# orjfickel/Small-Project-UV-Robot-Ray-Tracer

Hardware: AMD Instinct MI355X
Metric: Mray/s (extend+shade) on C046_1.glb 1920x1080x8-bounce (higher is better)
Workload: dtype f32; 1 GPU; testroomopt.glb (stand-in for the absent rooms/C046_1.glb), 2073600 photons/launch x 8 waves, lamp 0 of lange_route.xml, SEED_0=0; step = reset + generate + extend of all waves (batched), accumulate + shade replayed per wave + sync; triangles=44866, mode=batched, launch_pipelining=True, flavour=0, seed_mode=0, wide_bvh=False, parallelism=1 GPU, self_comm=False, high_priority_stream=False, full=False

## Files before the change

include/uvrt.h:

```cpp
#ifndef UVRT_H
#define UVRT_H

#include <stdint.h>

#ifdef __cplusplus
extern "C" {
#endif

typedef struct uvrt_ctx uvrt_ctx;

enum {
    UVRT_OK = 0,
    UVRT_ERR_INVALID = -1,
    UVRT_ERR_HIP = -2,
    UVRT_ERR_NO_DEVICE = -3,
    UVRT_ERR_BVH = -4,
    UVRT_ERR_STACK = -5
};

enum { UVRT_MAP_SUM = 0, UVRT_MAP_MAX = 1 };

const char* uvrt_last_error(void);
const char* uvrt_version(void);

// ... 32 lines not shown

int uvrt_get_seed(uvrt_ctx* ctx, uint32_t* seed);
int uvrt_set_seed(uvrt_ctx* ctx, uint32_t seed);
uint32_t uvrt_seed_next(const float light_pos[3], float light_length, uint32_t seed_prev);

int uvrt_advance_seed(uvrt_ctx* ctx, const float light_pos[3], float light_length);

int uvrt_set_seed_mode(uvrt_ctx* ctx, int32_t mode);
uint32_t uvrt_seed_next_mode(const float light_pos[3], float light_length, uint32_t seed_prev,
                             int32_t seed_mode);

int uvrt_generate_sweep(uvrt_ctx* ctx, const float from[3], const float to[3], float light_length,
                        int64_t first_gid, int64_t n);
uint32_t uvrt_seed_next_sweep(const float from[3], float light_length, uint32_t seed_prev);
int uvrt_write_free_rays(uvrt_ctx* ctx, const void* rays32, int64_t n);

int uvrt_occluded(uvrt_ctx* ctx, const void* rays32, int64_t n, uint8_t* out);
typedef struct {
    float from[3], to[3];
    float light_length;
    int32_t samples;
    uint32_t seed;
    int32_t photons_equiv;
    int32_t reserved[2];
} uvrt_gather_params;
enum { UVRT_GATHER_INDEPENDENT = 0, UVRT_GATHER_STRATIFIED = 1 };
int uvrt_set_gather_sampling(uvrt_ctx* ctx, int32_t mode);
int uvrt_get_gather_sampling(uvrt_ctx* ctx, int32_t* mode);
int uvrt_set_gather_variance(uvrt_ctx* ctx, int32_t on);
int uvrt_get_gather_variance(uvrt_ctx* ctx, int32_t* on);
int uvrt_read_variance(uvrt_ctx* ctx, double* out, int32_t first, int32_t count);
int uvrt_write_variance(uvrt_ctx* ctx, const double* in, int32_t first, int32_t count);
int uvrt_gather_direct(uvrt_ctx* ctx, const uvrt_gather_params* params, int32_t first_tri, int32_t tri_count);
int uvrt_accumulate_expected(uvrt_ctx* ctx, float time_step, int32_t tri_count);
int uvrt_read_expected(uvrt_ctx* ctx, double* out, int32_t first, int32_t count);
int uvrt_write_expected(uvrt_ctx* ctx, const double* in, int32_t first, int32_t count);

typedef struct {
    double  rel_error;
    double  min_expected;
    int32_t max_extra;
    uint32_t seed;
    int32_t reserved[2];
} uvrt_refine_params;
typedef struct { int64_t extra_rays; int32_t refined; int32_t reserved; } uvrt_refine_report;
int uvrt_gather_refine(uvrt_ctx* ctx, const uvrt_refine_params* params, int32_t first_tri, int32_t tri_count,
                       uvrt_refine_report* report );
int uvrt_read_gather_extra(uvrt_ctx* ctx, int32_t* out, int32_t first, int32_t count);
int uvrt_refine_counts(uvrt_ctx* ctx, int32_t samples0, const uvrt_refine_params* params, int32_t first_tri, int32_t tri_count,
                       int32_t* offsets_out );

enum { UVRT_GATHER_BATCH_MAX = 64 };
int uvrt_gather_direct_batch(uvrt_ctx* ctx, const uvrt_gather_params* launches, int32_t count,
                             int32_t first_tri, int32_t tri_count);
int uvrt_gather_batch_select(uvrt_ctx* ctx, int32_t k);
int uvrt_gather_batch_info(uvrt_ctx* ctx, int32_t out4[4]);
int uvrt_read_gather_batch(uvrt_ctx* ctx, int32_t k, int32_t which, double* out, int32_t first, int32_t count);

int uvrt_closest_hits(uvrt_ctx* ctx, const void* rays32, int64_t n, float* dist_out, int32_t* tri_out);

typedef struct {
    float    reflectance;
    int32_t  samples;
    uint32_t seed;
    int32_t  add;
    int32_t  reserved[2];
} uvrt_indirect_params;
int uvrt_indirect_source_from_expected(uvrt_ctx* ctx);
int uvrt_read_indirect_source(uvrt_ctx* ctx, double* out, int32_t first, int32_t count);
int uvrt_write_indirect_source(uvrt_ctx* ctx, const double* in, int32_t first, int32_t count);
int uvrt_gather_indirect(uvrt_ctx* ctx, const uvrt_indirect_params* params, int32_t first_tri, int32_t tri_count);
int uvrt_gather_indirect_rays(uvrt_ctx* ctx, const uvrt_indirect_params* params, int32_t first_tri, int32_t tri_count,
                              void* rays32_out);

typedef struct {
    int32_t  samples;
    uint32_t seed;
    int32_t  reserved[2];
} uvrt_links_params;
int uvrt_indirect_links_build(uvrt_ctx* ctx, const uvrt_links_params* params);
int uvrt_indirect_links_info(uvrt_ctx* ctx, int32_t out4[4]);
int uvrt_read_indirect_links(uvrt_ctx* ctx, int32_t* out, int32_t first_tri, int32_t tri_count);
typedef struct {
    float    reflectance;
    int32_t  bounces;
    int32_t  add;
    int32_t  reserved[3];
} uvrt_linked_params;
int uvrt_gather_indirect_linked(uvrt_ctx* ctx, const uvrt_linked_params* params, int32_t first_tri, int32_t tri_count);

int uvrt_set_gather_faces(uvrt_ctx* ctx, int32_t on);
int uvrt_get_gather_faces(uvrt_ctx* ctx, int32_t* on);
int uvrt_read_gather_faces(uvrt_ctx* ctx, int32_t face, double* out, int32_t first, int32_t count);
int uvrt_write_gather_faces(uvrt_ctx* ctx, int32_t face, const double* in, int32_t first, int32_t count);
int uvrt_indirect_links_build_sided(uvrt_ctx* ctx, const uvrt_links_params* params);
int uvrt_gather_indirect_linked_sided(uvrt_ctx* ctx, const uvrt_linked_params* params, int32_t first_tri, int32_t tri_count);

typedef struct {
    float duration;
    int32_t shade;
    int32_t which_map;
    int32_t photons_per_light;
    float scaled_power, min_value;
    int32_t threshold_view;
} uvrt_replay_op;

int uvrt_trace_batch(uvrt_ctx* ctx, const float* lamps, float light_length, int32_t count,
                     int64_t first_gid, int64_t n);
enum { UVRT_LAUNCH_STOP = 0, UVRT_LAUNCH_SWEEP = 1 };
typedef struct {
    float from[3];
    float to[3];
    int32_t kind;
    int32_t reserved;
} uvrt_launch;
int uvrt_trace_batch_launches(uvrt_ctx* ctx, const uvrt_launch* launches, float light_length,
                              int32_t count, int64_t first_gid, int64_t n);
int uvrt_replay_batch(uvrt_ctx* ctx, const uvrt_replay_op* ops, int32_t count, int32_t tri_count);
int uvrt_fold_batch(uvrt_ctx* ctx);
int uvrt_read_batch_counts(uvrt_ctx* ctx, int32_t launch, int32_t* out, int32_t first, int32_t count);

int uvrt_set_dedupe(uvrt_ctx* ctx, int32_t on);
int uvrt_set_dedupe_classes(uvrt_ctx* ctx, int32_t max_classes);
int uvrt_get_dedupe_classes(uvrt_ctx* ctx, int32_t* max_classes);
int32_t uvrt_dedupe_classes_default(void);
int uvrt_batch_deposits(uvrt_ctx* ctx, int64_t* out);
int uvrt_batch_residue(uvrt_ctx* ctx, int64_t* nonzero);
int uvrt_dedupe_classes(const float lamp[3], int32_t count, const uint32_t* seed_prev, const uint32_t* seed_next,
                        int32_t seed_mode, int64_t first_gid, int64_t n, int32_t max_classes, uint32_t* class_masks,
                        int32_t* class_count, int64_t* deposits);
int uvrt_set_helper_priority(uvrt_ctx* ctx, int32_t prio);
int uvrt_get_helper_priority(uvrt_ctx* ctx, int32_t* prio);
int uvrt_batch_traced_rays(uvrt_ctx* ctx, int64_t* out);
uint32_t uvrt_seed_input(int64_t gid, const float lamp[3], uint32_t seed_prev, uint32_t seed_next, int32_t seed_mode);
int uvrt_dedupe_plan(const float lamp[3], int32_t count, const uint32_t* seed_prev, const uint32_t* seed_next,
                     int32_t seed_mode, int64_t first_gid, int64_t n, uint32_t* masks);
int uvrt_dedupe_plan_tiled(const float lamp[3], int32_t count, const uint32_t* seed_prev, const uint32_t* seed_next,
                           int32_t seed_mode, int64_t first_gid, int64_t n, int32_t tile_keys, int64_t chunk_first,
                           int64_t chunk_n, uint32_t* masks);
int uvrt_dedupe_plan_strips(const float lamp[3], int32_t count, const uint32_t* seed_prev, const uint32_t* seed_next,
                            int32_t seed_mode, int64_t first_gid, int64_t n, int32_t tile_keys, int32_t strip_tiles,
                            int64_t chunk_first, int64_t chunk_n, uint32_t* masks);
int uvrt_dedupe_mark_device(uvrt_ctx* ctx, const float lamp[3], int32_t count, const uint32_t* seed_prev,
                            const uint32_t* seed_next, int32_t seed_mode, int64_t first_gid, int64_t n, int64_t chunk_first,
                            int64_t chunk_n, uint32_t* masks, uint32_t* block_owner_counts);
int uvrt_set_dedupe_periodic(uvrt_ctx* ctx, int32_t on);
int uvrt_get_dedupe_periodic(uvrt_ctx* ctx, int32_t* on);
int uvrt_dedupe_plan_periodic(const float lamp[3], int32_t count, const uint32_t* seed_prev, const uint32_t* seed_next,
                              int32_t seed_mode, int64_t first_gid, int64_t n, int64_t chunk_first, int64_t chunk_n,
                              uint32_t* masks, uint32_t* block_owner_counts, int64_t* from_table);
int uvrt_dedupe_generate_device(uvrt_ctx* ctx, const float lamp[3], float light_length, int32_t count, const uint32_t* seed_prev,
                                const uint32_t* seed_next, int32_t seed_mode, int64_t first_gid, int64_t n, int64_t chunk_first,
                                int64_t chunk_n, float* rays, uint32_t* words, uint32_t* total, uint32_t* deposits);

int uvrt_comm_available(void);
int uvrt_comm_unique_id(void* id128);
int uvrt_comm_init_rank(uvrt_ctx* ctx, const void* id128, int32_t rank, int32_t world);
int uvrt_comm_init_all(uvrt_ctx** ctxs, int32_t n);
int uvrt_comm_destroy(uvrt_ctx* ctx);
int uvrt_comm_info(uvrt_ctx* ctx, int32_t out4[4]);
int uvrt_reduce_batch(uvrt_ctx* ctx);
int uvrt_reduce_batch_group(uvrt_ctx** ctxs, int32_t n);

enum { UVRT_PLAN_CONVERGED = 0, UVRT_PLAN_ITERATION_CAP = 1 };
typedef struct {
    float min_dose;
    float scaled_power;
    int64_t photons_per_position;
    int32_t min_photons;
    int32_t max_iterations;
    double margin;
    double rel_gap;
    const uint8_t* mask;
    int32_t reserved[2];
} uvrt_plan_params;
typedef struct {
    int32_t status;
    int32_t iterations;
    int32_t positions;
    int32_t used_positions;
    int32_t required, unreachable, unresolved, masked_out;
    double area_required, area_unreachable, area_unresolved, area_masked_out;
    double total_duration;
    double lower_bound;
    double gap;
    double min_dose_ratio;
} uvrt_plan_report;
int uvrt_plan_begin(uvrt_ctx* ctx, int32_t positions);
int uvrt_plan_capture_batch(uvrt_ctx* ctx, const int32_t* position_of_launch, int32_t count);
int uvrt_plan_solve(uvrt_ctx* ctx, const uvrt_plan_params* params, float* durations_out, uvrt_plan_report* report);
int uvrt_plan_model_dose(uvrt_ctx* ctx, const float* durations, float* out, int32_t first, int32_t count);
int uvrt_plan_read_exposure(uvrt_ctx* ctx, int32_t position, uint32_t* out, int32_t first, int32_t count);
int uvrt_plan_read_required(uvrt_ctx* ctx, uint8_t* out, int32_t first, int32_t count);
int uvrt_plan_write_exposure(uvrt_ctx* ctx, int32_t position, const uint32_t* in, int32_t first, int32_t count);
int uvrt_plan_end(uvrt_ctx* ctx);
typedef struct {
    const float*   lower;
    const uint8_t* fixed;
    int32_t reserved[2];
} uvrt_plan_bounds;
typedef struct {
    int32_t fixed_columns, free_columns;
    int32_t met_by_lower;
    int32_t short_rows;
    double  area_met_by_lower, area_short;
    double  lower_total;
    int32_t reserved[2];
} uvrt_plan_bounds_report;
int uvrt_plan_solve_bounded(uvrt_ctx* ctx, const uvrt_plan_params* params, const uvrt_plan_bounds* bounds,
                            float* durations_out, uvrt_plan_report* report, uvrt_plan_bounds_report* bounds_report );
int uvrt_plan_read_classes(uvrt_ctx* ctx, uint8_t* out, int32_t first, int32_t count);
int uvrt_plan_begin_expected(uvrt_ctx* ctx, int32_t positions);
int uvrt_plan_capture_expected(uvrt_ctx* ctx, int32_t position);
int uvrt_plan_read_exposure_expected(uvrt_ctx* ctx, int32_t position, double* out, int32_t first, int32_t count);
int uvrt_plan_begin_expected_variance(uvrt_ctx* ctx, int32_t positions);
int uvrt_plan_read_exposure_variance(uvrt_ctx* ctx, int32_t position, double* out, int32_t first, int32_t count);
int uvrt_plan_lower_confidence(uvrt_ctx* ctx, double z);
float uvrt_plan_round_trip_up(float v);

int uvrt_set_sort_bits(uvrt_ctx* ctx, int32_t bits);
int uvrt_set_record_hits(uvrt_ctx* ctx, int32_t on);
int uvrt_set_flavour(uvrt_ctx* ctx, int32_t flavour);
int uvrt_set_wide_bvh(uvrt_ctx* ctx, int32_t on);
int uvrt_set_hot_records(uvrt_ctx* ctx, int32_t mode);
int uvrt_set_record_perm(uvrt_ctx* ctx, const uint32_t* perm, int32_t n);
int uvrt_read_record_perm(uvrt_ctx* ctx, uint32_t* out, int32_t n);

int uvrt_set_pipeline(uvrt_ctx* ctx, int32_t on);

int uvrt_set_variant(uvrt_ctx* ctx, int32_t variant);

int uvrt_read_rays(uvrt_ctx* ctx, void* rays32, int64_t first, int64_t count);
int uvrt_write_rays(uvrt_ctx* ctx, const void* rays32, int64_t n);
int uvrt_read_counts(uvrt_ctx* ctx, int32_t* out, int32_t first, int32_t count);
int uvrt_read_photon_map(uvrt_ctx* ctx, int32_t which_map, double* out, int32_t first,
                         int32_t count);
int uvrt_device_ptr(uvrt_ctx* ctx, int32_t which, void** ptr, int64_t* bytes);
int uvrt_copy_device(uvrt_ctx* ctx, int32_t which, void* ext_dev_ptr, int32_t to_ctx);
int uvrt_extend_time_ms(uvrt_ctx* ctx, double* ms, int64_t* launches);
int uvrt_set_timing(uvrt_ctx* ctx, int32_t on);
int uvrt_clock_probe_start(uvrt_ctx* ctx, int32_t microseconds);
int uvrt_clock_probe_read(uvrt_ctx* ctx, double* shader_mhz);
int uvrt_device_cus(uvrt_ctx* ctx);
int uvrt_device_count(void);

#ifdef __cplusplus
}
#endif
#endif
```

small-project-uv-robot-ray-tracer_amd/capi.py:

```python
from __future__ import annotations

import ctypes as C
import os

import numpy as np

_HERE = os.path.dirname(os.path.abspath(__file__))
LIB_PATH = os.path.join(_HERE, "libuvrt_hip.so")
LIB_DEV_PATH = os.path.join(_HERE, "libuvrt_hip_dev.so")

RAY_DT = np.dtype([("dirx", "<f4"), ("diry", "<f4"), ("dirz", "<f4"),
                   ("origx", "<f4"), ("origy", "<f4"), ("origz", "<f4"),
                   ("dist", "<f4"), ("triID", "<u4")])

MAP_SUM, MAP_MAX = 0, 1

_vp, _i32, _i64, _f32, _u32 = C.c_void_p, C.c_int32, C.c_int64, C.c_float, C.c_uint32
_fp = C.POINTER(C.c_float)
SYMBOLS = [
    ("uvrt_last_error", C.c_char_p, []),
    ("uvrt_version", C.c_char_p, []),
    ("uvrt_create", C.c_int, [C.c_int, C.POINTER(_vp)]),
    ("uvrt_destroy", None, [_vp]),
    ("uvrt_set_stream", C.c_int, [_vp, _vp]),
    ("uvrt_set_scene", C.c_int, [_vp, _vp, _i32, _vp, _i32, _vp]),
    ("uvrt_resize_rays", C.c_int, [_vp, _i64]),
    ("uvrt_reset", C.c_int, [_vp, _i32]),
    ("uvrt_generate", C.c_int, [_vp, _fp, _f32, _i64, _i64]),
    ("uvrt_extend", C.c_int, [_vp, _i64]),
    ("uvrt_accumulate", C.c_int, [_vp, _f32, _i32]),
    ("uvrt_compute_dosage", C.c_int, [_vp, _i32, _i32, _f32, _i32]),
    ("uvrt_dosage_to_color", C.c_int, [_vp, _f32, _i32, _i32]),
    ("uvrt_shade", C.c_int, [_vp, _i32, _i32, _f32, _f32, _i32, _i32]),
    ("uvrt_sync", C.c_int, [_vp]),
    ("uvrt_read_dosage", C.c_int, [_vp, _vp, _i32, _i32]),
    ("uvrt_read_color", C.c_int, [_vp, _vp, _i32, _i32]),
    ("uvrt_get_seed", C.c_int, [_vp, C.POINTER(_u32)]),
    ("uvrt_set_seed", C.c_int, [_vp, _u32]),
    ("uvrt_seed_next", _u32, [_fp, _f32, _u32]),
    ("uvrt_trace_batch", C.c_int, [_vp, _fp, _f32, _i32, _i64, _i64]),
    ("uvrt_trace_batch_launches", C.c_int, [_vp, _vp, _f32, _i32, _i64, _i64]),
    ("uvrt_replay_batch", C.c_int, [_vp, _vp, _i32, _i32]),
    ("uvrt_fold_batch", C.c_int, [_vp]),
    ("uvrt_read_batch_counts", C.c_int, [_vp, _i32, _vp, _i32, _i32]),
    ("uvrt_set_dedupe", C.c_int, [_vp, _i32]),
    ("uvrt_set_helper_priority", C.c_int, [_vp, _i32]),
    ("uvrt_get_helper_priority", C.c_int, [_vp, C.POINTER(_i32)]),
    ("uvrt_batch_traced_rays", C.c_int, [_vp, C.POINTER(_i64)]),
    ("uvrt_set_dedupe_classes", C.c_int, [_vp, _i32]),
    ("uvrt_get_dedupe_classes", C.c_int, [_vp, C.POINTER(_i32)]),
    ("uvrt_dedupe_classes_default", _i32, []),
    ("uvrt_batch_deposits", C.c_int, [_vp, C.POINTER(_i64)]),
    ("uvrt_batch_residue", C.c_int, [_vp, C.POINTER(_i64)]),
    ("uvrt_dedupe_classes", C.c_int, [_fp, _i32, _vp, _vp, _i32, _i64, _i64, _i32, _vp, C.POINTER(_i32), C.POINTER(_i64)]),
    ("uvrt_seed_input", _u32, [_i64, _fp, _u32, _u32, _i32]),
    ("uvrt_dedupe_plan", C.c_int, [_fp, _i32, _vp, _vp, _i32, _i64, _i64, _vp]),
    ("uvrt_dedupe_plan_tiled", C.c_int, [_fp, _i32, _vp, _vp, _i32, _i64, _i64, _i32, _i64, _i64, _vp]),
    ("uvrt_dedupe_plan_strips", C.c_int, [_fp, _i32, _vp, _vp, _i32, _i64, _i64, _i32, _i32, _i64, _i64, _vp]),
    ("uvrt_dedupe_mark_device", C.c_int, [_vp, _fp, _i32, _vp, _vp, _i32, _i64, _i64, _i64, _i64, _vp, _vp]),
    ("uvrt_set_dedupe_periodic", C.c_int, [_vp, _i32]),
    ("uvrt_get_dedupe_periodic", C.c_int, [_vp, C.POINTER(_i32)]),
    ("uvrt_dedupe_plan_periodic", C.c_int, [_fp, _i32, _vp, _vp, _i32, _i64, _i64, _i64, _i64, _vp, _vp, C.POINTER(_i64)]),
    ("uvrt_dedupe_generate_device", C.c_int, [_vp, _fp, C.c_float, _i32, _vp, _vp, _i32, _i64, _i64, _i64, _i64, _vp, _vp,
                                              C.POINTER(C.c_uint32), C.POINTER(C.c_uint32)]),
    ("uvrt_comm_available", C.c_int, []),
    ("uvrt_comm_info", C.c_int, [_vp, C.POINTER(_i32)]),
    ("uvrt_comm_unique_id", C.c_int, [_vp]),
    ("uvrt_comm_init_rank", C.c_int, [_vp, _vp, _i32, _i32]),
    ("uvrt_comm_init_all", C.c_int, [C.POINTER(_vp), _i32]),
    ("uvrt_comm_destroy", C.c_int, [_vp]),
    ("uvrt_reduce_batch", C.c_int, [_vp]),
    ("uvrt_reduce_batch_group", C.c_int, [C.POINTER(_vp), _i32]),
    ("uvrt_advance_seed", C.c_int, [_vp, _fp, _f32]),
    ("uvrt_set_seed_mode", C.c_int, [_vp, _i32]),
    ("uvrt_seed_next_mode", _u32, [_fp, _f32, _u32, _i32]),
    ("uvrt_set_sort_bits", C.c_int, [_vp, _i32]),
    ("uvrt_set_record_hits", C.c_int, [_vp, _i32]),
    ("uvrt_set_flavour", C.c_int, [_vp, _i32]),
    ("uvrt_set_variant", C.c_int, [_vp, _i32]),
    ("uvrt_set_pipeline", C.c_int, [_vp, _i32]),
    ("uvrt_set_record_perm", C.c_int, [_vp, _vp, _i32]),
    ("uvrt_read_record_perm", C.c_int, [_vp, _vp, _i32]),
    ("uvrt_set_hot_records", C.c_int, [_vp, _i32]),
    ("uvrt_set_wide_bvh", C.c_int, [_vp, _i32]),
    ("uvrt_read_rays", C.c_int, [_vp, _vp, _i64, _i64]),
    ("uvrt_write_rays", C.c_int, [_vp, _vp, _i64]),
    ("uvrt_write_free_rays", C.c_int, [_vp, _vp, _i64]),
    ("uvrt_generate_sweep", C.c_int, [_vp, _fp, _fp, _f32, _i64, _i64]),
    ("uvrt_seed_next_sweep", _u32, [_fp, _f32, _u32]),
    ("uvrt_occluded", C.c_int, [_vp, _vp, _i64, _vp]),
    ("uvrt_gather_direct", C.c_int, [_vp, _vp, _i32, _i32]),
    ("uvrt_set_gather_sampling", C.c_int, [_vp, _i32]),
    ("uvrt_get_gather_sampling", C.c_int, [_vp, C.POINTER(_i32)]),
    ("uvrt_accumulate_expected", C.c_int, [_vp, _f32, _i32]),
    ("uvrt_read_expected", C.c_int, [_vp, _vp, _i32, _i32]),
    ("uvrt_write_expected", C.c_int, [_vp, _vp, _i32, _i32]),
    ("uvrt_read_counts", C.c_int, [_vp, _vp, _i32, _i32]),
    ("uvrt_read_photon_map", C.c_int, [_vp, _i32, _vp, _i32, _i32]),
    ("uvrt_device_ptr", C.c_int, [_vp, _i32, C.POINTER(_vp), C.POINTER(_i64)]),
    ("uvrt_copy_device", C.c_int, [_vp, _i32, _vp, _i32]),
    ("uvrt_extend_time_ms", C.c_int, [_vp, C.POINTER(C.c_double), C.POINTER(_i64)]),
    ("uvrt_set_timing", C.c_int, [_vp, _i32]),
    ("uvrt_clock_probe_start", C.c_int, [_vp, _i32]),
    ("uvrt_clock_probe_read", C.c_int, [_vp, C.POINTER(C.c_double)]),
    ("uvrt_device_cus", C.c_int, [_vp]),
    ("uvrt_device_count", C.c_int, []),
    ("uvrt_plan_begin", C.c_int, [_vp, _i32]),
    ("uvrt_plan_capture_batch", C.c_int, [_vp, _vp, _i32]),
    ("uvrt_plan_solve", C.c_int, [_vp, _vp, _vp, _vp]),
    ("uvrt_plan_model_dose", C.c_int, [_vp, _vp, _vp, _i32, _i32]),
    ("uvrt_plan_read_exposure", C.c_int, [_vp, _i32, _vp, _i32, _i32]),
    ("uvrt_plan_read_required", C.c_int, [_vp, _vp, _i32, _i32]),
    ("uvrt_plan_end", C.c_int, [_vp]),
    ("uvrt_plan_solve_bounded", C.c_int, [_vp, _vp, _vp, _vp, _vp, _vp]),
    ("uvrt_plan_read_classes", C.c_int, [_vp, _vp, _i32, _i32]),
    ("uvrt_plan_round_trip_up", _f32, [_f32]),
    ("uvrt_plan_begin_expected", C.c_int, [_vp, _i32]),
    ("uvrt_plan_capture_expected", C.c_int, [_vp, _i32]),
    ("uvrt_plan_read_exposure_expected", C.c_int, [_vp, _i32, _vp, _i32, _i32]),
    ("uvrt_set_gather_variance", C.c_int, [_vp, _i32]),
    ("uvrt_get_gather_variance", C.c_int, [_vp, C.POINTER(_i32)]),
    ("uvrt_read_variance", C.c_int, [_vp, _vp, _i32, _i32]),
    ("uvrt_write_variance", C.c_int, [_vp, _vp, _i32, _i32]),
    ("uvrt_plan_begin_expected_variance", C.c_int, [_vp, _i32]),
    ("uvrt_plan_read_exposure_variance", C.c_int, [_vp, _i32, _vp, _i32, _i32]),
    ("uvrt_plan_lower_confidence", C.c_int, [_vp, C.c_double]),
    ("uvrt_plan_write_exposure", C.c_int, [_vp, _i32, _vp, _i32, _i32]),
    ("uvrt_gather_refine", C.c_int, [_vp, _vp, _i32, _i32, _vp]),
    ("uvrt_read_gather_extra", C.c_int, [_vp, _vp, _i32, _i32]),
    ("uvrt_refine_counts", C.c_int, [_vp, _i32, _vp, _i32, _i32, _vp]),
    ("uvrt_gather_direct_batch", C.c_int, [_vp, _vp, _i32, _i32, _i32]),
    ("uvrt_gather_batch_select", C.c_int, [_vp, _i32]),
    ("uvrt_gather_batch_info", C.c_int, [_vp, _vp]),
    ("uvrt_read_gather_batch", C.c_int, [_vp, _i32, _i32, _vp, _i32, _i32]),
    ("uvrt_closest_hits", C.c_int, [_vp, _vp, _i64, _vp, _vp]),
    ("uvrt_indirect_source_from_expected", C.c_int, [_vp]),
    ("uvrt_read_indirect_source", C.c_int, [_vp, _vp, _i32, _i32]),
    ("uvrt_write_indirect_source", C.c_int, [_vp, _vp, _i32, _i32]),
    ("uvrt_gather_indirect", C.c_int, [_vp, _vp, _i32, _i32]),
    ("uvrt_gather_indirect_rays", C.c_int, [_vp, _vp, _i32, _i32, _vp]),
    ("uvrt_indirect_links_build", C.c_int, [_vp, _vp]),
    ("uvrt_indirect_links_info", C.c_int, [_vp, _vp]),
    ("uvrt_read_indirect_links", C.c_int, [_vp, _vp, _i32, _i32]),
    ("uvrt_gather_indirect_linked", C.c_int, [_vp, _vp, _i32, _i32]),
    ("uvrt_set_gather_faces", C.c_int, [_vp, _i32]),
    ("uvrt_get_gather_faces", C.c_int, [_vp, C.POINTER(_i32)]),
    ("uvrt_read_gather_faces", C.c_int, [_vp, _i32, _vp, _i32, _i32]),
    ("uvrt_write_gather_faces", C.c_int, [_vp, _i32, _vp, _i32, _i32]),
    ("uvrt_indirect_links_build_sided", C.c_int, [_vp, _vp]),
    ("uvrt_gather_indirect_linked_sided", C.c_int, [_vp, _vp, _i32, _i32]),
]

PLAN_CONVERGED, PLAN_ITERATION_CAP = 0, 1


class GatherParams(C.Structure):
    _fields_ = [("from_", C.c_float * 3), ("to", C.c_float * 3), ("light_length", C.c_float), ("samples", C.c_int32),
                ("seed", C.c_uint32), ("photons_equiv", C.c_int32), ("reserved", C.c_int32 * 2)]


class RefineParams(C.Structure):
    _fields_ = [("rel_error", C.c_double), ("min_expected", C.c_double), ("max_extra", C.c_int32), ("seed", C.c_uint32),
                ("reserved", C.c_int32 * 2)]


class RefineReport(C.Structure):
    _fields_ = [("extra_rays", C.c_int64), ("refined", C.c_int32), ("reserved", C.c_int32)]


class IndirectParams(C.Structure):
    _fields_ = [("reflectance", C.c_float), ("samples", C.c_int32), ("seed", C.c_uint32), ("add", C.c_int32),
                ("reserved", C.c_int32 * 2)]


class LinksParams(C.Structure):
    _fields_ = [("samples", C.c_int32), ("seed", C.c_uint32), ("reserved", C.c_int32 * 2)]


class LinkedParams(C.Structure):
    _fields_ = [("reflectance", C.c_float), ("bounces", C.c_int32), ("add", C.c_int32), ("reserved", C.c_int32 * 3)]


class PlanParams(C.Structure):
    _fields_ = [("min_dose", C.c_float), ("scaled_power", C.c_float), ("photons_per_position", C.c_int64),
                ("min_photons", C.c_int32), ("max_iterations", C.c_int32), ("margin", C.c_double),
                ("rel_gap", C.c_double), ("mask", C.c_void_p), ("reserved", C.c_int32 * 2)]


class PlanReport(C.Structure):
    _fields_ = [("status", C.c_int32), ("iterations", C.c_int32), ("positions", C.c_int32), ("used_positions", C.c_int32),
                ("required", C.c_int32), ("unreachable", C.c_int32), ("unresolved", C.c_int32), ("masked_out", C.c_int32),
                ("area_required", C.c_double), ("area_unreachable", C.c_double), ("area_unresolved", C.c_double),
                ("area_masked_out", C.c_double), ("total_duration", C.c_double), ("lower_bound", C.c_double),
                ("gap", C.c_double), ("min_dose_ratio", C.c_double)]

    def as_dict(self):
        d = {name: getattr(self, name) for name, _ in self._fields_}
        d["converged"] = d["status"] == PLAN_CONVERGED
        return d


class PlanBounds(C.Structure):
    _fields_ = [("lower", C.c_void_p), ("fixed", C.c_void_p), ("reserved", C.c_int32 * 2)]


class PlanBoundsReport(C.Structure):
    _fields_ = [("fixed_columns", C.c_int32), ("free_columns", C.c_int32), ("met_by_lower", C.c_int32),
                ("short_rows", C.c_int32), ("area_met_by_lower", C.c_double), ("area_short", C.c_double),
                ("lower_total", C.c_double), ("reserved", C.c_int32 * 2)]

    def as_dict(self):
        return {name: getattr(self, name) for name, _ in self._fields_ if name != "reserved"}


PLAN_ACTIVE, PLAN_UNREACHABLE, PLAN_UNRESOLVED, PLAN_MASKED_OUT, PLAN_MET_BY_LOWER, PLAN_SHORT = range(6)


def round_trip_up(v):
    return np.float32(lib().uvrt_plan_round_trip_up(float(np.float32(v))))

REPLAY_OP_DT = np.dtype([("duration", "<f4"), ("shade", "<i4"), ("which_map", "<i4"), ("photons_per_light", "<i4"),
                         ("scaled_power", "<f4"), ("min_value", "<f4"), ("threshold_view", "<i4")])

LAUNCH_STOP, LAUNCH_SWEEP = 0, 1
LAUNCH_DT = np.dtype([("from", "<f4", (3,)), ("to", "<f4", (3,)), ("kind", "<i4"), ("reserved", "<i4")])


def stop(at):
    return (tuple(at), (0.0, 0.0, 0.0), LAUNCH_STOP, 0)


def sweep(frm, to):
    return (tuple(frm), tuple(to), LAUNCH_SWEEP, 0)


_LIB = {}


class UvrtError(RuntimeError):
    pass


def lib(dev=False):
    if dev not in _LIB:
        path = LIB_DEV_PATH if dev else LIB_PATH
        if not os.path.exists(path):
            raise UvrtError("HIP extension missing: %s (run `python -c 'import __graft_entry__ as g; "
                            "g.build()'` or `make -C small-project-uv-robot-ray-tracer_amd`). "
                            "There is no CPU fallback." % path)
        L = C.CDLL(path)
        for name, res, args in SYMBOLS:
            fn = getattr(L, name)
            fn.restype = res
            fn.argtypes = args
        _LIB[dev] = L
    return _LIB[dev]


def needs_dev(variant):
    return variant != 0 and variant % 10 != 1


def _f3(v):
    return (C.c_float * 3)(*[float(np.float32(x)) for x in v])


def _ptr(a):
    return a.ctypes.data_as(C.c_void_p)


def seed_next(light_pos, light_length, seed_prev, seed_mode=0):
    return int(lib().uvrt_seed_next_mode(_f3(light_pos), float(np.float32(light_length)), int(seed_prev),
                                         int(seed_mode)))


def seed_input(gid, lamp, seed_prev, seed_next_, seed_mode=0):
    return int(lib().uvrt_seed_input(int(gid), _f3(lamp), int(seed_prev), int(seed_next_), int(seed_mode)))


def dedupe_plan(lamp, seed_prev, seed_next_, seed_mode, first_gid, n):
    sp = np.ascontiguousarray(seed_prev, dtype=np.uint32)
    sn = np.ascontiguousarray(seed_next_, dtype=np.uint32)
    assert sp.size == sn.size
    out = np.empty((sp.size, int(n)), dtype=np.uint32)
    rc = lib().uvrt_dedupe_plan(_f3(lamp), int(sp.size), _ptr(sp), _ptr(sn), int(seed_mode), int(first_gid), int(n), _ptr(out))
    if rc != 0:
        raise UvrtError("uvrt error %d: %s" % (rc, lib().uvrt_last_error().decode()))
    return out


def dedupe_classes_default():
    return int(lib().uvrt_dedupe_classes_default())


def dedupe_classes(lamp, seed_prev, seed_next_, seed_mode, first_gid, n, max_classes=None):
    sp = np.ascontiguousarray(seed_prev, dtype=np.uint32)
    sn = np.ascontiguousarray(seed_next_, dtype=np.uint32)
    assert sp.size == sn.size
    max_classes = dedupe_classes_default() if max_classes is None else max_classes
    out = np.zeros(DEDUPE_CLASS_MAX, dtype=np.uint32)
    nc, dep = _i32(), _i64()
    rc = lib().uvrt_dedupe_classes(_f3(lamp), int(sp.size), _ptr(sp), _ptr(sn), int(seed_mode), int(first_gid), int(n),
                                   int(max_classes), _ptr(out), C.byref(nc), C.byref(dep))
    if rc != 0:
        raise UvrtError("uvrt error %d: %s" % (rc, lib().uvrt_last_error().decode()))
    return out[:int(nc.value)].copy(), int(dep.value)


DEDUPE_CLASS_MAX = 32
DEDUPE_CLASS_LAUNCHES = 30
DEDUPE_TILE_KEYS = 3840
DEDUPE_MARK_KEYS = 960
DEDUPE_STRIP_TILES = 4
DEDUPE_BLOCK_GIDS = 2048


def dedupe_plan_tiled(lamp, seed_prev, seed_next_, seed_mode, first_gid, n, tile_keys=DEDUPE_TILE_KEYS, chunk_first=None,
                      chunk_n=None, strip_tiles=None):
    sp = np.ascontiguousarray(seed_prev, dtype=np.uint32)
    sn = np.ascontiguousarray(seed_next_, dtype=np.uint32)
    assert sp.size == sn.size
    chunk_first = first_gid if chunk_first is None else chunk_first
    chunk_n = n if chunk_n is None else chunk_n
    out = np.empty((sp.size, int(chunk_n)), dtype=np.uint32)
    if strip_tiles is None:
        rc = lib().uvrt_dedupe_plan_tiled(_f3(lamp), int(sp.size), _ptr(sp), _ptr(sn), int(seed_mode), int(first_gid), int(n),
                                          int(tile_keys), int(chunk_first), int(chunk_n), _ptr(out))
    else:
        rc = lib().uvrt_dedupe_plan_strips(_f3(lamp), int(sp.size), _ptr(sp), _ptr(sn), int(seed_mode), int(first_gid), int(n),
                                           int(tile_keys), int(strip_tiles), int(chunk_first), int(chunk_n), _ptr(out))
    if rc != 0:
        raise UvrtError("uvrt error %d: %s" % (rc, lib().uvrt_last_error().decode()))
    return out


def dedupe_plan_periodic(lamp, seed_prev, seed_next_, seed_mode, first_gid, n, chunk_first=None, chunk_n=None):
    sp = np.ascontiguousarray(seed_prev, dtype=np.uint32)
    sn = np.ascontiguousarray(seed_next_, dtype=np.uint32)
    assert sp.size == sn.size
    chunk_first = first_gid if chunk_first is None else chunk_first
    chunk_n = n if chunk_n is None else chunk_n
    masks = np.empty((sp.size, int(chunk_n)), dtype=np.uint32)
    owners = np.empty((sp.size, (int(chunk_n) + DEDUPE_BLOCK_GIDS - 1) // DEDUPE_BLOCK_GIDS), dtype=np.uint32)
    from_table = _i64()
    rc = lib().uvrt_dedupe_plan_periodic(_f3(lamp), int(sp.size), _ptr(sp), _ptr(sn), int(seed_mode), int(first_gid), int(n),
                                         int(chunk_first), int(chunk_n), _ptr(masks), _ptr(owners), C.byref(from_table))
    if rc != 0:
        raise UvrtError("uvrt error %d: %s" % (rc, lib().uvrt_last_error().decode()))
    return masks, owners, int(from_table.value)


def seed_next_sweep(frm, light_length, seed_prev):
    return int(lib().uvrt_seed_next_sweep(_f3(frm), float(np.float32(light_length)), int(seed_prev)))


def comm_unique_id():
    buf = C.create_string_buffer(128)
    rc = lib().uvrt_comm_unique_id(buf)
    if rc != 0:
        raise UvrtError("uvrt error %d: %s" % (rc, lib().uvrt_last_error().decode()))
    return buf.raw


def comm_available():
    ok = bool(lib().uvrt_comm_available())
    return ok, ("" if ok else lib().uvrt_last_error().decode())


def _ctx_array(ctxs):
    return (C.c_void_p * len(ctxs))(*[c._h for c in ctxs])


def comm_init_all(ctxs):
    rc = lib().uvrt_comm_init_all(_ctx_array(ctxs), len(ctxs))
    if rc != 0:
        raise UvrtError("uvrt error %d: %s" % (rc, lib().uvrt_last_error().decode()))


def reduce_batch_group(ctxs):
    rc = lib().uvrt_reduce_batch_group(_ctx_array(ctxs), len(ctxs))
    if rc != 0:
        raise UvrtError("uvrt error %d: %s" % (rc, lib().uvrt_last_error().decode()))


class Ctx:

    def __init__(self, device=0, dev=False):
        self._L = lib(dev)
        h = C.c_void_p()
        self._h = None
        self._ck(self._L.uvrt_create(int(device), C.byref(h)))
        self._h = h
        self.T = 0

    def _ck(self, rc):
        if rc != 0:
            raise UvrtError("uvrt error %d: %s" % (rc, self._L.uvrt_last_error().decode()))

    def close(self):
        if self._h is not None:
            self._L.uvrt_destroy(self._h)
            self._h = None

    def __del__(self):
        try:
            self.close()
        except Exception:
            pass

    def set_stream(self, stream_ptr):
        self._ck(self._L.uvrt_set_stream(self._h, C.c_void_p(stream_ptr or 0)))

    def set_scene(self, tris, nodes, tri_idx):
        tris = np.ascontiguousarray(tris, dtype=np.float32).reshape(-1, 16)
        nodes = np.ascontiguousarray(nodes)
        tri_idx = np.ascontiguousarray(tri_idx, dtype=np.uint32)
        assert nodes.dtype.itemsize == 32
        self._ck(self._L.uvrt_set_scene(self._h, _ptr(tris), tris.shape[0], _ptr(nodes), nodes.shape[0],
                                        _ptr(tri_idx)))
        self.T = tris.shape[0]

    def resize_rays(self, n):
        self._ck(self._L.uvrt_resize_rays(self._h, int(n)))

    def reset(self, reset_color=True):
        self._ck(self._L.uvrt_reset(self._h, int(bool(reset_color))))

    def generate(self, light_pos, light_length, first_gid, n):
        self._ck(self._L.uvrt_generate(self._h, _f3(light_pos), float(np.float32(light_length)),
                                       int(first_gid), int(n)))

    def extend(self, n):
# ... 163 lines not shown

    def read_gather_batch(self, k, which=0, first=0, count=None):
        count = self.T - first if count is None else count
        out = np.empty(count, dtype=np.float64)
        self._ck(self._L.uvrt_read_gather_batch(self._h, int(k), int(which), _ptr(out), int(first), int(count)))
        return out

    def closest_hits(self, rays):
        rays = np.ascontiguousarray(rays, dtype=RAY_DT)
        dist = np.zeros(rays.size, dtype=np.float32)
        tri = np.zeros(rays.size, dtype=np.int32)
        self._ck(self._L.uvrt_closest_hits(self._h, _ptr(rays), rays.size, _ptr(dist), _ptr(tri)))
        return dist, tri

    def indirect_source_from_expected(self):
        self._ck(self._L.uvrt_indirect_source_from_expected(self._h))

    def read_indirect_source(self, first=0, count=None):
        count = self.T - first if count is None else count
        out = np.empty(count, dtype=np.float64)
        self._ck(self._L.uvrt_read_indirect_source(self._h, _ptr(out), int(first), int(count)))
        return out

    def write_indirect_source(self, values, first=0):
        v = np.ascontiguousarray(values, dtype=np.float64)
        self._ck(self._L.uvrt_write_indirect_source(self._h, _ptr(v), int(first), int(v.size)))

    @staticmethod
    def _indirect_params(reflectance, samples, seed, add):
        prm = IndirectParams()
        prm.reflectance = float(np.float32(reflectance))
        prm.samples = int(samples)
        prm.seed = int(seed) & 0xFFFFFFFF
        prm.add = int(add)
        return prm

    def gather_indirect(self, reflectance, samples, seed, add=0, first_tri=0, tri_count=None):
        prm = self._indirect_params(reflectance, samples, seed, add)
        self._ck(self._L.uvrt_gather_indirect(self._h, C.byref(prm), int(first_tri),
                                              self.T - int(first_tri) if tri_count is None else int(tri_count)))

    def gather_indirect_rays(self, reflectance, samples, seed, first_tri=0, tri_count=None):
        prm = self._indirect_params(reflectance, samples, seed, 0)
        tri_count = self.T - int(first_tri) if tri_count is None else int(tri_count)
        out = np.zeros(max(tri_count, 0) * max(int(samples), 0), dtype=RAY_DT)
        self._ck(self._L.uvrt_gather_indirect_rays(self._h, C.byref(prm), int(first_tri), tri_count, _ptr(out)))
        return out

    def indirect_links_build(self, samples, seed):
        prm = LinksParams()
        prm.samples = int(samples)
        prm.seed = int(seed) & 0xFFFFFFFF
        self._ck(self._L.uvrt_indirect_links_build(self._h, C.byref(prm)))

    def indirect_links_info(self):
        out = np.zeros(4, dtype=np.int32)
        self._ck(self._L.uvrt_indirect_links_info(self._h, _ptr(out)))
        return int(out[0]), int(out[1]) & 0xFFFFFFFF, int(out[2])

    def read_indirect_links(self, first_tri=0, tri_count=None):
        tri_count = self.T - int(first_tri) if tri_count is None else int(tri_count)
        s2 = self.indirect_links_info()[0]
        n = max(tri_count, 0) * s2
        out = np.zeros(max(n, 1), dtype=np.int32)
        self._ck(self._L.uvrt_read_indirect_links(self._h, _ptr(out), int(first_tri), tri_count))
        return out[:n].reshape(max(tri_count, 0), s2)

    def gather_indirect_linked(self, reflectance, bounces, add=0, first_tri=0, tri_count=None):
        prm = LinkedParams()
        prm.reflectance = float(np.float32(reflectance))
        prm.bounces = int(bounces)
        prm.add = int(add)
        self._ck(self._L.uvrt_gather_indirect_linked(self._h, C.byref(prm), int(first_tri),
                                                     self.T - int(first_tri) if tri_count is None else int(tri_count)))

    def indirect_links_build_sided(self, samples, seed):
        prm = LinksParams()
        prm.samples = int(samples)
        prm.seed = int(seed) & 0xFFFFFFFF
        self._ck(self._L.uvrt_indirect_links_build_sided(self._h, C.byref(prm)))

    def indirect_links_kind(self):
        out = np.zeros(4, dtype=np.int32)
        self._ck(self._L.uvrt_indirect_links_info(self._h, _ptr(out)))
        return int(out[3])

    def gather_indirect_linked_sided(self, reflectance, bounces, add=0, first_tri=0, tri_count=None):
        prm = LinkedParams()
        prm.reflectance = float(np.float32(reflectance))
        prm.bounces = int(bounces)
        prm.add = int(add)
        self._ck(self._L.uvrt_gather_indirect_linked_sided(self._h, C.byref(prm), int(first_tri),
                                                           self.T - int(first_tri) if tri_count is None else int(tri_count)))

    @property
    def seed(self):
        s = C.c_uint32()
        self._ck(self._L.uvrt_get_seed(self._h, C.byref(s)))
        return int(s.value)

    @seed.setter
    def seed(self, v):
        self._ck(self._L.uvrt_set_seed(self._h, int(v)))

    def trace_batch(self, lamps, light_length, first_gid, n):
        lamps = np.ascontiguousarray(lamps, dtype=np.float32).reshape(-1, 3)
        self._ck(self._L.uvrt_trace_batch(self._h, lamps.ctypes.data_as(_fp), float(np.float32(light_length)),
                                          lamps.shape[0], int(first_gid), int(n)))

    def trace_batch_launches(self, launches, light_length, first_gid, n):
        launches = np.ascontiguousarray(np.array(launches, dtype=LAUNCH_DT))
        self._ck(self._L.uvrt_trace_batch_launches(self._h, _ptr(launches), float(np.float32(light_length)),
                                                   launches.size, int(first_gid), int(n)))

    def replay_batch(self, ops, tri_count=None):
        ops = np.ascontiguousarray(np.array(ops, dtype=REPLAY_OP_DT))
        self._ck(self._L.uvrt_replay_batch(self._h, _ptr(ops), ops.size, self.T if tri_count is None else int(tri_count)))

    def fold_batch(self):
        self._ck(self._L.uvrt_fold_batch(self._h))

    def read_batch_counts(self, launch, first=0, count=None):
        count = self.T - first if count is None else count
        out = np.empty(count, dtype=np.int32)
        self._ck(self._L.uvrt_read_batch_counts(self._h, int(launch), _ptr(out), first, count))
        return out

    def set_dedupe(self, on):
        self._ck(self._L.uvrt_set_dedupe(self._h, 1 if on else 0))

    def set_helper_priority(self, prio):
        self._ck(self._L.uvrt_set_helper_priority(self._h, int(prio)))

    def get_helper_priority(self):
        m = _i32()
        self._ck(self._L.uvrt_get_helper_priority(self._h, C.byref(m)))
        return int(m.value)

    def set_dedupe_classes(self, max_classes):
        self._ck(self._L.uvrt_set_dedupe_classes(self._h, int(max_classes)))

    def get_dedupe_classes(self):
        m = _i32()
        self._ck(self._L.uvrt_get_dedupe_classes(self._h, C.byref(m)))
        return int(m.value)

    def set_dedupe_periodic(self, on):
        self._ck(self._L.uvrt_set_dedupe_periodic(self._h, 1 if on else 0))

    def get_dedupe_periodic(self):
        on = _i32()
        self._ck(self._L.uvrt_get_dedupe_periodic(self._h, C.byref(on)))
        return bool(on.value)

    def dedupe_generate_device(self, lamp, light_length, seed_prev, seed_next_, seed_mode, first_gid, n, chunk_first=None,
                               chunk_n=None):
        sp = np.ascontiguousarray(seed_prev, dtype=np.uint32)
        sn = np.ascontiguousarray(seed_next_, dtype=np.uint32)
        assert sp.size == sn.size
        chunk_first = first_gid if chunk_first is None else chunk_first
        chunk_n = n if chunk_n is None else chunk_n
        rays = np.zeros((sp.size * int(chunk_n), 4), dtype=np.float32)
        words = np.zeros(sp.size * int(chunk_n), dtype=np.uint32)
        total, deposits = C.c_uint32(), C.c_uint32()
        self._ck(self._L.uvrt_dedupe_generate_device(self._h, _f3(lamp), float(np.float32(light_length)), int(sp.size), _ptr(sp),
                                                     _ptr(sn), int(seed_mode), int(first_gid), int(n), int(chunk_first),
                                                     int(chunk_n), _ptr(rays), _ptr(words), C.byref(total), C.byref(deposits)))
        return rays[:total.value].copy(), words[:total.value].copy(), int(deposits.value)

    def batch_deposits(self):
        out = _i64()
        self._ck(self._L.uvrt_batch_deposits(self._h, C.byref(out)))
        return int(out.value)

    def batch_residue(self):
        out = _i64()
        self._ck(self._L.uvrt_batch_residue(self._h, C.byref(out)))
        return int(out.value)

    def batch_traced_rays(self):
        out = _i64()
        self._ck(self._L.uvrt_batch_traced_rays(self._h, C.byref(out)))
        return int(out.value)

    def dedupe_mark_device(self, lamp, seed_prev, seed_next_, seed_mode, first_gid, n, chunk_first=None, chunk_n=None):
        sp = np.ascontiguousarray(seed_prev, dtype=np.uint32)
        sn = np.ascontiguousarray(seed_next_, dtype=np.uint32)
        assert sp.size == sn.size
        chunk_first = first_gid if chunk_first is None else chunk_first
        chunk_n = n if chunk_n is None else chunk_n
        masks = np.empty((sp.size, int(chunk_n)), dtype=np.uint32)
        owners = np.empty((sp.size, (int(chunk_n) + DEDUPE_BLOCK_GIDS - 1) // DEDUPE_BLOCK_GIDS), dtype=np.uint32)
        self._ck(self._L.uvrt_dedupe_mark_device(self._h, _f3(lamp), int(sp.size), _ptr(sp), _ptr(sn), int(seed_mode),
                                                 int(first_gid), int(n), int(chunk_first), int(chunk_n), _ptr(masks),
                                                 _ptr(owners)))
        return masks, owners

    def comm_init_rank(self, id128, rank, world):
        assert len(id128) == 128
        self._ck(self._L.uvrt_comm_init_rank(self._h, C.c_char_p(id128), int(rank), int(world)))

    def comm_info(self):
        out = (C.c_int32 * 4)()
        self._ck(self._L.uvrt_comm_info(self._h, out))
        return {"world": int(out[0]), "rank": int(out[1]), "rccl_ranks": int(out[2]), "reserved_cus": int(out[3])}

    def comm_destroy(self):
        self._ck(self._L.uvrt_comm_destroy(self._h))

    def reduce_batch(self):
        self._ck(self._L.uvrt_reduce_batch(self._h))

    def advance_seed(self, light_pos, light_length):
        self._ck(self._L.uvrt_advance_seed(self._h, _f3(light_pos), float(np.float32(light_length))))

    def set_seed_mode(self, mode):
        self._ck(self._L.uvrt_set_seed_mode(self._h, int(mode)))

    def set_gather_sampling(self, mode):
        self._ck(self._L.uvrt_set_gather_sampling(self._h, int(mode)))

    def get_gather_sampling(self):
        m = _i32()
        self._ck(self._L.uvrt_get_gather_sampling(self._h, C.byref(m)))
        return int(m.value)

    def set_gather_variance(self, on):
        self._ck(self._L.uvrt_set_gather_variance(self._h, int(on)))

    def set_gather_faces(self, on):
        self._ck(self._L.uvrt_set_gather_faces(self._h, int(on)))

    def get_gather_faces(self):
        v = C.c_int32()
        self._ck(self._L.uvrt_get_gather_faces(self._h, C.byref(v)))
        return int(v.value)

    def get_gather_variance(self):
        v = _i32()
        self._ck(self._L.uvrt_get_gather_variance(self._h, C.byref(v)))
        return int(v.value)

    def set_sort_bits(self, bits):
        self._ck(self._L.uvrt_set_sort_bits(self._h, int(bits)))

    def set_record_hits(self, on):
        self._ck(self._L.uvrt_set_record_hits(self._h, int(bool(on))))

    def set_flavour(self, f):
        self._ck(self._L.uvrt_set_flavour(self._h, int(f)))

    def set_record_perm(self, perm):
        if perm is None:
            self._ck(self._L.uvrt_set_record_perm(self._h, None, 0))
            return
        perm = np.ascontiguousarray(perm, dtype=np.uint32)
        self._ck(self._L.uvrt_set_record_perm(self._h, perm.ctypes.data, int(perm.size)))

    def read_record_perm(self, npairs):
        out = np.empty(int(npairs), dtype=np.uint32)
        self._ck(self._L.uvrt_read_record_perm(self._h, _ptr(out), int(npairs)))
        return out

    def set_wide_bvh(self, on):
        self._ck(self._L.uvrt_set_wide_bvh(self._h, int(bool(on))))

    def set_hot_records(self, mode):
        self._ck(self._L.uvrt_set_hot_records(self._h, int(mode)))

    def set_pipeline(self, on):
        self._ck(self._L.uvrt_set_pipeline(self._h, int(bool(on))))

    def set_variant(self, v):
        self._ck(self._L.uvrt_set_variant(self._h, int(v)))

    def set_timing(self, on):
        self._ck(self._L.uvrt_set_timing(self._h, int(bool(on))))

    def extend_time_ms(self):
        ms, n = C.c_double(), C.c_int64()
        self._ck(self._L.uvrt_extend_time_ms(self._h, C.byref(ms), C.byref(n)))
        return float(ms.value), int(n.value)

    def copy_device(self, which, ext_ptr, to_ctx):
        self._ck(self._L.uvrt_copy_device(self._h, int(which), C.c_void_p(int(ext_ptr)), int(bool(to_ctx))))

    def clock_probe_start(self, microseconds):
        self._ck(self._L.uvrt_clock_probe_start(self._h, int(microseconds)))

    def clock_probe_read(self):
        mhz = C.c_double()
        self._ck(self._L.uvrt_clock_probe_read(self._h, C.byref(mhz)))
        return float(mhz.value)

    def device_cus(self):
        return int(self._L.uvrt_device_cus(self._h))

    def plan_begin(self, positions):
        self._ck(self._L.uvrt_plan_begin(self._h, int(positions)))
        self._plan_p = int(positions)

    def plan_begin_expected(self, positions):
        self._ck(self._L.uvrt_plan_begin_expected(self._h, int(positions)))
        self._plan_p = int(positions)

    def plan_capture_expected(self, position):
# ... 109 lines not shown
```

small-project-uv-robot-ray-tracer_amd/csrc/uvrt_capi.hip:

```cpp
#include "uvrt_ctx.h"
#include "uvrt_scene_layout.h"

#include <climits>
#include <cstddef>

using namespace uvrt;
using namespace uvrt_impl;

namespace uvrt_impl {

thread_local std::string g_err;

int fail(int code, const char* fmt, ...)
{
    char buf[512];
    va_list ap;
    va_start(ap, fmt);
    vsnprintf(buf, sizeof buf, fmt, ap);
    va_end(ap);
    g_err = buf;
    return code;
}

}

uvrt_ctx::~uvrt_ctx()
{
    plan_drop(this);
    (void)hot_reset(this, false);
    for (hipEvent_t e : {ev_fence, ev_mapfence}) if (e) (void)hipEventDestroy(e);
    for (hipEvent_t e : ev_pool) (void)hipEventDestroy(e);
    if (host_flag) (void)hipHostFree(host_flag);
    if (probe_stream) (void)hipStreamDestroy(probe_stream);
    if (own_stream) (void)hipStreamDestroy(own_stream);
}

namespace {

namespace sl = uvrt::scene_layout;
using sl::SceneLayout;

#define SAME_FIELD(A, B, f) (offsetof(A, f) == offsetof(B, f))
static_assert(sizeof(sl::F4) == sizeof(float4) && SAME_FIELD(sl::F4, float4, x) && SAME_FIELD(sl::F4, float4, y) &&
              SAME_FIELD(sl::F4, float4, z) && SAME_FIELD(sl::F4, float4, w), "F4 is float4's words");
static_assert(sizeof(sl::PairWords) == sizeof(PairRec) && SAME_FIELD(sl::PairWords, PairRec, c0min_ref0) &&
              SAME_FIELD(sl::PairWords, PairRec, c0max_ref1) && SAME_FIELD(sl::PairWords, PairRec, c1min) &&
              SAME_FIELD(sl::PairWords, PairRec, c1max), "PairWords is PairRec");
static_assert(sizeof(sl::QuadWords) == sizeof(QuadRec) && SAME_FIELD(sl::QuadWords, QuadRec, xz) && SAME_FIELD(sl::QuadWords, QuadRec, y01) &&
              SAME_FIELD(sl::QuadWords, QuadRec, y23) && SAME_FIELD(sl::QuadWords, QuadRec, ref) && SAME_FIELD(sl::QuadWords, QuadRec, pad),
              "QuadWords is QuadRec");
#undef SAME_FIELD
static_assert(sl::REF_LEAF_BIT == uvrt::REF_LEAF_BIT && sl::REF_DONE == uvrt::REF_DONE && sl::REF_COUNT_SHIFT == uvrt::REF_COUNT_SHIFT &&
              sl::MAX_TRIS == uvrt::MAX_TRIS && sl::TOP6_MAX == uvrt::TOP6_MAX, "uvrt_scene_layout.h restates uvrt_device.h's constants");

template <class I>
bool env_int(const char* name, long lo, long hi, I& field)
{
    const char* e = getenv(name);
    if (!e) return false;
    const long v = atol(e);
    if (v < lo || v > hi) return false;
    field = (I)v;
    return true;
}
void env_bool(const char* name, bool& field)
{
    if (const char* e = getenv(name)) field = atoi(e) != 0;
}

int provision_scene(uvrt_ctx* c, const SceneLayout& L, int32_t T)
{
    const bool resized = (T != c->T);
    int rc;
    if ((rc = c->pairs.ensure(std::max<size_t>(L.pairs.size(), 1) * sizeof(PairRec), false, c->stream))) return rc;
    for (int l = 0; l < c->nlanes; ++l)
        if ((rc = c->lanes[l].recs.ensure((L.pairs.size() + (size_t)T + 1) * 64, true, c->stream))) return rc;
    if ((rc = c->ltris.ensure((size_t)T * sizeof(LeafTri) + 16, true, c->stream))) return rc;
    if ((rc = c->leaf_count.ensure((size_t)T * 4, false, c->stream))) return rc;
    if ((rc = c->area.ensure((size_t)T * 4, false, c->stream))) return rc;
    if (resized || !c->photon_map.p) {
        for (DevBuf* b : {&c->photon_map, &c->max_map, &c->dosage}) b->release();
        for (Lane& La : c->lanes) La.counts.release();
        if ((rc = c->photon_map.ensure((size_t)T * 8, true, c->stream))) return rc;
        if ((rc = c->max_map.ensure((size_t)T * 8, true, c->stream))) return rc;
        int R = c->replicas_knob > 0 ? c->replicas_knob : 16;
        while (R > 1 && (size_t)R * (size_t)T * 4 > ((size_t)64 << 20)) R >>= 1;
        c->replicas = R;
        for (int l = 0; l < c->nlanes; ++l)
            if ((rc = c->lanes[l].counts.ensure((size_t)R * (size_t)T * 4, true, c->stream))) return rc;
        if ((rc = c->dosage.ensure((size_t)T * 4, true, c->stream))) return rc;
        if ((rc = c->color.ensure((size_t)T * 36, true, c->stream))) return rc;
    }
    return UVRT_OK;
}

int upload_scene(uvrt_ctx* c, const SceneLayout& L, const void* tris64, int32_t T, const uint32_t* tri_idx)
{
    int rc;
    if (!L.pairs.empty())
        HIP_TRY(hipMemcpyAsync(c->pairs.p, L.pairs.data(), L.pairs.size() * sizeof(PairRec), hipMemcpyHostToDevice, c->stream));
    if ((rc = c->quads.ensure(std::max<size_t>(L.quads.size(), 1) * sizeof(QuadRec), false, c->stream))) return rc;
    if (!L.quads.empty())
        HIP_TRY(hipMemcpyAsync(c->quads.p, L.quads.data(), L.quads.size() * sizeof(QuadRec), hipMemcpyHostToDevice, c->stream));
    HIP_TRY(hipMemcpyAsync(c->leaf_count.p, L.leaf_count.data(), (size_t)T * 4, hipMemcpyHostToDevice, c->stream));
    DevBuf d_tris, d_idx;
    if ((rc = d_tris.ensure((size_t)T * 64, false, c->stream))) return rc;
    if ((rc = d_idx.ensure((size_t)T * 4, false, c->stream))) return rc;
    HIP_TRY(hipMemcpyAsync(d_tris.p, tris64, (size_t)T * 64, hipMemcpyHostToDevice, c->stream));
    HIP_TRY(hipMemcpyAsync(d_idx.p, tri_idx, (size_t)T * 4, hipMemcpyHostToDevice, c->stream));
    launch_prepare_scene(d_tris.as<float4>(), d_idx.as<uint32_t>(), c->ltris.as<LeafTri>(),
                         c->area.as<float>(), T, c->stream);
    for (int l = 0; l < c->nlanes; ++l)
        launch_prepare_leaves6(c->ltris.as<LeafTri>(), c->lanes[l].recs.p, (int32_t)L.pairs.size(), T, c->stream);
    HIP_TRY(hipGetLastError());
    HIP_TRY(hipStreamSynchronize(c->stream));
    c->T = T;
    c->root_ref = L.root_ref;
    c->top_pairs = L.top_pairs;
    c->npairs = (int32_t)L.pairs.size();
    c->nquads = (int32_t)L.quads.size();
    c->top_quads = L.top_quads;
    c->scene_force_exact = L.force_exact;
    c->have_scene = true;
    return UVRT_OK;
}

int void_scene_state(uvrt_ctx* c)
{
    for (Lane& La : c->lanes) { La.recs_tag.valid = false; La.recs4_tag.valid = false; }
    for (Lane& La : c->lanes) La.recs4.release();
    c->have_perm = false;
    c->derived = {};
    if (int rc = hot_reset(c, true)) return rc;
    HIP_TRY(hipStreamSynchronize(c->stream));
    plan_drop(c);
    c->b_count = 0;
    c->b_is_folded = false;
    c->b_recs.clear();
    c->b_recs_key.clear();
    for (auto& bset : c->bs) for (DevBuf* b : {&bset.planes, &bset.folded}) b->release();
    return UVRT_OK;
}

}

extern "C" {

const char* uvrt_last_error(void) { return g_err.c_str(); }
const char* uvrt_version(void) { return "uvrt-mi355x 0.1 (gfx950)"; }
int uvrt_clock_probe_start(uvrt_ctx* c, int32_t microseconds)
{
    if (!c || microseconds < 1 || microseconds > 1000000) return fail(UVRT_ERR_INVALID, "uvrt_clock_probe_start: 1 .. 1 000 000 us");
    HIP_TRY(hipSetDevice(c->device));
    if (!c->probe_stream) {
        int lo = 0, hi = 0;
        HIP_TRY(hipDeviceGetStreamPriorityRange(&lo, &hi));
        HIP_TRY(hipStreamCreateWithPriority(&c->probe_stream, hipStreamNonBlocking, hi));
    }
    if (int rc = c->probe_out.ensure(16, true, c->probe_stream)) return rc;
    launch_clock_probe(c->probe_out.as<unsigned long long>(), (unsigned long long)microseconds * 100ull, c->probe_stream);
    HIP_TRY(hipGetLastError());
    return UVRT_OK;
}

int uvrt_clock_probe_read(uvrt_ctx* c, double* shader_mhz)
{
    if (!c || !shader_mhz || !c->probe_stream) return fail(UVRT_ERR_INVALID, "uvrt_clock_probe_read: no probe started");
    HIP_TRY(hipSetDevice(c->device));
    unsigned long long v[2] = {0, 0};
    HIP_TRY(hipMemcpyAsync(v, c->probe_out.p, 16, hipMemcpyDeviceToHost, c->probe_stream));
    HIP_TRY(hipStreamSynchronize(c->probe_stream));
    if (v[1] == 0) return fail(UVRT_ERR_HIP, "uvrt_clock_probe_read: the probe wrote nothing");
    *shader_mhz = (double)v[0] / (double)v[1] * 100.0;
    return UVRT_OK;
}

int uvrt_device_cus(uvrt_ctx* c) { return c ? c->num_cus : 0; }
int uvrt_device_count(void)
{
    int n = 0;
    return hipGetDeviceCount(&n) == hipSuccess ? n : 0;
}

int uvrt_create(int device_id, uvrt_ctx** out)
{
    if (!out) return fail(UVRT_ERR_INVALID, "uvrt_create: out is NULL");
    *out = nullptr;
    int ndev = 0;
    hipError_t e = hipGetDeviceCount(&ndev);
    if (e != hipSuccess || ndev <= 0)
        return fail(UVRT_ERR_NO_DEVICE, "uvrt_create: no HIP device (%s)", hipGetErrorString(e));
    if (device_id < 0 || device_id >= ndev)
        return fail(UVRT_ERR_INVALID, "uvrt_create: device %d out of range [0,%d)", device_id, ndev);
    hipDeviceProp_t prop;
    HIP_TRY(hipGetDeviceProperties(&prop, device_id));
    if (strncmp(prop.gcnArchName, "gfx950", 6) != 0)
        return fail(UVRT_ERR_NO_DEVICE, "uvrt_create: device %d is %s, this library is built for gfx950 only",
                    device_id, prop.gcnArchName);
    std::unique_ptr<uvrt_ctx> c(new uvrt_ctx());
    c->device = device_id;
    c->hot.reserve(uvrt_ctx::HOT_MAX);
    c->num_cus = prop.multiProcessorCount > 0 ? prop.multiProcessorCount : 256;
    if (c->num_cus > 256) c->num_cus = 256;
    env_int("UVRT_REPLICAS", 1, 64, c->replicas_knob);
    HIP_TRY(hipSetDevice(device_id));
    HIP_TRY(hipStreamCreateWithFlags(&c->own_stream, hipStreamNonBlocking));
    c->stream = c->own_stream;
    for (int l = 0; l < uvrt_ctx::MAXL; ++l) {
        if (l > 0) HIP_TRY(hipStreamCreateWithFlags(&c->lanes[l].side, hipStreamNonBlocking));
        HIP_TRY(hipEventCreateWithFlags(&c->lanes[l].ev_tail, hipEventDisableTiming));
    }
    HIP_TRY(hipEventCreateWithFlags(&c->ev_fence, hipEventDisableTiming));
    HIP_TRY(hipEventCreateWithFlags(&c->ev_mapfence, hipEventDisableTiming));
    env_int("UVRT_LANES", 1, uvrt_ctx::MAXL, c->nlanes);
    env_bool("UVRT_PIPELINE", c->pipeline);
    if (long mb = 0; env_int("UVRT_BATCH_CHUNK_MB", 1, LONG_MAX, mb)) c->batch_chunk_bytes = c->dedupe_chunk_bytes = (size_t)mb << 20;
#ifdef UVRT_DEV_VARIANTS
    env_int("UVRT_PROBE_SKIP_GENERATE", INT_MIN, INT_MAX, c->probe_skip_generate);
    env_bool("UVRT_NEARFAR_MINMAX", c->nearfar_minmax);
#endif
    env_bool("UVRT_DRAIN_MERGE", c->drain_merge);
    env_bool("UVRT_DEDUPE", c->dedupe);
    env_int("UVRT_DEDUPE_CLASSES", 0, DEDUPE_CLASS_MAX, c->dedupe_classes);
    env_bool("UVRT_DEDUPE_PERIODIC", c->dedupe_periodic);
    env_int("UVRT_DEDUPE_STRIP", 1, 1024, c->dedupe_strip);
    env_int("UVRT_DEDUPE_CLASS_REPLICAS", 1, 16, c->dedupe_class_replicas);
    if (long mb = 0; env_int("UVRT_DEDUPE_CLASS_MB", 1, 4096, mb)) c->dedupe_class_bytes = (size_t)mb << 20;
    env_int("UVRT_HELPER_PRIO", 0, 3, c->helper_prio);
    env_int("UVRT_BATCH_LANES", 1, uvrt_ctx::MAXL - 1, c->batch_lanes);
    if (int cus = 0; env_int("UVRT_COMM_RESERVE_CUS", 0, 64, cus) && cus % 8 == 0) c->comm_reserve_knob = cus;
    env_int("UVRT_HOT_SAMPLE", 256, 1 << 20, c->hot_sample);
    env_int("UVRT_HOT_DIRECT", 0, 8192, c->hot_direct);
    env_int("UVRT_HOT_TAIL", 0, 63, c->hot_tail);
    if (int rc = c->error_flag.ensure(256, true, c->stream)) return rc;
#ifndef UVRT_TRIP_STATS
    void* dp = nullptr;
    HIP_TRY(hipHostMalloc((void**)&c->host_flag, 64, hipHostMallocMapped | hipHostMallocCoherent));
    HIP_TRY(hipHostGetDevicePointer(&dp, c->host_flag, 0));
    memset(c->host_flag, 0, 64);
    c->host_flag_dev = (uint32_t*)dp;
#endif
    if (int rc = c->lanes[0].ovf.ensure((size_t)OVF_MAX_ENTRIES * sizeof(uint32_t), false, c->stream)) return rc;
    *out = c.release();
    return UVRT_OK;
}

void uvrt_destroy(uvrt_ctx* c)
{
    if (!c) return;
    (void)hipSetDevice(c->device);
    (void)hipStreamSynchronize(c->stream);
    for (Lane& L : c->lanes) if (L.side) (void)hipStreamSynchronize(L.side);
    if (c->probe_stream) (void)hipStreamSynchronize(c->probe_stream);
    if (c->comm) uvrt_comm_destroy(c);
    delete c;
}

int uvrt_set_stream(uvrt_ctx* c, void* hip_stream)
{
    if (!c) return fail(UVRT_ERR_INVALID, "null context");
    if (int rc = set_device(c)) return rc;
    if (int rc = join_all(c)) return rc;
    HIP_TRY(hipStreamSynchronize(c->stream));
    c->stream = hip_stream ? (hipStream_t)hip_stream : c->own_stream;
    c->lane = 0;
    return UVRT_OK;
}

int uvrt_set_scene(uvrt_ctx* c, const void* tris64, int32_t T, const void* nodes32,
                   int32_t node_count, const uint32_t* tri_idx)
{
    if (!c) return fail(UVRT_ERR_INVALID, "uvrt_set_scene: null argument");
    SceneLayout L;
    std::string why;
    if (int rc = sl::build_scene_layout(tris64, T, nodes32, node_count, tri_idx, L, why)) return fail(rc, "%s", why.c_str());
    if (int rc = set_device(c)) return rc;
    if (int rcj = join_all(c)) return rcj;
    HIP_TRY(hipStreamSynchronize(c->stream));
    c->lane = 0;
    if (int rc = provision_scene(c, L, T)) return rc;
    if (int rc = upload_scene(c, L, tris64, T, tri_idx)) return rc;
    return void_scene_state(c);
}

int uvrt_resize_rays(uvrt_ctx* c, int64_t photon_count)
{
    if (!c || photon_count < 0) return fail(UVRT_ERR_INVALID, "uvrt_resize_rays: bad argument");
    if (int rc = set_device(c)) return rc;
    if (photon_count == c->capacity && c->lanes[0].rays.p && (!c->record_hits || c->hits.p)) { c->last = {}; return UVRT_OK; }
    if (int rcj = join_all(c)) return rcj;
    HIP_TRY(hipStreamSynchronize(c->stream));
    c->lane = 0;
    int rc;
    const size_t n = (size_t)photon_count;
    for (int l = 0; l < c->nlanes; ++l)
        if ((rc = c->lanes[l].rays.ensure(n * 16, false, c->stream))) return rc;
    if ((rc = c->keyrank.ensure(n * 8, false, c->stream))) return rc;
    if ((rc = c->sorted.ensure(n * 16, false, c->stream))) return rc;
    if ((rc = c->order.ensure(n * 4, false, c->stream))) return rc;
    if (c->record_hits && (rc = c->hits.ensure(n * 8, false, c->stream))) return rc;
    for (Lane& L : c->lanes) L.oxz.release();
    c->capacity = photon_count;
    c->last = {};
    return UVRT_OK;
}

int uvrt_reset(uvrt_ctx* c, int32_t reset_color)
{
    if (!c || !c->have_scene) return fail(UVRT_ERR_INVALID, "uvrt_reset: no scene");
    if (int rc = set_device(c)) return rc;
    if (int rc = join_all(c)) return rc;
    launch_reset(c->photon_map.as<double>(), c->max_map.as<double>(), c->lanes[0].counts.as<int32_t>(),
                 c->replicas, c->T, c->color.as<float>(), reset_color, c->T, c->helper_prio, c->stream);
    HIP_TRY(hipGetLastError());
    bool dirty = false;
    for (int l = 0; l < uvrt_ctx::MAXL; ++l) {
        Lane& L = c->lanes[l];
        if (l > 0 && L.counts_dirty && L.counts.p) {
            HIP_TRY(hipMemsetAsync(L.counts.p, 0, L.counts.bytes, c->stream));
            dirty = true;
        }
        L.counts_dirty = false;
    }
    if (c->b_count > 0) {
        if (c->b_is_folded) HIP_TRY(hipMemsetAsync(c->bs[c->b_set].folded.p, 0, c->bs[c->b_set].folded.bytes, c->stream));
        else HIP_TRY(hipMemsetAsync(c->bs[c->b_set].planes.p, 0, c->bs[c->b_set].planes.bytes, c->stream));
        HIP_TRY(hipEventRecord(c->bs[c->b_set].free_ev, c->stream));
        c->b_count = 0;
        c->b_is_folded = false;
    }
    return dirty ? mark_fence(c) : mark_map_fence(c);
}

int uvrt_set_record_perm(uvrt_ctx* c, const uint32_t* perm, int32_t n)
{
    if (!c || !c->have_scene) return fail(UVRT_ERR_INVALID, "uvrt_set_record_perm: no scene");
    if (int rc = set_device(c)) return rc;
    if (int rc = join_all(c)) return rc;
    HIP_TRY(hipStreamSynchronize(c->stream));
    for (Lane& L : c->lanes) L.recs_tag.valid = false;
    if (!perm) { c->have_perm = false; return UVRT_OK; }
    if (n != c->npairs) return fail(UVRT_ERR_INVALID, "uvrt_set_record_perm: %d entries, the scene has %d inner nodes", n, c->npairs);
    std::vector<uint8_t> seen((size_t)n, 0);
    for (int32_t i = 0; i < n; ++i) {
        if (perm[i] >= (uint32_t)n || seen[perm[i]]) return fail(UVRT_ERR_INVALID, "uvrt_set_record_perm: not a permutation");
        seen[perm[i]] = 1;
    }
    if (n == 0) { c->have_perm = false; return UVRT_OK; }
    if (int rc = c->perm.ensure((size_t)n * 4, false, c->stream)) return rc;
    if (int rc = copy_sync(c, c->perm.p, perm, (size_t)n * 4, hipMemcpyHostToDevice)) return rc;
    c->have_perm = true;
    c->perm_gen = ++c->perm_clock;
    return UVRT_OK;
}

int uvrt_read_record_perm(uvrt_ctx* c, uint32_t* out, int32_t n)
{
    if (!c || !out || !c->have_scene || n != c->npairs)
        return fail(UVRT_ERR_INVALID, "uvrt_read_record_perm: need a scene and n = its %d inner nodes", c ? c->npairs : 0);
    if (int rc = set_device(c)) return rc;
    if (int rc = join_all(c)) return rc;
    const uint32_t* pm = c->have_perm ? c->perm.as<uint32_t>() : cur_lane(c).perm;
    if (!pm) { for (int32_t i = 0; i < n; ++i) out[i] = (uint32_t)i; return UVRT_OK; }
    return copy_sync(c, out, pm, (size_t)n * 4, hipMemcpyDeviceToHost);
}

int uvrt_sync(uvrt_ctx* c)
{
    if (!c) return fail(UVRT_ERR_INVALID, "null context");
    if (int rc = set_device(c)) return rc;
    if (int rc = join_all(c)) return rc;
    uint32_t flag = 0;
#ifdef UVRT_TRIP_STATS
    HIP_TRY(hipMemcpyAsync(&flag, c->error_flag.p, 4, hipMemcpyDeviceToHost, c->stream));
    HIP_TRY(hipStreamSynchronize(c->stream));
#else
    HIP_TRY(hipStreamSynchronize(c->stream));
// ... 316 lines not shown
```

small-project-uv-robot-ray-tracer_amd/csrc/uvrt_capi_batch.hip:

```cpp
#include "uvrt_ctx.h"

using namespace uvrt;
using namespace uvrt_impl;

namespace uvrt_impl {

static BatchKnobs batch_knobs(const uvrt_ctx* c)
{
    BatchKnobs kn = {};
    kn.seed = c->seed; kn.seed_mode = c->seed_mode; kn.T = c->T; kn.replicas = c->replicas;
    kn.may_dedupe = c->dedupe && variant_code6(c->variant) == 1;
#ifdef UVRT_DEV_VARIANTS
    kn.may_dedupe = kn.may_dedupe && c->probe_skip_generate <= 0;
#endif
    kn.dedupe_classes = c->dedupe_classes; kn.dedupe_class_replicas = c->dedupe_class_replicas;
    kn.dedupe_class_bytes = c->dedupe_class_bytes; kn.dedupe_periodic = c->dedupe_periodic;
    kn.dedupe_chunk_bytes = c->dedupe_chunk_bytes; kn.batch_chunk_bytes = c->batch_chunk_bytes; kn.dedupe_strip = c->dedupe_strip;
    return kn;
}

struct BatchRun {
    uvrt_ctx* c;
    int set;
    uvrt_ctx::BatchSet& S;
    const BatchPlan& P;
    const char* who;
    float light_length;
    int64_t first_gid, n;
    const uint32_t* gperm[MAX_BATCH];
    uint64_t ggen[MAX_BATCH];
    bool lane_waited[uvrt_ctx::MAXL];
    int per_cu;
    int64_t traced;
    size_t dd_used;
};

static int provision_records(BatchRun& r, bool* recs_stale)
{
    uvrt_ctx* c = r.c;
    const BatchPlan& P = r.P;
    uvrt_ctx::HotEntry* fresh[MAX_BATCH];
    uint32_t fresh_prev[MAX_BATCH], fresh_next[MAX_BATCH];
    int nfresh = 0;
    for (int g = 0; g < P.ngroups; ++g) {
        r.gperm[g] = c->have_perm ? c->perm.as<uint32_t>() : nullptr;
        bool is_fresh = false;
        if (!r.gperm[g] && (int64_t)P.gsize[g] * r.n >= 16384) {
            const int ph = P.gfirst[g];
            const float gl[3] = {P.gp.lx[ph], P.gp.ly[ph], P.gp.lz[ph]};
            uvrt_ctx::HotEntry* e = nullptr;
            if (int rcp = hot_lookup(c, gl, c->stream, &r.gperm[g], &e)) return rcp;
            if (e) {
                r.gperm[g] = e->perm;
                fresh[nfresh] = e; fresh_prev[nfresh] = P.gp.seed_prev[ph]; fresh_next[nfresh] = P.gp.seed_next[ph];
                ++nfresh;
                is_fresh = true;
            }
        }
        r.ggen[g] = perm_generation(c, r.gperm[g]);
        if (g >= (int)c->b_recs_key.size() || !c->b_recs_key[g].holds(P.gx[g], P.gz[g], r.gperm[g], r.ggen[g]) || is_fresh) {
            *recs_stale = true;
            if (g < (int)c->b_recs_key.size()) c->b_recs_key[g].tag.valid = false;
        }
    }
    if (nfresh > 0)
        if (int rcb = hot_build(c, fresh, fresh_prev, fresh_next, nfresh, r.light_length, c->stream, 0)) return rcb;
    return UVRT_OK;
}

static int provision_batch(BatchRun& r, int count)
{
    uvrt_ctx* c = r.c;
    uvrt_ctx::BatchSet& S = r.S;
    const BatchPlan& P = r.P;
    int rc;
    const int64_t n_pad = P.n_pad;
    const size_t plane_alloc = (size_t)c->replicas * (size_t)c->T;
    const size_t planes_bytes = (size_t)count * plane_alloc * 4 + (size_t)P.class_cap * P.plane_ints * 4;
    bool dd_scratch_short = false;
    for (int l = 0; l <= c->batch_lanes; ++l)
        dd_scratch_short = dd_scratch_short || c->lanes[l].dd_tmp.bytes < P.dd_tmp_bytes || c->lanes[l].dd_blocks.bytes < P.dd_block_bytes;
    const bool need_alloc = S.rays.bytes < (size_t)count * (size_t)n_pad * 16 || S.planes.bytes < planes_bytes ||
                            S.folded.bytes < (size_t)count * (size_t)c->T * 4 || (int)c->b_recs.size() < P.ngroups || !S.free_ev ||
                            S.oxz.bytes < (size_t)P.nsweeps * (size_t)n_pad * 8 || (P.nsweeps > 0 && !c->derived.free_recs_valid) ||
                            (P.dd_chunks > 0 && (S.masks.bytes < (size_t)count * (size_t)n_pad * 4 || S.dd_counts.bytes < P.dd_chunks * 8 ||
                                                 dd_scratch_short));
    bool recs_stale = false;
    if ((rc = provision_records(r, &recs_stale))) return rc;
    if (need_alloc || recs_stale) {
        if (int rcj = join_all(c)) return rcj;
    }
    if (need_alloc) {
        HIP_TRY(hipStreamSynchronize(c->stream));
        if (!S.free_ev) HIP_TRY(hipEventCreateWithFlags(&S.free_ev, hipEventDisableTiming));
        const bool grown = S.planes.bytes < planes_bytes || S.folded.bytes < (size_t)count * (size_t)c->T * 4;
        if ((rc = S.rays.ensure((size_t)count * (size_t)n_pad * 16, false, c->stream))) return rc;
        if ((rc = S.planes.ensure(planes_bytes, true, c->stream))) return rc;
        if ((rc = S.folded.ensure((size_t)count * (size_t)c->T * 4, true, c->stream))) return rc;
        if ((rc = S.oxz.ensure((size_t)P.nsweeps * (size_t)n_pad * 8, false, c->stream))) return rc;
        if (grown) HIP_TRY(hipEventRecord(S.free_ev, c->stream));
        while ((int)c->b_recs.size() < P.ngroups) {
            DevBuf b;
            if ((rc = b.ensure(((size_t)c->npairs + (size_t)c->T + 1) * 64, true, c->stream))) return rc;
            launch_prepare_leaves6(c->ltris.as<LeafTri>(), b.p, c->npairs, c->T, c->stream);
            c->b_recs.push_back(std::move(b));
        }
        c->b_recs_key.resize(c->b_recs.size());
        for (int l = 1; l <= c->batch_lanes; ++l)
            if ((rc = c->lanes[l].ovf.ensure(side_ovf_bytes(c), false, c->stream))) return rc;
        if (P.dd_chunks > 0) {
            if ((rc = S.masks.ensure((size_t)count * (size_t)n_pad * 4, false, c->stream))) return rc;
            if ((rc = S.dd_counts.ensure(P.dd_chunks * 8, false, c->stream))) return rc;
            for (int l = 0; l <= c->batch_lanes; ++l) {
                if ((rc = c->lanes[l].dd_tmp.ensure(P.dd_tmp_bytes, false, c->stream))) return rc;
                if ((rc = c->lanes[l].dd_blocks.ensure(P.dd_block_bytes, true, c->stream))) return rc;
            }
            HIP_TRY(hipStreamSynchronize(c->stream));
        }
    }
    if (need_alloc || recs_stale) {
        for (int g = 0; g < P.ngroups; ++g) {
            uvrt_ctx::RecsKey& key = c->b_recs_key[g];
            if (key.holds(P.gx[g], P.gz[g], r.gperm[g], r.ggen[g])) continue;
            launch_prepare_launch6(c->pairs.as<PairRec>(), c->b_recs[g].p, P.gx[g], P.gz[g], c->npairs, r.gperm[g], c->helper_prio, c->stream);
            key = {{true, P.gx[g], P.gz[g]}, r.gperm[g], r.ggen[g]};
        }
        if (P.nsweeps > 0 && !c->derived.free_recs_valid)
            if ((rc = make_free_records(c))) return rc;
        HIP_TRY(hipGetLastError());
        if (int rcf = mark_fence(c)) return rcf;
    }
    return UVRT_OK;
}

static int next_chunk_lane(BatchRun& r, hipStream_t* ls)
{
    uvrt_ctx* c = r.c;
    c->lane = c->pipeline ? 1 + (int)(c->b_chunks++ % (uint64_t)c->batch_lanes) : 0;
    *ls = stream_of(c, c->lane);
    if (c->lane != 0) cur_lane(c).used = true;
    if (!r.lane_waited[c->lane]) {
        HIP_TRY(hipStreamWaitEvent(*ls, r.S.free_ev, 0));
        r.lane_waited[c->lane] = true;
    }
    return UVRT_OK;
}
static void set_planes(const BatchRun& r, ExtendParams& p, int ph0, int kc)
{
    p.counts = r.S.planes.as<int32_t>() + (size_t)ph0 * r.P.plane_ints;
    p.count_replicas = r.P.R;
    p.count_stride = r.c->T;
    p.n = (int64_t)kc * r.P.n_pad;
    p.plane_batches = (uint32_t)(r.P.n_pad / 64);
    p.plane_n = (uint32_t)r.n;
    p.plane_stride = (uint32_t)r.P.plane_ints;
}

static void fill_dedupe_chunk(const uvrt_ctx* c, GenDedupeParams& dq, const Piece& pc, int64_t g0, int64_t gn, const Lane& L, float light_length)
{
    memset(&dq, 0, sizeof dq);
    dq.g = pc.G;
    dq.cls = pc.cls;
    dq.per = pc.per;
    dq.tmp = L.dd_tmp.as<uint32_t>();
    dq.g0 = g0;
    dq.gn = gn;
    dq.block_counts = L.dd_blocks.as<uint32_t>();
    mark_tiles(c->dedupe_strip, dq);
    dq.light_length = light_length;
    dq.prio = c->helper_prio;
}
static void copy_stops(GenBatchParams& gq, const BatchPlan& P, int ph0, int kc)
{
    for (int j = 0; j < kc; ++j) {
        gq.lx[j] = P.gp.lx[ph0 + j]; gq.ly[j] = P.gp.ly[ph0 + j]; gq.lz[j] = P.gp.lz[ph0 + j];
        gq.seed_prev[j] = P.gp.seed_prev[ph0 + j]; gq.seed_next[j] = P.gp.seed_next[ph0 + j];
    }
}
static void copy_sweeps(SweepBatchParams& sq, const BatchPlan& P, int k0, int kc)
{
    for (int j = 0; j < kc; ++j) {
        sq.fx[j] = P.sp.fx[k0 + j]; sq.fy[j] = P.sp.fy[k0 + j]; sq.fz[j] = P.sp.fz[k0 + j];
        sq.tx[j] = P.sp.tx[k0 + j]; sq.ty[j] = P.sp.ty[k0 + j]; sq.tz[j] = P.sp.tz[k0 + j];
        sq.seed_prev[j] = P.sp.seed_prev[k0 + j]; sq.seed_next[j] = P.sp.seed_next[k0 + j];
    }
}

static int enqueue_dedupe_chunk(BatchRun& r, const Piece& pc, int64_t g0, int64_t gn)
{
    uvrt_ctx* c = r.c;
    const BatchPlan& P = r.P;
    const int g = pc.g, ph0 = P.gfirst[g] + pc.k0;
    hipStream_t ls;
    if (int rcl = next_chunk_lane(r, &ls)) return rcl;
    const size_t at = (size_t)ph0 * (size_t)P.n_pad + (size_t)pc.kc * (size_t)g0;
    GenDedupeParams dq;
    fill_dedupe_chunk(c, dq, pc, r.first_gid + g0, gn, cur_lane(c), r.light_length);
    dq.rays = r.S.rays.as<float4>() + at;
    dq.masks = r.S.masks.as<uint32_t>() + at;
    dq.total = r.S.dd_counts.as<uint32_t>() + r.dd_used;
    dq.deposits = r.S.dd_counts.as<uint32_t>() + P.dd_chunks + r.dd_used++;
    launch_generate_dedupe(dq, ls);
    if (int rcl = lane_stream(c, &ls)) return rcl;
    ExtendParams p;
    fill_launch(c, p, P.gx[g], P.gz[g]);
    p.rays = dq.rays;
    p.masks = dq.masks;
    p.n_dev = dq.total;
    p.counts = r.S.planes.as<int32_t>() + (size_t)ph0 * P.plane_ints;
    p.count_replicas = P.R;
    p.count_stride = c->T;
    p.n = (int64_t)pc.kc * gn;
    p.plane_stride = (uint32_t)P.plane_ints;
    p.cls_replicas = pc.cls.count > 0 ? P.cls_repl : 0;
    p.recs = c->b_recs[g].p;
    p.perm = r.gperm[g];
    p.recs_prepared = 1;
    return timed_launch(c, ls, r.who, "the stops' launch", [&] { return launch_extend6_dedupe(p, variant_code6(c->variant), r.per_cu, ls); });
}

static int enqueue_stop_chunk(BatchRun& r, int g, int ph0, int kc)
{
    uvrt_ctx* c = r.c;
    const BatchPlan& P = r.P;
    r.traced += (int64_t)kc * r.n;
    hipStream_t ls;
    if (int rcl = next_chunk_lane(r, &ls)) return rcl;
    GenBatchParams gq;
    memset(&gq, 0, sizeof gq);
    gq.rays = r.S.rays.as<float4>() + (size_t)ph0 * (size_t)P.n_pad;
    gq.n_pad = P.n_pad;
    gq.first_gid = r.first_gid;
    gq.n = r.n;
    gq.light_length = r.light_length;
    gq.seed_mode = c->seed_mode;
    gq.count = kc;
    gq.prio = c->helper_prio;
    copy_stops(gq, P, ph0, kc);
#ifdef UVRT_DEV_VARIANTS
    if (!(c->probe_skip_generate > 0 && c->probe_batches >= c->probe_skip_generate))
#endif
    launch_generate_batch(gq, ls);
    if (int rcl = lane_stream(c, &ls)) return rcl;
    ExtendParams p;
    fill_launch(c, p, P.gx[g], P.gz[g]);
    p.rays = gq.rays;
    set_planes(r, p, ph0, kc);
    p.recs = c->b_recs[g].p;
    p.perm = r.gperm[g];
    p.recs_prepared = 1;
    return timed_launch(c, ls, r.who, "the stops' launch", [&] { return launch_extend6(p, variant_code6(c->variant), r.per_cu, c->helper_prio, ls); });
}

static int enqueue_sweep_chunk(BatchRun& r, int k0, int kc)
{
    uvrt_ctx* c = r.c;
    const BatchPlan& P = r.P;
    const int ph0 = P.nstops + k0;
    hipStream_t ls;
    if (int rcl = next_chunk_lane(r, &ls)) return rcl;
    SweepBatchParams sq;
    memset(&sq, 0, sizeof sq);
    sq.rays = r.S.rays.as<float4>() + (size_t)ph0 * (size_t)P.n_pad;
    sq.oxz = r.S.oxz.as<float2>() + (size_t)k0 * (size_t)P.n_pad;
    sq.n_pad = P.n_pad;
    sq.first_gid = r.first_gid;
    sq.n = r.n;
    sq.light_length = r.light_length;
    sq.count = kc;
    sq.prio = c->helper_prio;
    copy_sweeps(sq, P, k0, kc);
#ifdef UVRT_DEV_VARIANTS
    if (!(c->probe_skip_generate > 0 && c->probe_batches >= c->probe_skip_generate))
#endif
    launch_generate_sweep_batch(sq, ls);
    if (int rcl = lane_stream(c, &ls)) return rcl;
    FreeParams fp;
    fill_launch(c, fp.e, 0.0f, 0.0f);
    fp.e.rays = sq.rays;
    fp.oxz = sq.oxz;
    set_planes(r, fp.e, ph0, kc);
    fp.e.recs = c->derived.free_recs.p;
    return timed_launch(c, ls, r.who, "the free-ray launch", [&] { return launch_extend_free_planes(fp, r.per_cu, ls); });
}

static void commit_batch(BatchRun& r, int32_t count)
{
    uvrt_ctx* c = r.c;
    const BatchPlan& P = r.P;
    c->seed = P.seed_after;
    c->lane = 0;
    c->cur_pipelined = false;
    c->last = {};
    c->b_set = r.set;
    c->b_repl = P.R;
    c->b_count = count;
    c->b_n = r.n;
    c->b_npad = P.n_pad;
    c->b_is_folded = false;
    c->b_traced_known = r.traced;
    c->b_traced_chunks = (int32_t)r.dd_used;
    c->b_ncls = P.total_cls;
    c->b_cls_repl = P.cls_repl;
    for (const Piece& pc : P.pieces)
        for (int i = 0; i < pc.ncls; ++i) c->b_cls_launches[pc.cls_base + i] = (uint64_t)pc.cls.mask[i] << (P.gfirst[pc.g] + pc.k0);
    memcpy(c->b_phys, P.phys, sizeof(int32_t) * (size_t)count);
}

static int trace_launches(uvrt_ctx* c, const uvrt_launch* launches, float light_length, int32_t count, int64_t first_gid,
                          int64_t n, const char* who)
{
    if (!c || !launches || !c->have_scene) return fail(UVRT_ERR_INVALID, "%s: null argument or no scene", who);
    if (c->b_count > 0) return fail(UVRT_ERR_INVALID, "%s: the previous batch has not been replayed (uvrt_replay_batch)", who);
    if (c->record_hits || c->sort_bits != 0)
        return fail(UVRT_ERR_INVALID, "%s: per-ray hit records and ray ordering are per-launch features", who);
    BatchPlan P;
    const char* why = nullptr;
    if (int rc = plan_batch(batch_knobs(c), launches, light_length, count, first_gid, n, P, &why)) return fail(rc, "%s: %s", who, why);
    if (P.nsweeps > 0 && c->flavour != 0 && c->flavour != 1)
        return fail(UVRT_ERR_INVALID, "%s: rays with origins of their own are traced in flavours 0 and 1 only "
                    "(uvrt_set_flavour %d)", who, c->flavour);
    if (int rc = set_device(c)) return rc;
    const int set = c->b_set ^ 1;
    BatchRun r = {c, set, c->bs[set], P, who, light_length, first_gid, n, {}, {}, {}, variant_per_cu(c->variant, c->pipeline ? 7 : 8), 0, 0};
    if (int rc = provision_batch(r, count)) return rc;
    struct LaneGuard {
        uvrt_ctx* c; int lane; uint64_t chunks; bool armed;
        ~LaneGuard() { if (armed) { c->lane = lane; c->b_chunks = chunks; } }
    } guard{c, c->lane, c->b_chunks, true};
    for (const Piece& pc : P.pieces) {
        if (pc.dd) {
            for (int64_t g0 = 0; g0 < n; g0 += pc.chunk_gids)
                if (int rc = enqueue_dedupe_chunk(r, pc, g0, std::min(pc.chunk_gids, n - g0))) return rc;
            continue;
        }
        for (int k0 = pc.k0; k0 < pc.k0 + pc.kc; k0 += P.per_chunk)
            if (int rc = enqueue_stop_chunk(r, pc.g, P.gfirst[pc.g] + k0, std::min(P.per_chunk, pc.k0 + pc.kc - k0))) return rc;
    }
    for (int k0 = 0; k0 < P.nsweeps; k0 += P.per_sweep_chunk)
        if (int rc = enqueue_sweep_chunk(r, k0, std::min(P.per_sweep_chunk, P.nsweeps - k0))) return rc;
#ifdef UVRT_DEV_VARIANTS
    ++c->probe_batches;
#endif
    guard.armed = false;
    commit_batch(r, count);
    return UVRT_OK;
}

static int hook_group(DedupeGroup& G, const char* who, const float lamp[3], int32_t count, const uint32_t* seed_prev,
                      const uint32_t* seed_next, int32_t seed_mode, int64_t first_gid, int64_t n)
{
    if (!lamp || !seed_prev || !seed_next || count < 2 || count > DEDUPE_MAX)
        return fail(UVRT_ERR_INVALID, "%s: null argument, or count outside [2,%d]", who, DEDUPE_MAX);
    memset(&G, 0, sizeof G);
    G.lx = lamp[0]; G.ly = lamp[1]; G.lz = lamp[2];
    G.seed_mode = seed_mode;
    G.count = count;
    G.first_gid = first_gid; G.n = n;
    for (int j = 0; j < count; ++j) { G.seed_prev[j] = seed_prev[j]; G.seed_next[j] = seed_next[j]; }
    if (!dedupe_group_ok(G)) return fail(UVRT_ERR_INVALID, "%s: these launches cannot form a dedupe group", who);
    return UVRT_OK;
}
static bool chunk_ok(const DedupeGroup& G, int64_t chunk_first, int64_t chunk_n)
{
    return chunk_n > 0 && chunk_first >= G.first_gid && chunk_first + chunk_n <= G.first_gid + G.n;
}
static void hook_piece_tables(const uvrt_ctx* c, std::vector<Piece>& one)
{
    Piece& pc = one[0];
    std::vector<uint32_t> table((size_t)DEDUPE_TILE_KEYS);
    pc.kc = pc.G.count;
    pc.dd = true;
    if (c->dedupe_classes > 0 && pc.kc <= DEDUPE_CLASS_LAUNCHES)
        pc.ncand = dedupe_class_tally(pc.G, table.data(), pc.cand, c->dedupe_classes, &pc.keys);
    const int first_plane = 0;
    deal_classes(one, c->dedupe_classes, pc.kc, &first_plane);
    if (c->dedupe_periodic) dedupe_periodic_build(pc.G, pc.cls, table.data(), pc.per);
}

}

extern "C" {

int uvrt_trace_batch(uvrt_ctx* c, const float* lamps, float light_length, int32_t count, int64_t first_gid, int64_t n)
{
    uvrt_launch launches[MAX_BATCH];
    memset(launches, 0, sizeof launches);
    if (lamps && count > 0 && count <= MAX_BATCH)
        for (int k = 0; k < count; ++k) {
            memcpy(launches[k].from, &lamps[3 * k], 12);
            launches[k].kind = UVRT_LAUNCH_STOP;
        }
    return trace_launches(c, lamps ? launches : nullptr, light_length, count, first_gid, n, "uvrt_trace_batch");
}

int uvrt_trace_batch_launches(uvrt_ctx* c, const uvrt_launch* launches, float light_length, int32_t count, int64_t first_gid,
                              int64_t n)
{
    return trace_launches(c, launches, light_length, count, first_gid, n, "uvrt_trace_batch_launches");
}

int uvrt_batch_traced_rays(uvrt_ctx* c, int64_t* out)
{
    if (!c || !out) return fail(UVRT_ERR_INVALID, "uvrt_batch_traced_rays: null argument");
    if (c->b_traced_known < 0) return fail(UVRT_ERR_INVALID, "uvrt_batch_traced_rays: no batch has been traced");
    int64_t total = c->b_traced_known;
    if (c->b_traced_chunks > 0) {
        std::vector<uint32_t> counts((size_t)c->b_traced_chunks);
        if (int rc = range_copy(c, c->bs[c->b_set].dd_counts.p, 4, counts.data(), 0, c->b_traced_chunks, hipMemcpyDeviceToHost)) return rc;
        for (uint32_t v : counts) total += v;
    }
    *out = total;
    return UVRT_OK;
}

int uvrt_batch_deposits(uvrt_ctx* c, int64_t* out)
{
    if (!c || !out) return fail(UVRT_ERR_INVALID, "uvrt_batch_deposits: null argument");
    if (c->b_traced_known < 0) return fail(UVRT_ERR_INVALID, "uvrt_batch_deposits: no batch has been traced");
    int64_t total = 0;
    if (c->b_traced_chunks > 0) {
        std::vector<uint32_t> counts(2 * (size_t)c->b_traced_chunks);
        if (int rc = range_copy(c, c->bs[c->b_set].dd_counts.p, 4, counts.data(), 0, 2 * c->b_traced_chunks, hipMemcpyDeviceToHost)) return rc;
        for (int32_t i = 0; i < c->b_traced_chunks; ++i) total += counts[(size_t)c->b_traced_chunks + (size_t)i];
    }
    *out = total;
    return UVRT_OK;
}

int uvrt_batch_residue(uvrt_ctx* c, int64_t* nonzero)
{
    if (!c || !nonzero) return fail(UVRT_ERR_INVALID, "uvrt_batch_residue: null argument");
    if (c->b_count > 0) return fail(UVRT_ERR_INVALID, "uvrt_batch_residue: the traced batch has not been replayed (uvrt_replay_batch)");
    if (int rc = set_device(c)) return rc;
    if (int rc = join_all(c)) return rc;
    HIP_TRY(hipStreamSynchronize(c->stream));
    const size_t piece = (size_t)16 << 20;
    std::vector<int32_t> host;
    int64_t total = 0;
    for (const uvrt_ctx::BatchSet& S : c->bs) {
        const size_t ints = S.planes.p ? S.planes.bytes / 4 : 0;
        for (size_t at = 0; at < ints; at += piece) {
            const size_t m = std::min(piece, ints - at);
            host.resize(std::max(host.size(), m));
            if (int rc = copy_sync(c, host.data(), (const int32_t*)S.planes.p + at, m * 4, hipMemcpyDeviceToHost)) return rc;
            for (size_t i = 0; i < m; ++i) total += host[i] != 0;
        }
    }
    *nonzero = total;
    return UVRT_OK;
}

uint32_t uvrt_seed_input(int64_t gid, const float lamp[3], uint32_t seed_prev, uint32_t seed_next, int32_t seed_mode)
{
    return seed_input(gid, lamp[0], lamp[1], lamp[2], seed_prev, seed_next, seed_mode);
}

int uvrt_dedupe_plan(const float lamp[3], int32_t count, const uint32_t* seed_prev, const uint32_t* seed_next, int32_t seed_mode,
                     int64_t first_gid, int64_t n, uint32_t* masks)
{
    DedupeGroup G;
    if (int rc = hook_group(G, "uvrt_dedupe_plan", masks ? lamp : nullptr, count, seed_prev, seed_next, seed_mode, first_gid, n)) return rc;
    for (int k = 0; k < count; ++k)
        for (int64_t i = 0; i < n; ++i) masks[(size_t)k * (size_t)n + (size_t)i] = dedupe_mask(G, k, first_gid + i);
    return UVRT_OK;
}

int uvrt_dedupe_plan_strips(const float lamp[3], int32_t count, const uint32_t* seed_prev, const uint32_t* seed_next,
                            int32_t seed_mode, int64_t first_gid, int64_t n, int32_t tile_keys, int32_t strip_tiles,
                            int64_t chunk_first, int64_t chunk_n, uint32_t* masks)
{
    DedupeGroup G;
    if (int rc = hook_group(G, "uvrt_dedupe_plan_tiled", lamp, count, seed_prev, seed_next, seed_mode, first_gid, n)) return rc;
    if (!masks || tile_keys <= 0 || strip_tiles <= 0 || !chunk_ok(G, chunk_first, chunk_n))
        return fail(UVRT_ERR_INVALID, "uvrt_dedupe_plan_tiled: null masks, no tile width, no strip length, or a chunk outside the range");
    std::vector<uint32_t> table((size_t)tile_keys);
    dedupe_plan_tiled(G, tile_keys, strip_tiles, chunk_first, chunk_n, table.data(), masks);
    return UVRT_OK;
}

int uvrt_dedupe_plan_tiled(const float lamp[3], int32_t count, const uint32_t* seed_prev, const uint32_t* seed_next,
                           int32_t seed_mode, int64_t first_gid, int64_t n, int32_t tile_keys, int64_t chunk_first,
                           int64_t chunk_n, uint32_t* masks)
{
    return uvrt_dedupe_plan_strips(lamp, count, seed_prev, seed_next, seed_mode, first_gid, n, tile_keys, DEDUPE_STRIP_TILES, chunk_first,
                                   chunk_n, masks);
}

int32_t uvrt_dedupe_classes_default(void) { return DEDUPE_CLASSES_DEFAULT; }

int uvrt_dedupe_classes(const float lamp[3], int32_t count, const uint32_t* seed_prev, const uint32_t* seed_next, int32_t seed_mode,
                        int64_t first_gid, int64_t n, int32_t max_classes, uint32_t* class_masks, int32_t* class_count,
                        int64_t* deposits)
{
    DedupeGroup G;
    if (int rc = hook_group(G, "uvrt_dedupe_classes", lamp, count, seed_prev, seed_next, seed_mode, first_gid, n)) return rc;
    if (!class_masks || !class_count || max_classes < 0 || max_classes > DEDUPE_CLASS_MAX)
        return fail(UVRT_ERR_INVALID, "uvrt_dedupe_classes: null output, or a maximum outside [0,%d]", DEDUPE_CLASS_MAX);
    std::vector<uint32_t> table((size_t)DEDUPE_TILE_KEYS);
    DedupeTally cand[DEDUPE_CLASS_MAX];
    int nc = 0;
    if (max_classes > 0 && count <= DEDUPE_CLASS_LAUNCHES)
        nc = dedupe_class_tally(G, table.data(), cand, max_classes, nullptr);
    for (int i = 0; i < nc; ++i) class_masks[i] = cand[i].mask;
    *class_count = nc;
    if (deposits) {
        DedupeClasses C;
        dedupe_classes_fill(C, class_masks, nc, (uint32_t)count);
        *deposits = dedupe_class_deposits(G, DEDUPE_TILE_KEYS, C, table.data());
    }
    return UVRT_OK;
}

int uvrt_dedupe_mark_device(uvrt_ctx* c, const float lamp[3], int32_t count, const uint32_t* seed_prev, const uint32_t* seed_next,
                            int32_t seed_mode, int64_t first_gid, int64_t n, int64_t chunk_first, int64_t chunk_n,
                            uint32_t* masks, uint32_t* block_owner_counts)
{
    if (!c) return fail(UVRT_ERR_INVALID, "uvrt_dedupe_mark_device: null context");
    Piece pc = {};
    if (int rc = hook_group(pc.G, "uvrt_dedupe_mark_device", lamp, count, seed_prev, seed_next, seed_mode, first_gid, n)) return rc;
    if (!masks || !block_owner_counts || !chunk_ok(pc.G, chunk_first, chunk_n))
        return fail(UVRT_ERR_INVALID, "uvrt_dedupe_mark_device: null output, or a chunk outside the range");
    if (int rc = set_device(c)) return rc;
    if (int rc = join_all(c)) return rc;
    Lane& L = c->lanes[0];
    const size_t nblocks = (size_t)count * (size_t)((chunk_n + DD_SLOTS - 1) / DD_SLOTS);
    HIP_TRY(hipStreamSynchronize(c->stream));
    if (int rc = L.dd_tmp.ensure((size_t)count * (size_t)chunk_n * 4, false, c->stream)) return rc;
    if (int rc = L.dd_blocks.ensure((size_t)count * (size_t)((chunk_n + 255) / 256) * 4, true, c->stream)) return rc;
    GenDedupeParams dq;
    fill_dedupe_chunk(c, dq, pc, chunk_first, chunk_n, L, 0.0f);
    launch_dedupe_mark(dq, c->stream);
    HIP_TRY(hipGetLastError());
    HIP_TRY(hipMemcpyAsync(masks, dq.tmp, (size_t)count * (size_t)chunk_n * 4, hipMemcpyDeviceToHost, c->stream));
    HIP_TRY(hipMemcpyAsync(block_owner_counts, dq.block_counts, nblocks * 4, hipMemcpyDeviceToHost, c->stream));
    HIP_TRY(hipMemsetAsync(dq.block_counts, 0, nblocks * 4, c->stream));
    HIP_TRY(hipStreamSynchronize(c->stream));
    return UVRT_OK;
}

int uvrt_dedupe_plan_periodic(const float lamp[3], int32_t count, const uint32_t* seed_prev, const uint32_t* seed_next,
                              int32_t seed_mode, int64_t first_gid, int64_t n, int64_t chunk_first, int64_t chunk_n,
                              uint32_t* masks, uint32_t* block_owner_counts, int64_t* from_table)
{
    DedupeGroup G;
    if (int rc = hook_group(G, "uvrt_dedupe_plan_periodic", lamp, count, seed_prev, seed_next, seed_mode, first_gid, n)) return rc;
    if (!masks || !block_owner_counts || !from_table || !chunk_ok(G, chunk_first, chunk_n))
        return fail(UVRT_ERR_INVALID, "uvrt_dedupe_plan_periodic: null output, or a chunk outside the range");
    std::vector<uint32_t> table((size_t)DEDUPE_TILE_KEYS);
    DedupeClasses none = {};
    DedupePeriodic T;
    dedupe_periodic_build(G, none, table.data(), T);
    *from_table = dedupe_plan_periodic(G, T, DEDUPE_MARK_KEYS, DEDUPE_STRIP_TILES, DD_SLOTS, chunk_first, chunk_n, table.data(), masks,
                                       block_owner_counts);
    return UVRT_OK;
}

int uvrt_dedupe_generate_device(uvrt_ctx* c, const float lamp[3], float light_length, int32_t count, const uint32_t* seed_prev,
                                const uint32_t* seed_next, int32_t seed_mode, int64_t first_gid, int64_t n, int64_t chunk_first,
                                int64_t chunk_n, float* rays, uint32_t* words, uint32_t* total, uint32_t* deposits)
{
    if (!c) return fail(UVRT_ERR_INVALID, "uvrt_dedupe_generate_device: null context");
    std::vector<Piece> one(1);
    const Piece& pc = one[0];
    if (int rc = hook_group(one[0].G, "uvrt_dedupe_generate_device", lamp, count, seed_prev, seed_next, seed_mode, first_gid, n)) return rc;
    if (!rays || !words || !total || !deposits || !chunk_ok(pc.G, chunk_first, chunk_n))
        return fail(UVRT_ERR_INVALID, "uvrt_dedupe_generate_device: null output, or a chunk outside the range");
    if (int rc = set_device(c)) return rc;
    if (int rc = join_all(c)) return rc;
    hook_piece_tables(c, one);
    Lane& L = c->lanes[0];
    const size_t slots = (size_t)count * (size_t)chunk_n;
    HIP_TRY(hipStreamSynchronize(c->stream));
    if (int rc = L.dd_tmp.ensure(slots * 4, false, c->stream)) return rc;
    if (int rc = L.dd_blocks.ensure((size_t)count * (size_t)((chunk_n + 255) / 256) * 4, true, c->stream)) return rc;
    DevBuf out_rays, out_words, out_counts;
    if (int rc = out_rays.ensure(slots * 16, false, c->stream)) return rc;
    if (int rc = out_words.ensure(slots * 4, false, c->stream)) return rc;
    if (int rc = out_counts.ensure(8, true, c->stream)) return rc;
    GenDedupeParams dq;
    fill_dedupe_chunk(c, dq, pc, chunk_first, chunk_n, L, light_length);
    dq.rays = out_rays.as<float4>();
    dq.masks = out_words.as<uint32_t>();
    dq.total = out_counts.as<uint32_t>();
    dq.deposits = out_counts.as<uint32_t>() + 1;
    launch_generate_dedupe(dq, c->stream);
    HIP_TRY(hipGetLastError());
    uint32_t counts[2] = {0u, 0u};
    HIP_TRY(hipMemcpyAsync(counts, dq.total, 8, hipMemcpyDeviceToHost, c->stream));
    HIP_TRY(hipStreamSynchronize(c->stream));
    if ((size_t)counts[0] > slots) return fail(UVRT_ERR_INVALID, "uvrt_dedupe_generate_device: more rays than occurrences");
    if (counts[0] > 0u) {
        HIP_TRY(hipMemcpyAsync(rays, dq.rays, (size_t)counts[0] * 16, hipMemcpyDeviceToHost, c->stream));
        HIP_TRY(hipMemcpyAsync(words, dq.masks, (size_t)counts[0] * 4, hipMemcpyDeviceToHost, c->stream));
        HIP_TRY(hipStreamSynchronize(c->stream));
    }
    *total = counts[0];
    *deposits = counts[1];
    return UVRT_OK;
}

int uvrt_fold_batch(uvrt_ctx* c)
{
    if (!c || c->b_count <= 0) return fail(UVRT_ERR_INVALID, "uvrt_fold_batch: no traced batch");
    if (c->b_is_folded) return UVRT_OK;
    if (int rc = set_device(c)) return rc;
    if (int rc = join_all(c)) return rc;
    launch_fold_planes(c->bs[c->b_set].planes.as<int32_t>(), c->bs[c->b_set].folded.as<int32_t>(), c->b_count, c->b_repl, c->T, c->helper_prio, c->stream);
    if (c->b_ncls > 0) {
        FoldClassParams q;
        memset(&q, 0, sizeof q);
        q.planes = c->bs[c->b_set].planes.as<int32_t>();
        q.folded = c->bs[c->b_set].folded.as<int32_t>();
        q.plane_stride = (int64_t)c->b_repl * c->T;
        q.nplanes = c->b_count;
        q.ncls = c->b_ncls;
        q.cls_replicas = c->b_cls_repl;
        q.T = c->T;
        q.prio = c->helper_prio;
        memcpy(q.launches, c->b_cls_launches, sizeof(uint64_t) * (size_t)c->b_ncls);
        launch_fold_classes(q, c->stream);
    }
    HIP_TRY(hipGetLastError());
    c->b_is_folded = true;
    return UVRT_OK;
}

int uvrt_replay_batch(uvrt_ctx* c, const uvrt_replay_op* ops, int32_t count, int32_t tri_count)
{
    if (!c || !ops || c->b_count <= 0) return fail(UVRT_ERR_INVALID, "uvrt_replay_batch: no traced batch");
    if (count != c->b_count) return fail(UVRT_ERR_INVALID, "uvrt_replay_batch: %d operations for a batch of %d launches", count, c->b_count);
    if (tri_count < 0 || tri_count > c->T) return fail(UVRT_ERR_INVALID, "uvrt_replay_batch: bad tri_count");
    if (int rc = set_device(c)) return rc;
    if (int rc = join_all(c)) return rc;
    ReplayParams p;
    memset(&p, 0, sizeof p);
    p.photon_map = c->photon_map.as<double>();
    p.max_map = c->max_map.as<double>();
    p.planes = c->bs[c->b_set].planes.as<int32_t>();
    p.folded = c->bs[c->b_set].folded.as<int32_t>();
    p.dosage = c->dosage.as<float>();
    p.color = c->color.as<float>();
    p.area = c->area.as<float>();
    p.plane_stride = (int64_t)c->b_repl * c->T;
    p.replicas = c->b_repl;
    p.T = c->T;
    p.bound = tri_count;
    p.count = count;
    p.is_folded = c->b_is_folded ? 1 : 0;
    p.prio = c->helper_prio;
    p.nplanes = c->b_count;
    p.ncls = c->b_ncls;
    p.cls_replicas = c->b_cls_repl;
    for (int k = 0; k < count; ++k)
        for (int cl = 0; cl < c->b_ncls; ++cl)
            if ((c->b_cls_launches[cl] >> c->b_phys[k]) & 1ull) p.class_of[k] |= 1ull << cl;
    for (int k = 0; k < count; ++k) {
        if (ops[k].which_map != UVRT_MAP_SUM && ops[k].which_map != UVRT_MAP_MAX)
            return fail(UVRT_ERR_INVALID, "uvrt_replay_batch: which_map must be 0 or 1");
        p.ops[k].plane = c->b_phys[k];
        p.ops[k].duration = ops[k].duration;
        p.ops[k].shade = ops[k].shade;
        p.ops[k].which_map = ops[k].which_map;
        p.ops[k].photons_per_light = ops[k].photons_per_light;
        p.ops[k].scaled_power = ops[k].scaled_power;
        p.ops[k].min_value = ops[k].min_value;
        p.ops[k].threshold_view = ops[k].threshold_view;
    }
    launch_replay_batch(p, c->stream);
    HIP_TRY(hipGetLastError());
    if (tri_count < c->T) {
        if (c->b_is_folded) HIP_TRY(hipMemsetAsync(c->bs[c->b_set].folded.p, 0, c->bs[c->b_set].folded.bytes, c->stream));
        else HIP_TRY(hipMemsetAsync(c->bs[c->b_set].planes.p, 0, c->bs[c->b_set].planes.bytes, c->stream));
    }
    HIP_TRY(hipEventRecord(c->bs[c->b_set].free_ev, c->stream));
    c->b_count = 0;
    c->b_is_folded = false;
    return mark_map_fence(c);
}

int uvrt_read_batch_counts(uvrt_ctx* c, int32_t launch, int32_t* out, int32_t first, int32_t count)
{
    if (!c || c->b_count <= 0 || launch < 0 || launch >= c->b_count)
        return fail(UVRT_ERR_INVALID, "uvrt_read_batch_counts: no such launch in the traced batch");
    if (int rc = uvrt_fold_batch(c)) return rc;
    if (!range_ok(out, first, count, c->T)) return fail(UVRT_ERR_INVALID, "uvrt_read_batch_counts: bad range");
    return range_copy(c, c->bs[c->b_set].folded.as<int32_t>() + (size_t)c->b_phys[launch] * c->T, 4, out, first, count, hipMemcpyDeviceToHost);
}

}
```

small-project-uv-robot-ray-tracer_amd/csrc/uvrt_ctx.h:

```cpp
#pragma once
#include "../../include/uvrt.h"
#include "uvrt_device.h"
#include "uvrt_batch_plan.h"

#include <cmath>
#include <cstdarg>
#include <cstdio>
#include <cstring>
#include <memory>
#include <string>
#include <vector>

namespace uvrt_impl {

extern thread_local std::string g_err;
int fail(int code, const char* fmt, ...);

#define HIP_TRY(expr)                                                                   \
    do {                                                                                \
        hipError_t e_ = (expr);                                                         \
        if (e_ != hipSuccess)                                                           \
            return ::uvrt_impl::fail(UVRT_ERR_HIP, "%s failed: %s (%s:%d)", #expr,      \
                                     hipGetErrorString(e_), __FILE__, __LINE__);        \
    } while (0)
// ... 16 lines not shown
        if (need == 0) return UVRT_OK;
        HIP_TRY(hipMalloc(&p, need));
        bytes = need;
        if (zero) HIP_TRY(hipMemsetAsync(p, 0, need, s));
        return UVRT_OK;
    }
    void release() { if (p) (void)hipFree(p); p = nullptr; bytes = 0; }
    template <class T> T* as() const { return (T*)p; }
};

struct RecsTag {
    bool valid = false;
    float ox = 0, oz = 0;
    bool matches(float x, float z) const { return valid && memcmp(&ox, &x, 4) == 0 && memcmp(&oz, &z, 4) == 0; }
};

struct Lane {
    hipStream_t side = nullptr;
    hipEvent_t ev_tail = nullptr;
    bool used = false;
    uint64_t seen_fence = 0, seen_mapfence = 0;
    DevBuf rays, recs, counts;
    DevBuf ovf;
    RecsTag recs_tag;
    bool counts_dirty = false;
    DevBuf recs4;
    RecsTag recs4_tag;
    DevBuf hot_hist, hot_list;
    const uint32_t* perm = nullptr;
    DevBuf oxz;
    DevBuf dd_tmp, dd_blocks;
    ~Lane() { if (ev_tail) (void)hipEventDestroy(ev_tail); if (side) (void)hipStreamDestroy(side); }
};

}

using uvrt_impl::DevBuf;
using uvrt_impl::Lane;
using uvrt_impl::RecsTag;

struct uvrt_ctx {
    int device = 0;
    int num_cus = 256;
    hipStream_t own_stream = nullptr;
    hipStream_t stream = nullptr;

    int32_t T = 0;
    DevBuf pairs, perm, ltris, leaf_count, area;
    bool have_perm = false;
    uint64_t perm_clock = 0;
    uint64_t perm_gen = 0;
    int32_t npairs = 0;
    uint32_t root_ref = uvrt::REF_DONE;
    uint32_t top_pairs = 0;
    bool have_scene = false;
    int32_t replicas = 1;
    int32_t replicas_knob = -1;

    DevBuf photon_map, max_map, dosage, color;

    int64_t capacity = 0;
    DevBuf keyrank, sorted, order, hits, hist, bin_start, export_buf;
    bool drain_merge = true;
    bool nearfar_minmax = false;
    bool scene_force_exact = false;
    int32_t hist_bins = 0;
    struct LastRays { int64_t n = -1, first = 0; bool sorted = false, extended = false, free_rays = false; } last;
    float ox = 0, oz = 0;
    DevBuf g_oxz, g_tmax, g_occ, g_w;
    DevBuf g_face;
    DevBuf g_hit;
    DevBuf g_offs, g_scan;
    struct GatherMemo {
        bool valid = false;
        int32_t first = 0, count = 0, samples = 0, mode = 0, photons_equiv = 0;
        uint32_t seed = 0;
        float from[3] = {0, 0, 0}, to[3] = {0, 0, 0}, light_length = 0;
    };
    struct SceneDerived {
        DevBuf free_recs;
        bool free_recs_valid = false;
        DevBuf g_tris;
        bool g_tris_valid = false;
        DevBuf expected, variance;
        DevBuf faces;
        DevBuf g_extra;
        DevBuf source;
        DevBuf links, link_e[2], link_total;
        int32_t links_samples = 0, links_flavour = 0;
        int32_t links_kind = 0;
        uint32_t links_seed = 0;
        GatherMemo gather_memo;
        struct GatherBatch {
            int32_t count = 0, samples = 0, first = 0, tri_count = 0, mode = 0, flavour = 0;
            bool var = false;
            std::vector<uvrt_gather_params> launches;
            DevBuf e, v;
        } gather_batch;
    } derived;
    std::vector<uvrt::GatherBatchLaunch> gb_host;
    DevBuf gb_table;

    static constexpr int MAXL = 4;
    Lane lanes[MAXL];
    bool pipeline = true;
    int nlanes = 2;
    bool ext_touch = false;
    bool ext_touch_maps = false;
    hipEvent_t ev_mapfence = nullptr;
    uint64_t mapfence_seq = 0;
    int lane = 0;
    int prev_lane = 0;
    bool cur_pipelined = false;
    hipEvent_t ev_fence = nullptr;
    uint64_t fence_seq = 0;

    bool wide = false;
    DevBuf quads;
    int32_t nquads = 0;
    uint32_t top_quads = 0;

    static constexpr int HOT_SLAB = 16, HOT_MAX = 64;
    struct HotEntry { float lamp[3]; uint32_t* perm; uint64_t stamp; hipEvent_t ready; uint64_t gen; };
    std::vector<HotEntry> hot;
    std::vector<DevBuf> hot_slabs;
    int32_t hot_sample = 32768;
    int32_t hot_direct = 8192;
    int32_t hot_tail = 16;
    uint64_t hot_clock = 0;
    int32_t hot_mode = 1;

    struct BatchSet { DevBuf rays, planes, folded, oxz, masks, dd_counts; hipEvent_t free_ev = nullptr; ~BatchSet() { if (free_ev) (void)hipEventDestroy(free_ev); } };
    BatchSet bs[2];
    int b_set = 0;
    uint64_t b_chunks = 0;
    int batch_lanes = 2;
    int32_t b_repl = 16;
    std::vector<DevBuf> b_recs;
    struct RecsKey {
        RecsTag tag; const uint32_t* perm = nullptr; uint64_t gen = 0;
        bool holds(float ox, float oz, const uint32_t* pm, uint64_t g) const { return tag.matches(ox, oz) && perm == pm && gen == g; }
    };
    std::vector<RecsKey> b_recs_key;
    int32_t b_count = 0;
    int64_t b_n = 0, b_npad = 0;
    int32_t b_phys[uvrt::MAX_BATCH] = {};
    int helper_prio = 1;
    bool dedupe = true;
    int64_t b_traced_known = -1;
    int32_t dedupe_strip = 0;
    int32_t b_traced_chunks = 0;
    int32_t dedupe_classes = uvrt::DEDUPE_CLASSES_DEFAULT;
    bool dedupe_periodic = uvrt::DEDUPE_PERIODIC_DEFAULT;
    int32_t dedupe_class_replicas = 4;
    size_t dedupe_class_bytes = (size_t)96 << 20;
    int32_t b_ncls = 0, b_cls_repl = 1;
    uint64_t b_cls_launches[uvrt::MAX_CLASS_PLANES] = {};
    bool b_is_folded = false;
    void* comm = nullptr;
    int comm_reserve_knob = 8;
    int lanes_masked_cus = 0;
    int comm_rank = 0, comm_world = 1;

    uint32_t seed = 0;
    int32_t seed_mode = 0;

    int32_t sort_bits = 0;
    bool record_hits = false;
    int32_t variant = 0;
    int32_t flavour = 0;
    int32_t gather_sampling = 0;
    int32_t gather_variance = 0;
    int32_t gather_faces = 0;
#ifdef UVRT_DEV_VARIANTS
    int probe_skip_generate = 0;
    int probe_batches = 0;
#endif
    size_t dedupe_chunk_bytes = (size_t)192 << 20;
    size_t batch_chunk_bytes = (size_t)96 << 20;

    struct PendingAcc { bool valid = false; int lane = 0; float time_step = 0; } pend;
    uint32_t* host_flag = nullptr;
    uint32_t* host_flag_dev = nullptr;
    DevBuf error_flag;
    hipStream_t probe_stream = nullptr;
    DevBuf probe_out;
    bool timing = false;
    std::vector<hipEvent_t> ev_pool;
    size_t ev_used = 0;

    struct PlanState* plan = nullptr;

    ~uvrt_ctx();
};

namespace uvrt_impl {
using namespace uvrt;

inline hipStream_t stream_of(uvrt_ctx* c, int l) { return l == 0 ? c->stream : c->lanes[l].side; }
inline Lane& cur_lane(uvrt_ctx* c) { return c->lanes[c->lane]; }
inline size_t side_ovf_bytes(const uvrt_ctx* c) { return (size_t)c->num_cus * 8 * 256 * 24 * sizeof(uint32_t); }

inline int set_device_only(uvrt_ctx* c)
{
    HIP_TRY(hipSetDevice(c->device));
    return UVRT_OK;
}
inline int flush_pending(uvrt_ctx* c)
{
    if (!c->pend.valid) return UVRT_OK;
    c->pend.valid = false;
    const int l = c->pend.lane;
    launch_accumulate(c->photon_map.as<double>(), c->max_map.as<double>(), c->lanes[l].counts.as<int32_t>(),
                      c->replicas, c->T, c->pend.time_step, c->T, c->helper_prio, stream_of(c, l));
    HIP_TRY(hipGetLastError());
    return UVRT_OK;
}
inline int set_device(uvrt_ctx* c)
{
    HIP_TRY(hipSetDevice(c->device));
    return flush_pending(c);
}
inline int join_all(uvrt_ctx* c)
{
    for (int l = 1; l < uvrt_ctx::MAXL; ++l) {
        Lane& L = c->lanes[l];
        if (!L.used) continue;
        HIP_TRY(hipEventRecord(L.ev_tail, L.side));
        HIP_TRY(hipStreamWaitEvent(c->stream, L.ev_tail, 0));
        L.used = false;
    }
    return UVRT_OK;
}
inline int mark_fence(uvrt_ctx* c)
{
    HIP_TRY(hipEventRecord(c->ev_fence, c->stream));
    ++c->fence_seq;
    return UVRT_OK;
}
inline int mark_map_fence(uvrt_ctx* c)
{
    HIP_TRY(hipEventRecord(c->ev_mapfence, c->stream));
    ++c->mapfence_seq;
    return UVRT_OK;
}
inline int lane_stream(uvrt_ctx* c, hipStream_t* out, bool maps = false)
{
    if (c->ext_touch) { c->ext_touch = false; if (int rc = mark_fence(c)) return rc; }
    if (c->ext_touch_maps) { c->ext_touch_maps = false; if (int rc = mark_map_fence(c)) return rc; }
    if (c->lane == 0) { *out = stream_of(c, 0); return UVRT_OK; }
    Lane& L = cur_lane(c);
    if (c->fence_seq != L.seen_fence) {
        HIP_TRY(hipStreamWaitEvent(L.side, c->ev_fence, 0));
        L.seen_fence = c->fence_seq;
    }
    if (maps && c->mapfence_seq != L.seen_mapfence) {
        HIP_TRY(hipStreamWaitEvent(L.side, c->ev_mapfence, 0));
        L.seen_mapfence = c->mapfence_seq;
    }
    L.used = true;
    *out = L.side;
    return UVRT_OK;
}
inline int order_after_previous(uvrt_ctx* c)
{
    const int l = c->lane, q = c->prev_lane;
    if (q == l) return UVRT_OK;
    if (l == 0) return join_all(c);
    HIP_TRY(hipEventRecord(c->lanes[q].ev_tail, stream_of(c, q)));
    HIP_TRY(hipStreamWaitEvent(c->lanes[l].side, c->lanes[q].ev_tail, 0));
    c->lanes[l].used = true;
    return UVRT_OK;
}
inline int next_launch_lane(uvrt_ctx* c, bool may_pipeline)
{
    const bool pipe_ok = may_pipeline && c->pipeline && c->nlanes > 1 && !c->record_hits && c->lanes[1].rays.p;
    c->prev_lane = c->lane;
    c->cur_pipelined = pipe_ok;
    if (pipe_ok) c->lane = (c->lane + 1) % c->nlanes;
    else { if (int rc = join_all(c)) return rc; c->lane = 0; }
    return c->lane == 0 ? UVRT_OK : cur_lane(c).ovf.ensure(side_ovf_bytes(c), false, c->stream);
}
inline int lane_cus(const uvrt_ctx* c) { return c->lane == 0 ? c->num_cus : c->num_cus - c->lanes_masked_cus; }

inline int copy_sync(uvrt_ctx* c, void* dst, const void* src, size_t bytes, hipMemcpyKind kind)
{
    if (bytes == 0) return UVRT_OK;
    HIP_TRY(hipMemcpyAsync(dst, src, bytes, kind, c->stream));
    HIP_TRY(hipStreamSynchronize(c->stream));
    return UVRT_OK;
}
inline bool range_ok(const void* host, int64_t first, int64_t count, int64_t limit)
{
    return host && first >= 0 && count >= 0 && first + count <= limit;
}
inline int range_copy(uvrt_ctx* c, void* base, size_t elem, void* host, int64_t first, int64_t count, hipMemcpyKind kind)
{
    if (int rc = set_device(c)) return rc;
    if (int rc = join_all(c)) return rc;
    char* dev = (char*)base + (size_t)first * elem;
    return kind == hipMemcpyDeviceToHost ? copy_sync(c, host, dev, (size_t)count * elem, kind)
                                         : copy_sync(c, dev, host, (size_t)count * elem, kind);
}

struct HostRay { float d[3], o[3], dist; uint32_t tri; };
inline void unpack_rays(const HostRay* hr, int64_t n, std::vector<float>& packed, std::vector<float>* oxz = nullptr,
// ... 180 lines not shown
```

small-project-uv-robot-ray-tracer_amd/csrc/uvrt_dedupe.h:

```cpp
#pragma once
#include <stdint.h>
#include <algorithm>

#if defined(__HIPCC__)
#define UVRT_HD __host__ __device__ __forceinline__
#else
#define UVRT_HD inline
#endif

namespace uvrt {

constexpr int MAX_BATCH = 64;
constexpr int MAX_CLASS_PLANES = 64;

constexpr int DEDUPE_MAX = 31;
constexpr int64_t DEDUPE_GID_END = 126322567;

UVRT_HD float seed_sum_of(int threadID, uint32_t SEED, float lx, float ly, float lz)
{
    float acc = (float)(int)((uint32_t)threadID * 17u + 1u);
    acc = acc + lx * 13.0f;
    acc = acc + ly * 7.0f;
    acc = acc + lz * 11.0f;
    acc = acc + (float)(SEED >> 15);
// ... 425 lines not shown
}
UVRT_HD uint32_t dedupe_periodic_owners(const DedupeGroup& G, const DedupePeriodic& T, const uint32_t* words, int k, int32_t x0, int32_t x1)
{
    if (x0 >= x1) return 0u;
    const uint32_t seed1 = dedupe_seed1(G, k);
    const int32_t ka = dedupe_key1_of(G, seed1, x0), kb = dedupe_key1_of(G, seed1, x1 - 1);
    uint32_t total = 0u;
    for (int s = 0; s < T.count; ++s) {
        const int64_t A = T.key_lo[s], B = A + (int64_t)T.keys[s];
        if ((int64_t)kb < A || (int64_t)ka >= B) continue;
        const int32_t a = (int64_t)ka >= A ? x0 : dedupe_lower_bound(G, k, A, x0, x1);
        const int32_t b = (int64_t)kb < B ? x1 : dedupe_lower_bound(G, k, B, a, x1);
        const int32_t P = T.period[s], n = b - a, q = n / P, rest = n & (P - 1);
        for (int32_t r = 0; r < P; ++r)
            if (words[dedupe_periodic_index(T, s, k, a + r)] != 0u) total += (uint32_t)(q + (r < rest));
    }
    return total;
}

inline int dedupe_periodic_gaps(const DedupePeriodic& T, int64_t key_lo, int64_t keys, int32_t W, int32_t strip, int32_t* gap_key,
                                uint32_t* gap_keys, int32_t* strip0)
{
    int n = 0;
    int64_t cur = key_lo, strips = 0;
    const int64_t end = key_lo + keys;
    const auto gap = [&](int64_t a, int64_t b) {
        gap_key[n] = (int32_t)a;
        gap_keys[n] = (uint32_t)(b - a);
        strip0[n++] = (int32_t)strips;
        strips += ((b - a + W - 1) / W + strip - 1) / strip;
    };
    for (int s = 0; s < T.count && cur < end; ++s) {
        const int64_t A = T.key_lo[s], B = A + (int64_t)T.keys[s];
        if (B <= cur || A >= end) continue;
        if (A > cur) gap(cur, A);
        cur = B;
    }
    if (cur < end) gap(cur, end);
    strip0[n] = (int32_t)strips;
    return n;
}

inline bool dedupe_periodic_tile(const DedupeGroup& G, int64_t t0, int32_t P, uint32_t* table, uint32_t* out)
{
    const int32_t W = 68 * P;
    int32_t g_lo[DEDUPE_MAX], g_hi[DEDUPE_MAX];
    if (dedupe_tile_fill(G, t0, W, nullptr, table, g_lo, g_hi)) return false;
    for (int32_t i = 0; i < W; ++i)
        if (table[i] & DEDUPE_MANY) return false;
    for (int k = 0; k < G.count; ++k) {
        if (g_hi[k] - g_lo[k] < P) return false;
        for (int32_t g = g_lo[k]; g < g_hi[k]; ++g) {
            const uint32_t mask = dedupe_tile_resolve(table[dedupe_tile_slot(dedupe_key1(G, k, g), t0)], k);
            uint32_t& e = out[k * P + (g & (P - 1))];
            if (g - g_lo[k] < P) e = mask;
            else if (e != mask) return false;
        }
    }
    return true;
}

inline void dedupe_periodic_build(const DedupeGroup& G, const DedupeClasses& C, uint32_t* table, DedupePeriodic& T)
{
    static_assert(DEDUPE_PERIODIC_TILE <= DEDUPE_TILE_KEYS, "the build tile fits the host's table");
    T = DedupePeriodic{};
    const int K = G.count;
    const int64_t last = G.first_gid + G.n - 1, lo1 = G.first_gid > 1 ? G.first_gid : 1;
    if (K > DEDUPE_PERIODIC_LAUNCHES || lo1 > last) return;
    const double lamp = 13.0 * (double)(G.lx < 0 ? -G.lx : G.lx) + 7.0 * (double)(G.ly < 0 ? -G.ly : G.ly) + 11.0 * (double)(G.lz < 0 ? -G.lz : G.lz);
    if (!(lamp < 1e6)) return;
    const int64_t L = (int64_t)lamp + 1, E = 32, M = L + E + 34 * DEDUPE_PERIOD_MAX;
    constexpr int BINADES = 27;
    int64_t cut[3 * DEDUPE_MAX + BINADES * (DEDUPE_MAX + 1) + 2];
    int64_t klo, khi, smax = 0;
    dedupe_key_span(G, lo1, last, klo, khi);
    for (int j = 0; j < K; ++j) smax = std::max(smax, (int64_t)(dedupe_seed1(G, j) >> 15));
    const int64_t floor_key = smax + L + E + 1;
    klo = klo < floor_key ? floor_key : klo;
    khi = khi > ((int64_t)1 << 27) ? ((int64_t)1 << 27) : khi;
    if (khi - klo < 2 * M) return;
    const int ncut = dedupe_cuts(G, lo1, last, 0, BINADES - 1, true, klo, khi, cut);
    struct Cand { int64_t a, b; int32_t P; };
    Cand cand[DEDUPE_PERIODIC_STRATA + 1];
    int nc = 0, words = 0;
    for (int i = 0; i + 1 < ncut; ++i) {
        const int64_t a = (cut[i] < klo ? klo : cut[i]) + M, b = (cut[i + 1] > khi ? khi : cut[i + 1]) - M;
        if (b - a < 4 * (int64_t)DEDUPE_PERIODIC_TILE) continue;
        int64_t ulp = 1;
        while (((int64_t)1 << 24) * ulp < b + M) ulp += ulp;
        const Cand v = {a, b, (int32_t)(2 * ulp)};
        if (v.P > DEDUPE_PERIOD_MAX) continue;
        int at = nc;
        for (; at > 0 && cand[at - 1].b - cand[at - 1].a < b - a; --at) cand[at] = cand[at - 1];
        cand[at] = v;
        if (nc < DEDUPE_PERIODIC_STRATA) ++nc;
    }
    int take = 0;
    for (; take < nc && words + K * cand[take].P <= DEDUPE_PERIODIC_WORDS; ++take) words += K * cand[take].P;
    for (int i = 1; i < take; ++i) {
        const Cand v = cand[i];
        int at = i;
        for (; at > 0 && cand[at - 1].a > v.a; --at) cand[at] = cand[at - 1];
        cand[at] = v;
    }
    uint32_t first[DEDUPE_PERIODIC_LAUNCHES * DEDUPE_PERIOD_MAX], second[DEDUPE_PERIODIC_LAUNCHES * DEDUPE_PERIOD_MAX];
    int32_t off = 0;
    for (int i = 0; i < take; ++i) {
        const Cand& v = cand[i];
        const int32_t P = v.P;
        if (!dedupe_periodic_tile(G, v.a, P, table, first) || !dedupe_periodic_tile(G, v.b - 68 * P, P, table, second)) continue;
        bool same = true;
        for (int e = 0; e < K * P; ++e) same = same && first[e] == second[e];
        if (!same) continue;
        const int s = T.count++;
        T.key_lo[s] = (int32_t)v.a;
        T.keys[s] = (uint32_t)(v.b - v.a);
        T.period[s] = P;
        T.word_off[s] = off;
        for (int e = 0; e < K * P; ++e)
            T.words[off + e] = first[e] == 0u ? 0u : dedupe_deposit_word(C.count > 0, C.slot_mask, C.slot_word, first[e]);
        off += K * P;
    }
}

inline int64_t dedupe_plan_periodic(const DedupeGroup& G, const DedupePeriodic& T, int32_t W, int32_t strip, int32_t block, int64_t c0,
                                    int64_t cn, uint32_t* table, uint32_t* masks, uint32_t* counts)
{
    const int64_t nb = (cn + block - 1) / block;
    for (int64_t i = 0; i < (int64_t)G.count * cn; ++i) masks[i] = 0u;
    int64_t key_lo, tiles;
    dedupe_tile_range(G, c0, cn, W, key_lo, tiles);
    int32_t gap_key[DEDUPE_PERIODIC_STRATA + 1], strip0[DEDUPE_PERIODIC_STRATA + 2];
    uint32_t gap_keys[DEDUPE_PERIODIC_STRATA + 1];
    const int gaps = dedupe_periodic_gaps(T, key_lo, tiles * W, W, strip, gap_key, gap_keys, strip0);
    for (int i = 0; i < gaps; ++i) dedupe_plan_tiled_keys(G, W, strip, c0, cn, gap_key[i], gap_keys[i], table, masks);
    int64_t from_table = 0;
    for (int k = 0; k < G.count; ++k) {
        for (int64_t b = 0; b < nb; ++b) {
            const int64_t x0 = c0 + b * block, x1 = x0 + block < c0 + cn ? x0 + block : c0 + cn;
            uint32_t owners = 0u;
            for (int64_t g = x0; g < x1; ++g) owners += masks[(int64_t)k * cn + (g - c0)] != 0u;
            counts[(int64_t)k * nb + b] = owners + dedupe_periodic_owners(G, T, T.words, k, (int32_t)(x0 > 1 ? x0 : 1), (int32_t)x1);
        }
        for (int64_t g = c0 > 1 ? c0 : 1; g < c0 + cn; ++g) {
            const int s = dedupe_periodic_find(T, dedupe_key1(G, k, (int32_t)g));
            if (s < 0) continue;
            masks[(int64_t)k * cn + (g - c0)] = T.words[dedupe_periodic_index(T, s, k, (int32_t)g)];
            ++from_table;
        }
    }
    return from_table;
}

}
```

small-project-uv-robot-ray-tracer_amd/csrc/uvrt_device.h:

```cpp
#pragma once
#include <hip/hip_runtime.h>
#include <stdint.h>
#include "uvrt_dedupe.h"

namespace uvrt {

constexpr uint32_t REF_LEAF_BIT = 0x80000000u;
constexpr uint32_t REF_DONE = 0xFFFFFFFFu;
constexpr uint32_t REF_FIRST_MASK = 0x07FFFFFFu;
constexpr int REF_COUNT_SHIFT = 27;
constexpr int MAX_TRIS = 1 << 27;

struct alignas(16) PairRec {
    float4 c0min_ref0;
    float4 c0max_ref1;
    float4 c1min;
    float4 c1max;
};

struct alignas(16) LeafTri {
    float4 v0_id;
    float4 e1;
    float4 e2;
};

struct alignas(16) QuadRec {
    float4 xz[4];
    float4 y01, y23;
    uint32_t ref[4];
    uint32_t pad[4];
};

struct SceneDev {
    const PairRec* pairs;
    const LeafTri* ltris;
    const uint32_t* leaf_count;
    uint32_t root_ref;
    int32_t tri_count;
};

__device__ __forceinline__ void ascending(float& lo, float& hi)
{
    if (hi < lo) { const float t = lo; lo = hi; hi = t; }
}
__device__ __forceinline__ void prepare_record6(const PairRec* __restrict__ pairs, float4* __restrict__ recs,
                                                float ox, float oz, int32_t npairs, int src,
                                                const uint32_t* __restrict__ perm)
{
    const PairRec pr = pairs[src];
    uint32_t r0 = __float_as_uint(pr.c0min_ref0.w), r1 = __float_as_uint(pr.c0max_ref1.w);
    if (r0 >= REF_LEAF_BIT) r0 += (uint32_t)npairs; else if (perm) r0 = perm[r0];
    if (r1 >= REF_LEAF_BIT) r1 += (uint32_t)npairs; else if (perm) r1 = perm[r1];
    const int i = perm ? (int)perm[src] : src;
    float4 w0 = make_float4(pr.c0min_ref0.x - ox, pr.c0max_ref1.x - ox, pr.c0min_ref0.z - oz, pr.c0max_ref1.z - oz);
    float4 w1 = make_float4(pr.c1min.x - ox, pr.c1max.x - ox, pr.c1min.z - oz, pr.c1max.z - oz);
    float4 w2 = make_float4(pr.c0min_ref0.y, pr.c0max_ref1.y, pr.c1min.y, pr.c1max.y);
    ascending(w0.x, w0.y); ascending(w0.z, w0.w);
    ascending(w1.x, w1.y); ascending(w1.z, w1.w);
    ascending(w2.x, w2.y); ascending(w2.z, w2.w);
    recs[i * 4 + 0] = w0;
    recs[i * 4 + 1] = w1;
    recs[i * 4 + 2] = w2;
    recs[i * 4 + 3] = make_float4(__uint_as_float(r0), __uint_as_float(r1), 0.f, 0.f);
}

__device__ __forceinline__ void helper_priority(int prio)
{
    switch (prio) {
        case 1: __builtin_amdgcn_s_setprio(1); break;
        case 2: __builtin_amdgcn_s_setprio(2); break;
        case 3: __builtin_amdgcn_s_setprio(3); break;
        default: break;
    }
}


__device__ __forceinline__ uint32_t wang_hash(uint32_t s)
{
    s = (s ^ 61u) ^ (s >> 16);
    s *= 9u;
    s = s ^ (s >> 4);
    s *= 0x27d4eb2du;
    s = s ^ (s >> 15);
    return s;
}

__device__ __forceinline__ float random_float(uint32_t& s)
{
    s ^= s << 13;
    s ^= s >> 17;
    s ^= s << 5;
    return (float)s * 2.3283064365387e-10f;
}

__device__ __forceinline__ float4 generate_ray_rng(float lx, float ly, float lz, float light_length, int64_t gid,
                                                   uint32_t seed_prev, uint32_t seed_next, int32_t seed_mode,
                                                   float& r0, double& x, double& y, uint32_t& seed)
{
    seed = wang_hash(seed_input(gid, lx, ly, lz, seed_prev, seed_next, seed_mode));

    r0 = random_float(seed);
    const float origy = ly + r0 * light_length;
    const float diry = random_float(seed) * 2.0f - 1.0f;
    const double dirxzlength = sqrt(1.0 - (double)diry * (double)diry);

    x = (double)(random_float(seed) * 2.0f - 1.0f);
    y = (double)(random_float(seed) * 2.0f - 1.0f);
    while (x * x + y * y > 1.0) {
        x = (double)(random_float(seed) * 2.0f - 1.0f);
        y = (double)(random_float(seed) * 2.0f - 1.0f);
    }
    const double s = dirxzlength / sqrt(x * x + y * y);
    return make_float4((float)(x * s), diry, (float)(y * s), origy);
}
__device__ __forceinline__ float4 generate_ray(float lx, float ly, float lz, float light_length, int64_t gid,
                                               uint32_t seed_prev, uint32_t seed_next, int32_t seed_mode,
                                               float& r0, double& x, double& y)
{
    uint32_t seed;
    return generate_ray_rng(lx, ly, lz, light_length, gid, seed_prev, seed_next, seed_mode, r0, x, y, seed);
}

constexpr uint32_t TOP6_MAX = 175;

struct GenBatchParams {
    float4* rays;
    int64_t n_pad;
    int64_t first_gid, n;
    float light_length;
    int32_t seed_mode;
    int32_t count;
    float lx[MAX_BATCH], ly[MAX_BATCH], lz[MAX_BATCH];
    uint32_t seed_prev[MAX_BATCH], seed_next[MAX_BATCH];
    int32_t prio;
};

constexpr int DD_ROUNDS = 8, DD_SLOTS = 256 * DD_ROUNDS;
struct GenDedupeParams {
    DedupeGroup g;
    float4* rays;
    uint32_t* masks;
    uint32_t* total;
    uint32_t* tmp;
    uint32_t* block_counts;
    int64_t g0, gn;
    int64_t key_lo, tiles;
    int32_t strip_tiles;
    float light_length;
    int32_t prio;
    uint32_t* deposits;
    DedupeClasses cls;
    DedupePeriodic per;
    int32_t gaps;
    int32_t gap_key[DEDUPE_PERIODIC_STRATA + 1];
    uint32_t gap_keys[DEDUPE_PERIODIC_STRATA + 1];
    int32_t gap_strip0[DEDUPE_PERIODIC_STRATA + 2];
};
static_assert(sizeof(GenDedupeParams) <= 3584, "kernel arguments: 4 KB with the hidden ones");
void launch_generate_dedupe(const GenDedupeParams& p, hipStream_t s);
void launch_dedupe_mark(const GenDedupeParams& p, hipStream_t s);
struct ExtendParams;
bool launch_extend6_dedupe(const ExtendParams& p, int code, int grid_per_cu, hipStream_t s);

struct ReplayOp {
    int32_t plane;
    float duration;
    int32_t shade;
    int32_t which_map;
    int32_t photons_per_light;
    float scaled_power, min_value;
    int32_t threshold_view;
};

struct ReplayParams {
    double* photon_map;
    double* max_map;
    int32_t* planes;
    int32_t* folded;
    float* dosage;
    float* color;
    const float* area;
    int64_t plane_stride;
    int32_t replicas, T, count, is_folded;
    int32_t prio;
    int32_t bound;
    int32_t nplanes, ncls, cls_replicas;
    uint64_t class_of[MAX_BATCH];
    ReplayOp ops[MAX_BATCH];
};

struct FoldClassParams {
    int32_t* planes;
    int32_t* folded;
    int64_t plane_stride;
    int32_t nplanes, ncls, cls_replicas, T, prio;
    uint64_t launches[MAX_CLASS_PLANES];
};
void launch_fold_classes(const FoldClassParams& p, hipStream_t s);

struct GenParams {
    float4* rays;
    uint2* keyrank;
    uint32_t* hist;
    float lx, ly, lz;
    float light_length;
    int64_t first_gid;
    int64_t n;
    uint32_t seed_prev;
    uint32_t seed_next;
    int32_t seed_mode;
    int32_t bits_phi, bits_y, bits_o;
    const PairRec* prep_pairs;
    float4* prep_recs;
    const uint32_t* prep_perm;
    int32_t prep_npairs;
    uint32_t ray_blocks;
    int32_t prio;
};

struct ExtendParams {
    SceneDev scene;
    const float4* rays;
    uint32_t chunk;
    int32_t cls_replicas;
    uint32_t* ovf_stack;
    uint64_t ovf_capacity;
    int32_t num_cus;
    uint32_t top_pairs;
    int32_t force_exact;
    int32_t drain_merge;
    int32_t nearfar_minmax;
    int32_t flavour;
    const uint32_t* order;
    uint2* hits;
    int32_t* counts;
    int32_t count_replicas;
    int64_t count_stride;
    uint32_t* error_flag;
    float ox, oz;
    int64_t n;
    int32_t npairs;
    void* recs;
    int32_t refill_min;
    const uint32_t* perm;
    int32_t recs_prepared;
    uint32_t root_ref6;
    uint32_t plane_batches;
    uint32_t plane_n;
    uint32_t plane_stride;
    float plane_inv;
    const void* recs4;
    int32_t nquads;
    uint32_t top_quads;
    uint32_t root_ref4;
    const uint32_t* masks;
    const uint32_t* n_dev;
};

void launch_generate(const GenParams& p, hipStream_t s);
void launch_generate_batch(const GenBatchParams& p, hipStream_t s);
void launch_fold_planes(int32_t* planes, int32_t* folded, int32_t nplanes, int32_t replicas, int32_t T, int prio, hipStream_t s);
void launch_replay_batch(const ReplayParams& p, hipStream_t s);
void launch_add_counts(int32_t* dst, const int32_t* src, int64_t n, hipStream_t s);
void launch_prepare_launch6(const PairRec* pairs, void* recs, float ox, float oz, int32_t npairs, const uint32_t* perm,
                            int prio, hipStream_t s);
void launch_scan_bins(uint32_t* hist, uint32_t* bin_start, int32_t nbins, hipStream_t s);
void launch_scatter(const float4* rays, const uint2* keyrank, const uint32_t* bin_start,
                    float4* sorted, uint32_t* order, int64_t n, hipStream_t s);
bool launch_extend6(const ExtendParams& p, int code, int grid_per_cu, int prep_prio, hipStream_t s);
bool launch_extend4(const ExtendParams& p, int grid_per_cu, hipStream_t s);
void launch_prepare_launch4(const QuadRec* quads, void* recs4, float ox, float oz, int32_t nquads, hipStream_t s);
constexpr int HS_GROUPS = 16;
struct HotSetupParams {
    const PairRec* pairs;
    const LeafTri* ltris;
    const uint32_t* leaf_count;
    uint32_t root_ref;
    float light_length;
    int32_t seed_mode;
    int32_t n;
    int32_t npairs, keep, count;
    int32_t tail_lanes;
    int32_t direct_bins;
    uint32_t* hist;
    uint32_t* hot_list;
    uint32_t* perm[HS_GROUPS];
    float lx[HS_GROUPS], ly[HS_GROUPS], lz[HS_GROUPS];
    uint32_t seed_prev[HS_GROUPS], seed_next[HS_GROUPS];
};
void launch_hot_setup(const HotSetupParams& p, hipStream_t s);
void launch_prepare_leaves6(const LeafTri* ltris, void* recs, int32_t npairs, int32_t T, hipStream_t s);
constexpr uint64_t OVF_MAX_ENTRIES = (uint64_t)256 * 16 * 256 * 24;
void launch_accumulate(double* photon_map, double* max_map, int32_t* counts, int32_t replicas,
                       int64_t stride, float time_step, int32_t T, int prio, hipStream_t s);
void launch_reset(double* photon_map, double* max_map, int32_t* counts, int32_t replicas,
                  int64_t stride, float* color, int32_t reset_color, int32_t T, int prio, hipStream_t s);
void launch_fold_counts(int32_t* counts, int32_t replicas, int64_t stride, int32_t T, hipStream_t s);
void launch_compute_dosage(const double* map, float* dosage, const float* area,
                           int32_t photons_per_light, float scaled_power, int32_t T,
                           hipStream_t s);
void launch_shade(const double* map, float* dosage, const float* area, float* color, int32_t photons_per_light,
                  float scaled_power, float min_value, int32_t threshold_view, int32_t T, int prio, hipStream_t s);
void launch_accumulate_shade(double* photon_map, double* max_map, int32_t* counts, int32_t replicas, int64_t stride,
                             float time_step, float* dosage, const float* area, float* color, int32_t which_map,
                             int32_t photons_per_light, float scaled_power, float min_value, int32_t threshold_view,
                             int32_t T, int prio, hipStream_t s);
void launch_dosage_to_color(const float* dosage, float* color, float min_value,
                            int32_t threshold_view, int32_t T, hipStream_t s);
void launch_prepare_scene(const float4* tris64, const uint32_t* tri_idx, LeafTri* ltris,
                          float* area, int32_t T, hipStream_t s);
void launch_clock_probe(unsigned long long* out2, unsigned long long ticks_100mhz, hipStream_t s);
void launch_export_rays(const float4* rays, const uint2* hits, void* out32, float ox, float oz,
// ... 169 lines not shown
```

small-project-uv-robot-ray-tracer_amd/csrc/uvrt_kernels.hip:

```cpp
#include "uvrt_device.h"

namespace uvrt {


__device__ __forceinline__ uint32_t coherence_key(uint32_t qphi, uint32_t qy, uint32_t qo,
                                                  int bphi, int by, int bo)
{
    uint32_t key = 0;
    while (bphi > 0 || by > 0 || bo > 0) {
        if (bphi > 0) { --bphi; key = (key << 1) | ((qphi >> bphi) & 1u); }
        if (by > 0) { --by; key = (key << 1) | ((qy >> by) & 1u); }
        if (bo > 0) { --bo; key = (key << 1) | ((qo >> bo) & 1u); }
    }
    return key;
}

__global__ __launch_bounds__(256) void k_generate(GenParams p)
{
    helper_priority(p.prio);
    if (blockIdx.x >= p.ray_blocks) {
        const int j = (int)(blockIdx.x - p.ray_blocks) * 256 + threadIdx.x;
        if (j < p.prep_npairs) prepare_record6(p.prep_pairs, p.prep_recs, p.lx, p.lz, p.prep_npairs, j, p.prep_perm);
        return;
    }
// ... 54 lines not shown
            const uint32_t owners = dedupe_periodic_owners(p.g, p.per, s_table, (int)k, max(x0, 1), x1);
            if (owners != 0u) atomicAdd(&p.block_counts[t], owners);
        }
        return;
    }
    int gap = 0;
    while (gap + 1 < p.gaps && (int32_t)blockIdx.x >= p.gap_strip0[gap + 1]) ++gap;
    const int64_t gap_lo = p.gap_key[gap];
    const uint32_t gap_keys = p.gap_keys[gap];
    const int64_t gap_tiles = (int64_t)((gap_keys + (uint32_t)W - 1u) / (uint32_t)W);
    const int64_t tile0 = (int64_t)((int32_t)blockIdx.x - p.gap_strip0[gap]) * p.strip_tiles;
    const int64_t tile1 = tile0 + p.strip_tiles < gap_tiles ? tile0 + p.strip_tiles : gap_tiles;
    int32_t run_lo = hi, run_hi = hi, key0 = 0;
    uint32_t seed1 = 0u;
    if (lane < K) {
        run_lo = dedupe_strip_first(p.g, lane, gap_lo + tile0 * W);
        seed1 = dedupe_seed1(p.g, lane);
        key0 = p.g.key0[lane];
    }
    uint32_t cnt_block = 0u, cnt = 0u;
    const auto add_owners = [&](int j, uint32_t block, uint32_t owners) { atomicAdd(&p.block_counts[(size_t)j * nb + block], owners); };
    const auto count_owners = [&](int j, uint32_t block, uint32_t owners) {
        if (lane == j && owners != 0u) {
            if (block != cnt_block) {
                if (cnt != 0u) add_owners(j, cnt_block, cnt);
                cnt_block = block;
                cnt = 0u;
            }
            cnt += owners;
        }
    };
    for (int64_t tile = tile0; tile < tile1; ++tile) {
        const int64_t t0 = gap_lo + tile * W;
        const int32_t w = (int32_t)min((uint32_t)W, gap_keys - (uint32_t)(tile * W));
        static_assert(W % 64 == 0, "the wave zeroes the table in whole rounds");
#pragma unroll
        for (int i = 0; i < W; i += 64) s_table[i + lane] = 0u;
        __syncthreads();
        for (int j = 0; j < K; ++j) {
            int32_t base = __builtin_amdgcn_readlane(run_lo, j);
            const uint32_t seed = (uint32_t)__builtin_amdgcn_readlane((int)seed1, j);
            for (;;) {
                const int32_t g = base + lane;
                bool in = false;
                if (g < hi) {
                    const int32_t key = dedupe_key1_of(p.g, seed, g);
                    in = dedupe_in_tile(key, t0, w);
                    if (in) dedupe_tile_insert_run(s_table, dedupe_tile_slot(key, t0), j, dedupe_run_twice(p.g, seed, g, key, lo, hi));
                }
                const int32_t n_in = (int32_t)__popcll(__builtin_amdgcn_ballot_w64(in));
                base += n_in;
                if (n_in < 64) break;
            }
            if (lane == j) run_hi = base;
        }
        const bool holds0 = lane < K && dedupe_tile_holds_key0(p.g, key0, t0, w);
        if (holds0) dedupe_tile_insert(s_table, dedupe_tile_slot(key0, t0), lane);
        __syncthreads();
        for (int j = 0; j < K; ++j) {
            const int32_t a = max(__builtin_amdgcn_readlane(run_lo, j), c0), b = min(__builtin_amdgcn_readlane(run_hi, j), c1);
            const uint32_t seed = (uint32_t)__builtin_amdgcn_readlane((int)seed1, j);
            for (int32_t base = a; base < b; base += 64) {
                const int32_t g = base + lane;
                const uint32_t fb = (uint32_t)(base - c0) / (uint32_t)DD_SLOTS;
                uint32_t mask = 0u, blk = fb;
                if (g < b) {
                    const uint32_t slot = dedupe_tile_slot(dedupe_key1_of(p.g, seed, g), t0);
                    mask = dedupe_tile_resolve(slot < (uint32_t)w ? s_table[slot] : DEDUPE_MANY, j);
                    p.tmp[(int64_t)j * p.gn + (g - c0)] = mask;
                    blk = (uint32_t)(g - c0) / (uint32_t)DD_SLOTS;
                }
                const int32_t last = min(base + 63, b - 1);
                if ((uint32_t)(last - c0) / (uint32_t)DD_SLOTS == fb) {
                    count_owners(j, fb, (uint32_t)__popcll(__builtin_amdgcn_ballot_w64(mask != 0u)));
                } else {
                    const uint32_t n0 = (uint32_t)__popcll(__builtin_amdgcn_ballot_w64(mask != 0u && blk == fb));
                    const uint32_t n1 = (uint32_t)__popcll(__builtin_amdgcn_ballot_w64(mask != 0u && blk != fb));
                    count_owners(j, fb, n0);
                    count_owners(j, fb + 1u, n1);
                }
            }
        }
        if (c0 == 0 && holds0) {
            const uint32_t mask = dedupe_tile_resolve(s_table[dedupe_tile_slot(key0, t0)], lane);
            p.tmp[(int64_t)lane * p.gn] = mask;
            if (mask != 0u) add_owners(lane, 0u, 1u);
        }
        run_lo = run_hi;
        __syncthreads();
    }
    if (lane < K && cnt != 0u) add_owners(lane, cnt_block, cnt);
}

__global__ __launch_bounds__(256) void k_dedupe_scan(uint32_t* block_counts, uint32_t* total, uint32_t* deposits, uint32_t nblocks, int prio)
{
    helper_priority(prio);
    __shared__ uint32_t s_part[256];
    const uint32_t tid = threadIdx.x;
    if (tid == 0u) *deposits = 0u;
    const uint32_t per = (nblocks + 255u) / 256u;
    const uint32_t lo = min(tid * per, nblocks), hi = min(lo + per, nblocks);
    uint32_t sum = 0;
    for (uint32_t b = lo; b < hi; ++b) sum += block_counts[b];
    s_part[tid] = sum;
    __syncthreads();
    for (uint32_t off = 1; off < 256u; off <<= 1) {
        const uint32_t v = tid >= off ? s_part[tid - off] : 0u;
        __syncthreads();
        s_part[tid] += v;
        __syncthreads();
    }
    uint32_t run = s_part[tid] - sum;
    for (uint32_t b = lo; b < hi; ++b) {
        const uint32_t c = block_counts[b];
        block_counts[b] = run;
        run += c;
    }
    if (tid == 255u) *total = s_part[255];
}

__global__ __launch_bounds__(256) void k_dedupe_write(GenDedupeParams p)
{
    helper_priority(p.prio);
    __shared__ uint32_t s_cnt[DD_ROUNDS][4];
    __shared__ uint32_t s_slot_mask[DEDUPE_CLASS_SLOTS], s_slot_word[DEDUPE_CLASS_SLOTS], s_dep;
    if (threadIdx.x < (unsigned)DEDUPE_CLASS_SLOTS) {
        s_slot_mask[threadIdx.x] = p.cls.slot_mask[threadIdx.x];
        s_slot_word[threadIdx.x] = p.cls.slot_word[threadIdx.x];
    }
    if (threadIdx.x == 0) s_dep = 0u;
    const bool classes = p.cls.count > 0;
    uint32_t dep = 0u;
    const int k = blockIdx.y;
    const uint32_t wv = threadIdx.x >> 6;
    static_assert(256 % DEDUPE_PERIOD_MAX == 0, "a thread's rounds share their residue");
    uint32_t near = 0u, worded = 0u;
    bool inside = false;
    const uint32_t seed1 = dedupe_seed1(p.g, k);
    const int32_t gid0 = (int32_t)(p.g0 + (int64_t)blockIdx.x * DD_SLOTS) + (int32_t)threadIdx.x;
    if (p.per.count > 0) {
        const int32_t x0 = max((int32_t)(p.g0 + (int64_t)blockIdx.x * DD_SLOTS), 1);
        const int32_t x1 = (int32_t)min(p.g0 + ((int64_t)blockIdx.x + 1) * DD_SLOTS, p.g0 + p.gn);
        const int32_t ka = __builtin_amdgcn_readfirstlane(dedupe_key1_of(p.g, seed1, x0));
        const int32_t kb = __builtin_amdgcn_readfirstlane(dedupe_key1_of(p.g, seed1, x1 - 1));
#pragma unroll
        for (int s = 0; s < DEDUPE_PERIODIC_STRATA; ++s) {
            const int32_t A = p.per.key_lo[s], B = A + (int32_t)p.per.keys[s];
            if (s < p.per.count && kb >= A && ka < B) {
                near |= 1u << s;
                inside = ka >= A && kb < B;
            }
        }
    }
    uint32_t mask[DD_ROUNDS], rank[DD_ROUNDS];
#pragma unroll
    for (int r = 0; r < DD_ROUNDS; ++r) mask[r] = 0u;
    for (uint32_t left = near; left != 0u; left &= left - 1u) {
        const int s = __builtin_ctz(left);
        const int32_t A = p.per.key_lo[s], P = p.per.period[s];
        const uint32_t len = p.per.keys[s];
        const uint32_t* w = &p.per.words[p.per.word_off[s] + k * P];
        const int32_t res = gid0 & (P - 1);
        uint32_t word = 0u;
#pragma unroll
        for (int q = 0; q < DEDUPE_PERIOD_MAX; ++q) {
            const uint32_t wq = w[q];
            if (res == q) word = wq;
        }
#pragma unroll
        for (int r = 0; r < DD_ROUNDS; ++r) {
            const int64_t i = (int64_t)blockIdx.x * DD_SLOTS + r * 256 + threadIdx.x;
            const int32_t g = gid0 + r * 256;
            if (i < p.gn && g >= 1 && (inside || (uint32_t)dedupe_key1_of(p.g, seed1, g) - (uint32_t)A < len)) {
                mask[r] = word;
                worded |= 1u << r;
            }
        }
    }
    uint32_t pos = p.block_counts[(size_t)k * gridDim.x + blockIdx.x];
#pragma unroll
    for (int r = 0; r < DD_ROUNDS; ++r) {
        const int64_t i = (int64_t)blockIdx.x * DD_SLOTS + r * 256 + threadIdx.x;
        if (!((worded >> r) & 1u) && i < p.gn) mask[r] = p.tmp[(int64_t)k * p.gn + i];
        const unsigned long long owners = __builtin_amdgcn_ballot_w64(mask[r] != 0u);
        rank[r] = __builtin_amdgcn_mbcnt_hi((uint32_t)(owners >> 32), __builtin_amdgcn_mbcnt_lo((uint32_t)owners, 0u));
        if ((threadIdx.x & 63u) == 0u) s_cnt[r][wv] = (uint32_t)__popcll(owners);
    }
    __syncthreads();
    if (threadIdx.x == 0) p.block_counts[(size_t)k * gridDim.x + blockIdx.x] = 0u;
#pragma unroll
    for (int r = 0; r < DD_ROUNDS; ++r) {
        for (uint32_t w = 0; w < 4u; ++w) {
            if (w == wv && mask[r] != 0u) {
                const int64_t i = (int64_t)blockIdx.x * DD_SLOTS + r * 256 + threadIdx.x;
                float r0;
                double x, y;
                p.rays[pos + rank[r]] = generate_ray(p.g.lx, p.g.ly, p.g.lz, p.light_length, p.g0 + i, p.g.seed_prev[k],
                                                     p.g.seed_next[k], p.g.seed_mode, r0, x, y);
                const uint32_t word = ((worded >> r) & 1u) ? mask[r] : dedupe_deposit_word(classes, s_slot_mask, s_slot_word, mask[r]);
                p.masks[pos + rank[r]] = word;
                dep += (uint32_t)dedupe_word_deposits(classes, word);
            }
            pos += s_cnt[r][w];
        }
    }
    if (dep != 0u) atomicAdd(&s_dep, dep);
    __syncthreads();
    if (threadIdx.x == 0 && s_dep != 0u) atomicAdd(p.deposits, s_dep);
}

__global__ __launch_bounds__(1024) void k_scan_bins(uint32_t* hist, uint32_t* bin_start,
                                                    int32_t nbins)
{
    __shared__ uint32_t s_part[1024];
    const int tid = threadIdx.x;
    const int per = (nbins + 1023) / 1024;
    const int lo = tid * per, hi = min(lo + per, nbins);
    uint32_t sum = 0;
    for (int b = lo; b < hi; ++b) sum += hist[b];
    s_part[tid] = sum;
    __syncthreads();
    for (int off = 1; off < 1024; off <<= 1) {
        uint32_t v = tid >= off ? s_part[tid - off] : 0u;
        __syncthreads();
        s_part[tid] += v;
        __syncthreads();
    }
    uint32_t run = s_part[tid] - sum;
    for (int b = lo; b < hi; ++b) {
        const uint32_t c = hist[b];
        bin_start[b] = run;
        hist[b] = 0;
        run += c;
    }
}

__global__ __launch_bounds__(256) void k_scatter(const float4* __restrict__ rays,
                                                 const uint2* __restrict__ keyrank,
                                                 const uint32_t* __restrict__ bin_start,
                                                 float4* __restrict__ sorted,
                                                 uint32_t* __restrict__ order, int64_t n)
{
    const int64_t i = (int64_t)blockIdx.x * 256 + threadIdx.x;
    if (i >= n) return;
    const uint2 kr = keyrank[i];
    const uint32_t pos = bin_start[kr.x] + kr.y;
    const float4 r = rays[i];
    sorted[pos] = r;
    order[pos] = (uint32_t)i;
}


__global__ __launch_bounds__(256) void k_accumulate(double* __restrict__ photon_map,
                                                    double* __restrict__ max_map,
                                                    int32_t* __restrict__ counts, int32_t replicas,
                                                    int64_t stride, float time_step, int32_t T, int prio)
{
    helper_priority(prio);
    const int g = blockIdx.x * 256 + threadIdx.x;
    const int i = g >> 2, part = g & 3;
    int32_t total = 0;
    if (i < T) {
        for (int r = part; r < replicas; r += 4) {
            total += counts[r * stride + i];
            counts[r * stride + i] = 0;
        }
    }
    total += __builtin_amdgcn_mov_dpp(total, 0xb1, 0xf, 0xf, true);
    total += __builtin_amdgcn_mov_dpp(total, 0x4e, 0xf, 0xf, true);
    if (i >= T || part != 0) return;
    const double c = (double)total;
    photon_map[i] = photon_map[i] + c * (double)time_step;
    const double m = max_map[i];
    max_map[i] = m < c ? c : m;
}

__global__ __launch_bounds__(256) void k_fold_counts(int32_t* __restrict__ counts, int32_t replicas,
                                                     int64_t stride, int32_t T)
{
    const int i = blockIdx.x * 256 + threadIdx.x;
    if (i >= T) return;
    int32_t total = counts[i];
    for (int r = 1; r < replicas; ++r) {
        total += counts[r * stride + i];
        counts[r * stride + i] = 0;
    }
    counts[i] = total;
}

__device__ __forceinline__ void heatmap(float intensity, float& r, float& g, float& b)
{
    const float minDosageColor = 0.5f;
    const float upperHalfColor = 0.75f;
    const float lowerHalfColor = 0.25f;
    if (intensity > minDosageColor) {
        if (intensity > upperHalfColor) {
            r = 1.0f; g = (1.0f - intensity) / (1.0f - upperHalfColor); b = 0.0f;
        } else {
            r = (intensity - minDosageColor) / (upperHalfColor - minDosageColor);
            g = 1.0f; b = 0.0f;
        }
    } else {
        if (intensity > lowerHalfColor) {
            r = 0.0f; g = 1.0f;
            b = (minDosageColor - intensity) / (minDosageColor - lowerHalfColor);
        } else {
            r = 0.0f; g = intensity / lowerHalfColor; b = 1.0f;
        }
    }
}

__global__ __launch_bounds__(256) void k_fold_planes(int32_t* __restrict__ planes, int32_t* __restrict__ folded,
                                                     int32_t replicas, int32_t T, int prio)
{
    helper_priority(prio);
    const int g = blockIdx.x * 256 + threadIdx.x;
    const int i = g >> 2, part = g & 3;
    int32_t* pl = planes + (int64_t)blockIdx.y * replicas * T;
    int32_t total = 0;
    if (i < T) {
        for (int r = part; r < replicas; r += 4) {
            total += pl[(int64_t)r * T + i];
            pl[(int64_t)r * T + i] = 0;
        }
    }
    total += __builtin_amdgcn_mov_dpp(total, 0xb1, 0xf, 0xf, true);
    total += __builtin_amdgcn_mov_dpp(total, 0x4e, 0xf, 0xf, true);
    if (i < T && part == 0) folded[(int64_t)blockIdx.y * T + i] = total;
}

__device__ __forceinline__ int32_t take_class_plane(int32_t* pl, int32_t replicas, int64_t replica_stride, int i, int part, bool in)
{
    int32_t total = 0;
    if (in) {
        for (int r = part; r < replicas; r += 4) {
            total += pl[(int64_t)r * replica_stride + i];
            pl[(int64_t)r * replica_stride + i] = 0;
        }
    }
    total += __builtin_amdgcn_mov_dpp(total, 0xb1, 0xf, 0xf, true);
    total += __builtin_amdgcn_mov_dpp(total, 0x4e, 0xf, 0xf, true);
    return total;
}

__global__ __launch_bounds__(256) void k_fold_classes(FoldClassParams p)
{
    helper_priority(p.prio);
    const int g = blockIdx.x * 256 + threadIdx.x;
    const int i = g >> 2, part = g & 3;
    const bool in = i < p.T;
    for (int c = 0; c < p.ncls; ++c) {
        const int32_t total = take_class_plane(p.planes + (int64_t)(p.nplanes + c) * p.plane_stride, p.cls_replicas, p.T, i, part, in);
        if (!in || part != 0 || total == 0) continue;
        for (uint64_t m = p.launches[c]; m != 0ull; m &= m - 1ull) p.folded[(int64_t)__builtin_ctzll(m) * p.T + i] += total;
    }
}

__global__ __launch_bounds__(256) void k_replay_batch(ReplayParams p)
{
    helper_priority(p.prio);
    const int g = blockIdx.x * 256 + threadIdx.x;
// ... 110 lines not shown
                                                        float scaled_power, int32_t T)
{
    const int i = blockIdx.x * 256 + threadIdx.x;
    if (i >= T) return;
    const double num = (double)scaled_power * map[i];
    const float den = area[i] * (float)photons_per_light;
    dosage[i] = (float)(num / (double)den);
}

__global__ __launch_bounds__(256) void k_dosage_to_color(const float* __restrict__ dosage,
                                                         float* __restrict__ color,
                                                         float min_value, int32_t threshold_view,
                                                         int32_t T)
{
    const int i = blockIdx.x * 256 + threadIdx.x;
    if (i >= T) return;
    const float maxValue = min_value * 2;
    const float norm = dosage[i] / maxValue;
    float r, g, b;
    if (threshold_view && norm < 0.5f) { r = 0.0f; g = 0.0f; b = norm * 2.0f; }
    else heatmap(norm, r, g, b);
    float* c = color + (int64_t)i * 9;
    c[0] = r; c[1] = g; c[2] = b;
    c[3] = r; c[4] = g; c[5] = b;
    c[6] = r; c[7] = g; c[8] = b;
}

__device__ __forceinline__ void shade_one(int i, double map_value, float* __restrict__ dosage, const float* __restrict__ area,
                                          float* __restrict__ color, int32_t photons_per_light, float scaled_power,
                                          float min_value, int32_t threshold_view)
{
    const double num = (double)scaled_power * map_value;
    const float den = area[i] * (float)photons_per_light;
    const float dose = (float)(num / (double)den);
    dosage[i] = dose;
    const float maxValue = min_value * 2;
    const float norm = dose / maxValue;
    float r, g, b;
    if (threshold_view && norm < 0.5f) { r = 0.0f; g = 0.0f; b = norm * 2.0f; }
    else heatmap(norm, r, g, b);
    float* c = color + (int64_t)i * 9;
    c[0] = r; c[1] = g; c[2] = b;
    c[3] = r; c[4] = g; c[5] = b;
    c[6] = r; c[7] = g; c[8] = b;
}

__global__ __launch_bounds__(256) void k_shade(const double* __restrict__ map, float* __restrict__ dosage,
                                               const float* __restrict__ area, float* __restrict__ color,
                                               int32_t photons_per_light, float scaled_power,
                                               float min_value, int32_t threshold_view, int32_t T, int prio)
{
    helper_priority(prio);
    const int i = blockIdx.x * 256 + threadIdx.x;
    if (i >= T) return;
    shade_one(i, map[i], dosage, area, color, photons_per_light, scaled_power, min_value, threshold_view);
}

__global__ __launch_bounds__(256) void k_accumulate_shade(double* __restrict__ photon_map, double* __restrict__ max_map,
                                                          int32_t* __restrict__ counts, int32_t replicas, int64_t stride,
                                                          float time_step, float* __restrict__ dosage,
                                                          const float* __restrict__ area, float* __restrict__ color,
                                                          int32_t which_map, int32_t photons_per_light, float scaled_power,
                                                          float min_value, int32_t threshold_view, int32_t T, int prio)
{
    helper_priority(prio);
    const int g = blockIdx.x * 256 + threadIdx.x;
    const int i = g >> 2, part = g & 3;
    int32_t total = 0;
    if (i < T) {
        for (int r = part; r < replicas; r += 4) {
            total += counts[r * stride + i];
            counts[r * stride + i] = 0;
        }
    }
    total += __builtin_amdgcn_mov_dpp(total, 0xb1, 0xf, 0xf, true);
    total += __builtin_amdgcn_mov_dpp(total, 0x4e, 0xf, 0xf, true);
    if (i >= T || part != 0) return;
    const double c = (double)total;
    const double sum = photon_map[i] + c * (double)time_step;
    photon_map[i] = sum;
    const double m = max_map[i];
    const double mx = m < c ? c : m;
    max_map[i] = mx;
    shade_one(i, which_map ? mx : sum, dosage, area, color, photons_per_light, scaled_power, min_value, threshold_view);
}

__global__ __launch_bounds__(64) void k_clock_probe(unsigned long long* out, unsigned long long ticks)
{
    const unsigned long long r0 = __builtin_amdgcn_s_memrealtime();
    const unsigned long long t0 = __builtin_amdgcn_s_memtime();
    unsigned long long r1 = r0;
    while (r1 - r0 < ticks) {
        __builtin_amdgcn_s_sleep(32);
        r1 = __builtin_amdgcn_s_memrealtime();
    }
    const unsigned long long t1 = __builtin_amdgcn_s_memtime();
    r1 = __builtin_amdgcn_s_memrealtime();
    if (threadIdx.x == 0) { out[0] = t1 - t0; out[1] = r1 - r0; }
}

void launch_clock_probe(unsigned long long* out, unsigned long long ticks, hipStream_t s)
{
    hipLaunchKernelGGL(k_clock_probe, dim3(1), dim3(64), 0, s, out, ticks);
}

__global__ __launch_bounds__(256) void k_export_rays(const float4* __restrict__ rays,
                                                     const uint2* __restrict__ hits,
                                                     float4* __restrict__ out, float ox,
                                                     float oz, int64_t first, int64_t count)
{
    const int64_t i = (int64_t)blockIdx.x * 256 + threadIdx.x;
    if (i >= count) return;
    const float4 rec = rays[first + i];
    uint2 h = make_uint2(__float_as_uint(1e30f), 0u);
    if (hits) h = hits[first + i];
    out[i * 2 + 0] = make_float4(rec.x, rec.y, rec.z, ox);
    out[i * 2 + 1] = make_float4(rec.w, oz, __uint_as_float(h.x), __uint_as_float(h.y));
}


static inline unsigned blocks_for(int64_t n, int per) { return (unsigned)((n + per - 1) / per); }

void launch_generate(const GenParams& p0, hipStream_t s)
{
    GenParams p = p0;
    p.ray_blocks = p.n > 0 ? blocks_for(p.n, 256) : 0u;
    const unsigned prep_blocks = p.prep_recs ? blocks_for(p.prep_npairs, 256) : 0u;
    if (p.ray_blocks + prep_blocks == 0) return;
    hipLaunchKernelGGL(k_generate, dim3(p.ray_blocks + prep_blocks), dim3(256), 0, s, p);
}

void launch_generate_batch(const GenBatchParams& p, hipStream_t s)
{
    if (p.n <= 0 || p.count <= 0) return;
    hipLaunchKernelGGL(k_generate_batch, dim3(blocks_for(p.n, 256), (unsigned)p.count), dim3(256), 0, s, p);
}

void launch_dedupe_mark(const GenDedupeParams& p, hipStream_t s)
{
    if (p.gn <= 0 || p.g.count <= 0 || (p.gaps <= 0 && p.per.count <= 0) || p.strip_tiles <= 0) return;
    const unsigned count_groups = p.per.count > 0 ? blocks_for((int64_t)p.g.count * blocks_for(p.gn, DD_SLOTS), 64) : 0u;
    hipLaunchKernelGGL(k_dedupe_mark, dim3((unsigned)p.gap_strip0[p.gaps] + count_groups), dim3(64), 0, s, p);
}

void launch_generate_dedupe(const GenDedupeParams& p, hipStream_t s)
{
    if (p.gn <= 0 || p.g.count <= 0) return;
    const dim3 grid(blocks_for(p.gn, DD_SLOTS), (unsigned)p.g.count);
    launch_dedupe_mark(p, s);
    hipLaunchKernelGGL(k_dedupe_scan, dim3(1), dim3(256), 0, s, p.block_counts, p.total, p.deposits, grid.x * grid.y, (int)p.prio);
    hipLaunchKernelGGL(k_dedupe_write, grid, dim3(256), 0, s, p);
}

void launch_fold_planes(int32_t* planes, int32_t* folded, int32_t nplanes, int32_t replicas, int32_t T, int prio, hipStream_t s)
{
    if (nplanes <= 0 || T <= 0) return;
    hipLaunchKernelGGL(k_fold_planes, dim3(blocks_for((int64_t)T * 4, 256), (unsigned)nplanes), dim3(256), 0, s, planes,
                       folded, replicas, T, prio);
}

void launch_replay_batch(const ReplayParams& p, hipStream_t s)
{
    if (p.count <= 0 || p.bound <= 0) return;
    const size_t lds = p.is_folded ? 0 : (size_t)p.ncls * 64 * sizeof(int32_t);
    hipLaunchKernelGGL(k_replay_batch, dim3(blocks_for((int64_t)p.bound * 4, 256)), dim3(256), lds, s, p);
}

void launch_fold_classes(const FoldClassParams& p, hipStream_t s)
{
    if (p.ncls <= 0 || p.T <= 0) return;
    hipLaunchKernelGGL(k_fold_classes, dim3(blocks_for((int64_t)p.T * 4, 256)), dim3(256), 0, s, p);
}

void launch_add_counts(int32_t* dst, const int32_t* src, int64_t n, hipStream_t s)
{
    if (n <= 0) return;
    hipLaunchKernelGGL(k_add_counts, dim3(blocks_for(n, 256)), dim3(256), 0, s, dst, src, n);
}

void launch_scan_bins(uint32_t* hist, uint32_t* bin_start, int32_t nbins, hipStream_t s)
{
    hipLaunchKernelGGL(k_scan_bins, dim3(1), dim3(1024), 0, s, hist, bin_start, nbins);
}

void launch_scatter(const float4* rays, const uint2* keyrank, const uint32_t* bin_start,
                    float4* sorted, uint32_t* order, int64_t n, hipStream_t s)
{
    if (n <= 0) return;
    hipLaunchKernelGGL(k_scatter, dim3(blocks_for(n, 256)), dim3(256), 0, s, rays, keyrank,
                       bin_start, sorted, order, n);
}

void launch_accumulate(double* photon_map, double* max_map, int32_t* counts, int32_t replicas,
                       int64_t stride, float time_step, int32_t T, int prio, hipStream_t s)
{
    if (T <= 0) return;
    hipLaunchKernelGGL(k_accumulate, dim3(blocks_for((int64_t)T * 4, 256)), dim3(256), 0, s, photon_map,
                       max_map, counts, replicas, stride, time_step, T, prio);
}

void launch_fold_counts(int32_t* counts, int32_t replicas, int64_t stride, int32_t T, hipStream_t s)
{
    if (T <= 0 || replicas <= 1) return;
    hipLaunchKernelGGL(k_fold_counts, dim3(blocks_for(T, 256)), dim3(256), 0, s, counts, replicas,
                       stride, T);
}

void launch_reset(double* photon_map, double* max_map, int32_t* counts, int32_t replicas,
                  int64_t stride, float* color, int32_t reset_color, int32_t T, int prio, hipStream_t s)
{
    if (T <= 0) return;
    hipLaunchKernelGGL(k_reset, dim3(blocks_for(T, 256)), dim3(256), 0, s, photon_map, max_map,
                       counts, replicas, stride, color, reset_color, T, prio);
}

void launch_compute_dosage(const double* map, float* dosage, const float* area,
                           int32_t photons_per_light, float scaled_power, int32_t T,
                           hipStream_t s)
{
    if (T <= 0) return;
    hipLaunchKernelGGL(k_compute_dosage, dim3(blocks_for(T, 256)), dim3(256), 0, s, map, dosage,
                       area, photons_per_light, scaled_power, T);
}

void launch_shade(const double* map, float* dosage, const float* area, float* color, int32_t photons_per_light,
                  float scaled_power, float min_value, int32_t threshold_view, int32_t T, int prio, hipStream_t s)
{
    if (T <= 0) return;
    hipLaunchKernelGGL(k_shade, dim3(blocks_for(T, 256)), dim3(256), 0, s, map, dosage, area, color,
                       photons_per_light, scaled_power, min_value, threshold_view, T, prio);
}

void launch_accumulate_shade(double* photon_map, double* max_map, int32_t* counts, int32_t replicas, int64_t stride,
                             float time_step, float* dosage, const float* area, float* color, int32_t which_map,
                             int32_t photons_per_light, float scaled_power, float min_value, int32_t threshold_view,
                             int32_t T, int prio, hipStream_t s)
{
    if (T <= 0) return;
    hipLaunchKernelGGL(k_accumulate_shade, dim3(blocks_for((int64_t)T * 4, 256)), dim3(256), 0, s, photon_map, max_map, counts,
                       replicas, stride, time_step, dosage, area, color, which_map, photons_per_light, scaled_power, min_value,
                       threshold_view, T, prio);
}

void launch_dosage_to_color(const float* dosage, float* color, float min_value,
                            int32_t threshold_view, int32_t T, hipStream_t s)
{
    if (T <= 0) return;
    hipLaunchKernelGGL(k_dosage_to_color, dim3(blocks_for(T, 256)), dim3(256), 0, s, dosage,
                       color, min_value, threshold_view, T);
}

void launch_prepare_scene(const float4* tris64, const uint32_t* tri_idx, LeafTri* ltris,
                          float* area, int32_t T, hipStream_t s)
{
    if (T <= 0) return;
    hipLaunchKernelGGL(k_prepare_scene, dim3(blocks_for(T, 256)), dim3(256), 0, s, tris64,
                       tri_idx, ltris, area, T);
}

void launch_export_rays(const float4* rays, const uint2* hits, void* out32, float ox, float oz,
                        int64_t first, int64_t count, hipStream_t s)
{
    if (count <= 0) return;
    hipLaunchKernelGGL(k_export_rays, dim3(blocks_for(count, 256)), dim3(256), 0, s, rays, hits,
                       (float4*)out32, ox, oz, first, count);
}

}
```

Baseline: 17370 Mray/s.

## Add precomputed per-key ray direction table to dedupe write kernel

Adds an optional device table that maps a seed key to a precomputed ray direction and the r0 fraction, built once by a new kernel. The dedupe write kernel then loads rays from it instead of hashing and running the rejection-sampled direction generation. The write loop is also restructured to compute slot positions from wave-uniform counts rather than looping over all four waves. The table is off by default (budget 0 MB), so only the loop restructuring runs unless UVRT_RAY_TABLE_MB is set.

```diff
diff --git a/include/uvrt.h b/include/uvrt.h
--- a/include/uvrt.h
+++ b/include/uvrt.h
@@ -208,6 +208,15 @@
 int uvrt_dedupe_generate_device(uvrt_ctx* ctx, const float lamp[3], float light_length, int32_t count, const uint32_t* seed_prev,
                                 const uint32_t* seed_next, int32_t seed_mode, int64_t first_gid, int64_t n, int64_t chunk_first,
                                 int64_t chunk_n, float* rays, uint32_t* words, uint32_t* total, uint32_t* deposits);
+int uvrt_set_ray_table(uvrt_ctx* ctx, int32_t max_mb);
+int uvrt_set_ray_table_bytes(uvrt_ctx* ctx, uint64_t max_bytes);
+int uvrt_get_ray_table(uvrt_ctx* ctx, uint64_t* budget_bytes, uint32_t* entries, uint32_t* keys);
+int uvrt_ray_table_build(uvrt_ctx* ctx, uint32_t max_key);
+int uvrt_ray_table_read(uvrt_ctx* ctx, uint32_t first, uint32_t count, float* out);
+uint32_t uvrt_ray_table_index(uint32_t key);
+uint32_t uvrt_ray_table_key(uint32_t index);
+uint32_t uvrt_ray_table_entries(uint32_t max_key);
+uint32_t uvrt_ray_table_fit(uint32_t max_key, uint64_t budget_bytes);
 
 int uvrt_comm_available(void);
 int uvrt_comm_unique_id(void* id128);
diff --git a/small-project-uv-robot-ray-tracer_amd/capi.py b/small-project-uv-robot-ray-tracer_amd/capi.py
--- a/small-project-uv-robot-ray-tracer_amd/capi.py
+++ b/small-project-uv-robot-ray-tracer_amd/capi.py
@@ -63,6 +63,15 @@
     ("uvrt_dedupe_plan_periodic", C.c_int, [_fp, _i32, _vp, _vp, _i32, _i64, _i64, _i64, _i64, _vp, _vp, C.POINTER(_i64)]),
     ("uvrt_dedupe_generate_device", C.c_int, [_vp, _fp, C.c_float, _i32, _vp, _vp, _i32, _i64, _i64, _i64, _i64, _vp, _vp,
                                               C.POINTER(C.c_uint32), C.POINTER(C.c_uint32)]),
+    ("uvrt_set_ray_table", C.c_int, [_vp, _i32]),
+    ("uvrt_set_ray_table_bytes", C.c_int, [_vp, C.c_uint64]),
+    ("uvrt_get_ray_table", C.c_int, [_vp, C.POINTER(C.c_uint64), C.POINTER(_u32), C.POINTER(_u32)]),
+    ("uvrt_ray_table_build", C.c_int, [_vp, _u32]),
+    ("uvrt_ray_table_read", C.c_int, [_vp, _u32, _u32, _vp]),
+    ("uvrt_ray_table_index", _u32, [_u32]),
+    ("uvrt_ray_table_key", _u32, [_u32]),
+    ("uvrt_ray_table_entries", _u32, [_u32]),
+    ("uvrt_ray_table_fit", _u32, [_u32, C.c_uint64]),
     ("uvrt_comm_available", C.c_int, []),
     ("uvrt_comm_info", C.c_int, [_vp, C.POINTER(_i32)]),
     ("uvrt_comm_unique_id", C.c_int, [_vp]),
@@ -278,6 +287,22 @@
     return int(lib().uvrt_seed_input(int(gid), _f3(lamp), int(seed_prev), int(seed_next_), int(seed_mode)))
 
 
+def ray_table_index(key):
+    return int(lib().uvrt_ray_table_index(int(key)))
+
+
+def ray_table_key(index):
+    return int(lib().uvrt_ray_table_key(int(index)))
+
+
+def ray_table_entries(max_key):
+    return int(lib().uvrt_ray_table_entries(int(max_key)))
+
+
+def ray_table_fit(max_key, budget_bytes):
+    return int(lib().uvrt_ray_table_fit(int(max_key), int(budget_bytes)))
+
+
 def dedupe_plan(lamp, seed_prev, seed_next_, seed_mode, first_gid, n):
     sp = np.ascontiguousarray(seed_prev, dtype=np.uint32)
     sn = np.ascontiguousarray(seed_next_, dtype=np.uint32)
@@ -747,6 +772,25 @@
         on = _i32()
         self._ck(self._L.uvrt_get_dedupe_periodic(self._h, C.byref(on)))
         return bool(on.value)
+
+    def set_ray_table(self, max_mb=None, max_bytes=None):
+        if max_bytes is not None:
+            self._ck(self._L.uvrt_set_ray_table_bytes(self._h, int(max_bytes)))
+        else:
+            self._ck(self._L.uvrt_set_ray_table(self._h, int(max_mb)))
+
+    def get_ray_table(self):
+        budget, entries, keys = C.c_uint64(), _u32(), _u32()
+        self._ck(self._L.uvrt_get_ray_table(self._h, C.byref(budget), C.byref(entries), C.byref(keys)))
+        return int(budget.value), int(entries.value), int(keys.value)
+
+    def ray_table_build(self, max_key):
+        self._ck(self._L.uvrt_ray_table_build(self._h, int(max_key)))
+
+    def ray_table_read(self, first, count):
+        out = np.empty((int(count), 4), dtype=np.float32)
+        self._ck(self._L.uvrt_ray_table_read(self._h, int(first), int(count), _ptr(out)))
+        return out
 
     def dedupe_generate_device(self, lamp, light_length, seed_prev, seed_next_, seed_mode, first_gid, n, chunk_first=None,
                                chunk_n=None):
diff --git a/small-project-uv-robot-ray-tracer_amd/csrc/uvrt_capi.hip b/small-project-uv-robot-ray-tracer_amd/csrc/uvrt_capi.hip
--- a/small-project-uv-robot-ray-tracer_amd/csrc/uvrt_capi.hip
+++ b/small-project-uv-robot-ray-tracer_amd/csrc/uvrt_capi.hip
@@ -28,7 +28,7 @@
 {
     plan_drop(this);
     (void)hot_reset(this, false);
-    for (hipEvent_t e : {ev_fence, ev_mapfence}) if (e) (void)hipEventDestroy(e);
+    for (hipEvent_t e : {ev_fence, ev_mapfence, ray_table_ev}) if (e) (void)hipEventDestroy(e);
     for (hipEvent_t e : ev_pool) (void)hipEventDestroy(e);
     if (host_flag) (void)hipHostFree(host_flag);
     if (probe_stream) (void)hipStreamDestroy(probe_stream);
@@ -223,6 +223,7 @@
     env_bool("UVRT_DEDUPE", c->dedupe);
     env_int("UVRT_DEDUPE_CLASSES", 0, DEDUPE_CLASS_MAX, c->dedupe_classes);
     env_bool("UVRT_DEDUPE_PERIODIC", c->dedupe_periodic);
+    if (long mb = 0; env_int("UVRT_RAY_TABLE_MB", 0, 1 << 20, mb)) c->ray_table_budget = (uint64_t)mb << 20;
     env_int("UVRT_DEDUPE_STRIP", 1, 1024, c->dedupe_strip);
     env_int("UVRT_DEDUPE_CLASS_REPLICAS", 1, 16, c->dedupe_class_replicas);
     if (long mb = 0; env_int("UVRT_DEDUPE_CLASS_MB", 1, 4096, mb)) c->dedupe_class_bytes = (size_t)mb << 20;
diff --git a/small-project-uv-robot-ray-tracer_amd/csrc/uvrt_capi_batch.hip b/small-project-uv-robot-ray-tracer_amd/csrc/uvrt_capi_batch.hip
--- a/small-project-uv-robot-ray-tracer_amd/csrc/uvrt_capi_batch.hip
+++ b/small-project-uv-robot-ray-tracer_amd/csrc/uvrt_capi_batch.hip
@@ -18,6 +18,8 @@
     kn.dedupe_chunk_bytes = c->dedupe_chunk_bytes; kn.batch_chunk_bytes = c->batch_chunk_bytes; kn.dedupe_strip = c->dedupe_strip;
     return kn;
 }
+
+struct RayTableUse { uint32_t entries, build; };
 
 struct BatchRun {
     uvrt_ctx* c;
@@ -33,7 +35,58 @@
     int per_cu;
     int64_t traced;
     size_t dd_used;
+    RayTableUse table;
 };
+
+static uint32_t ray_table_want(const uvrt_ctx* c, const std::vector<Piece>& pieces)
+{
+    uint32_t want = 0;
+    if (c->ray_table_budget == 0) return 0;
+    for (const Piece& pc : pieces) {
+        const int64_t kmax = pc.dd ? dedupe_max_key(pc.G) : -1;
+        if (kmax >= 0) want = std::max(want, ray_table_fit((uint32_t)kmax, c->ray_table_budget));
+    }
+    return want;
+}
+static void ray_table_grow(uvrt_ctx* c, uint32_t want)
+{
+    c->ray_table.release();
+    c->ray_table_entries = 0;
+    void* p = nullptr;
+    if (hipMalloc(&p, (size_t)want * 16) != hipSuccess) { (void)hipGetLastError(); return; }
+    c->ray_table.p = p;
+    c->ray_table.bytes = (size_t)want * 16;
+}
+static RayTableUse ray_table_use(const uvrt_ctx* c, uint32_t want)
+{
+    RayTableUse u = {};
+    if (want == 0 || !c->ray_table.p) return u;
+    if (want > c->ray_table_entries && c->ray_table.bytes >= (size_t)want * 16) u.build = want;
+    u.entries = u.build ? u.build : c->ray_table_entries;
+    return u;
+}
+static int ray_table_order(uvrt_ctx* c, RayTableUse& u, int lane, hipStream_t s)
+{
+    if (u.entries == 0) return UVRT_OK;
+    if (u.build != 0) {
+        if (!c->ray_table_ev) HIP_TRY(hipEventCreateWithFlags(&c->ray_table_ev, hipEventDisableTiming));
+        launch_ray_table_build(c->ray_table.as<float4>(), u.build, s);
+        HIP_TRY(hipGetLastError());
+        HIP_TRY(hipEventRecord(c->ray_table_ev, s));
+        c->ray_table_entries = u.build;
+        c->ray_table_seen[lane] = ++c->ray_table_gen;
+        u.build = 0;
+    } else if (c->ray_table_seen[lane] != c->ray_table_gen) {
+        HIP_TRY(hipStreamWaitEvent(s, c->ray_table_ev, 0));
+        c->ray_table_seen[lane] = c->ray_table_gen;
+    }
+    return UVRT_OK;
+}
+static void set_ray_table(const uvrt_ctx* c, const RayTableUse& u, GenDedupeParams& dq)
+{
+    dq.ray_table = u.entries ? c->ray_table.as<float4>() : nullptr;
+    dq.ray_table_keys = u.entries ? ray_table_key(u.entries) : 0u;
+}
 
 static int provision_records(BatchRun& r, bool* recs_stale)
 {
@@ -80,11 +133,14 @@
     bool dd_scratch_short = false;
     for (int l = 0; l <= c->batch_lanes; ++l)
         dd_scratch_short = dd_scratch_short || c->lanes[l].dd_tmp.bytes < P.dd_tmp_bytes || c->lanes[l].dd_blocks.bytes < P.dd_block_bytes;
-    const bool need_alloc = S.rays.bytes < (size_t)count * (size_t)n_pad * 16 || S.planes.bytes < planes_bytes ||
+    bool need_alloc = S.rays.bytes < (size_t)count * (size_t)n_pad * 16 || S.planes.bytes < planes_bytes ||
                             S.folded.bytes < (size_t)count * (size_t)c->T * 4 || (int)c->b_recs.size() < P.ngroups || !S.free_ev ||
                             S.oxz.bytes < (size_t)P.nsweeps * (size_t)n_pad * 8 || (P.nsweeps > 0 && !c->derived.free_recs_valid) ||
                             (P.dd_chunks > 0 && (S.masks.bytes < (size_t)count * (size_t)n_pad * 4 || S.dd_counts.bytes < P.dd_chunks * 8 ||
                                                  dd_scratch_short));
+    const uint32_t table_want = ray_table_want(c, P.pieces);
+    const bool table_short = table_want > c->ray_table_entries && c->ray_table.bytes < (size_t)table_want * 16;
+    need_alloc = need_alloc || table_short;
     bool recs_stale = false;
     if ((rc = provision_records(r, &recs_stale))) return rc;
     if (need_alloc || recs_stale) {
@@ -117,7 +173,9 @@
             }
             HIP_TRY(hipStreamSynchronize(c->stream));
         }
-    }
+        if (table_short) ray_table_grow(c, table_want);
+    }
+    r.table = ray_table_use(c, table_want);
     if (need_alloc || recs_stale) {
         for (int g = 0; g < P.ngroups; ++g) {
             uvrt_ctx::RecsKey& key = c->b_recs_key[g];
@@ -193,9 +251,11 @@
     const int g = pc.g, ph0 = P.gfirst[g] + pc.k0;
     hipStream_t ls;
     if (int rcl = next_chunk_lane(r, &ls)) return rcl;
+    if (int rct = ray_table_order(c, r.table, c->lane, ls)) return rct;
     const size_t at = (size_t)ph0 * (size_t)P.n_pad + (size_t)pc.kc * (size_t)g0;
     GenDedupeParams dq;
     fill_dedupe_chunk(c, dq, pc, r.first_gid + g0, gn, cur_lane(c), r.light_length);
+    set_ray_table(c, r.table, dq);
     dq.rays = r.S.rays.as<float4>() + at;
     dq.masks = r.S.masks.as<uint32_t>() + at;
     dq.total = r.S.dd_counts.as<uint32_t>() + r.dd_used;
@@ -322,7 +382,7 @@
                     "(uvrt_set_flavour %d)", who, c->flavour);
     if (int rc = set_device(c)) return rc;
     const int set = c->b_set ^ 1;
-    BatchRun r = {c, set, c->bs[set], P, who, light_length, first_gid, n, {}, {}, {}, variant_per_cu(c->variant, c->pipeline ? 7 : 8), 0, 0};
+    BatchRun r = {c, set, c->bs[set], P, who, light_length, first_gid, n, {}, {}, {}, variant_per_cu(c->variant, c->pipeline ? 7 : 8), 0, 0, {}};
     if (int rc = provision_batch(r, count)) return rc;
     struct LaneGuard {
         uvrt_ctx* c; int lane; uint64_t chunks; bool armed;
@@ -578,8 +638,13 @@
     if (int rc = out_rays.ensure(slots * 16, false, c->stream)) return rc;
     if (int rc = out_words.ensure(slots * 4, false, c->stream)) return rc;
     if (int rc = out_counts.ensure(8, true, c->stream)) return rc;
+    const uint32_t table_want = ray_table_want(c, one);
+    if (table_want > c->ray_table_entries && c->ray_table.bytes < (size_t)table_want * 16) ray_table_grow(c, table_want);
+    RayTableUse table = ray_table_use(c, table_want);
+    if (int rc = ray_table_order(c, table, 0, c->stream)) return rc;
     GenDedupeParams dq;
     fill_dedupe_chunk(c, dq, pc, chunk_first, chunk_n, L, light_length);
+    set_ray_table(c, table, dq);
     dq.rays = out_rays.as<float4>();
     dq.masks = out_words.as<uint32_t>();
     dq.total = out_counts.as<uint32_t>();
@@ -598,6 +663,61 @@
     *total = counts[0];
     *deposits = counts[1];
     return UVRT_OK;
+}
+
+uint32_t uvrt_ray_table_index(uint32_t key) { return key < RAY_TABLE_KEY_END ? ray_table_index(key) : UINT32_MAX; }
+uint32_t uvrt_ray_table_key(uint32_t index) { return index <= RAY_TABLE_ENTRIES_MAX ? ray_table_key(index) : UINT32_MAX; }
+uint32_t uvrt_ray_table_entries(uint32_t max_key) { return ray_table_entries(max_key); }
+uint32_t uvrt_ray_table_fit(uint32_t max_key, uint64_t budget_bytes) { return ray_table_fit(max_key, budget_bytes); }
+
+int uvrt_set_ray_table(uvrt_ctx* c, int32_t max_mb)
+{
+    if (!c || max_mb < 0) return fail(UVRT_ERR_INVALID, "uvrt_set_ray_table: null context or a negative budget");
+    c->ray_table_budget = (uint64_t)max_mb << 20;
+    return UVRT_OK;
+}
+
+int uvrt_set_ray_table_bytes(uvrt_ctx* c, uint64_t max_bytes)
+{
+    if (!c) return fail(UVRT_ERR_INVALID, "uvrt_set_ray_table_bytes: null context");
+    c->ray_table_budget = max_bytes;
+    return UVRT_OK;
+}
+
+int uvrt_get_ray_table(uvrt_ctx* c, uint64_t* budget_bytes, uint32_t* entries, uint32_t* keys)
+{
+    if (!c || !budget_bytes || !entries || !keys) return fail(UVRT_ERR_INVALID, "uvrt_get_ray_table: null argument");
+    *budget_bytes = c->ray_table_budget;
+    *entries = c->ray_table_entries;
+    *keys = c->ray_table_entries ? ray_table_key(c->ray_table_entries) : 0u;
+    return UVRT_OK;
+}
+
+int uvrt_ray_table_build(uvrt_ctx* c, uint32_t max_key)
+{
+    if (!c) return fail(UVRT_ERR_INVALID, "uvrt_ray_table_build: null context");
+    if (int rc = set_device(c)) return rc;
+    if (int rc = join_all(c)) return rc;
+    HIP_TRY(hipStreamSynchronize(c->stream));
+    const uint32_t want = ray_table_fit(max_key, c->ray_table_budget);
+    if (want > c->ray_table_entries && c->ray_table.bytes < (size_t)want * 16) ray_table_grow(c, want);
+    RayTableUse table = ray_table_use(c, want);
+    if (int rc = ray_table_order(c, table, 0, c->stream)) return rc;
+    HIP_TRY(hipStreamSynchronize(c->stream));
+    return UVRT_OK;
+}
+
+int uvrt_ray_table_read(uvrt_ctx* c, uint32_t first, uint32_t count, float* out)
+{
+    if (!c || !out || (uint64_t)first + count > c->ray_table_entries)
+        return fail(UVRT_ERR_INVALID, "uvrt_ray_table_read: null argument, or entries the table does not hold");
+    if (int rc = set_device(c)) return rc;
+    if (int rc = join_all(c)) return rc;
+    if (c->ray_table_seen[0] != c->ray_table_gen) {
+        HIP_TRY(hipStreamWaitEvent(c->stream, c->ray_table_ev, 0));
+        c->ray_table_seen[0] = c->ray_table_gen;
+    }
+    return copy_sync(c, out, c->ray_table.as<float4>() + first, (size_t)count * 16, hipMemcpyDeviceToHost);
 }
 
 int uvrt_fold_batch(uvrt_ctx* c)
diff --git a/small-project-uv-robot-ray-tracer_amd/csrc/uvrt_ctx.h b/small-project-uv-robot-ray-tracer_amd/csrc/uvrt_ctx.h
--- a/small-project-uv-robot-ray-tracer_amd/csrc/uvrt_ctx.h
+++ b/small-project-uv-robot-ray-tracer_amd/csrc/uvrt_ctx.h
@@ -192,6 +192,12 @@
     int32_t b_traced_chunks = 0;
     int32_t dedupe_classes = uvrt::DEDUPE_CLASSES_DEFAULT;
     bool dedupe_periodic = uvrt::DEDUPE_PERIODIC_DEFAULT;
+    uint64_t ray_table_budget = (uint64_t)uvrt::RAY_TABLE_DEFAULT_MB << 20;
+    DevBuf ray_table;
+    uint32_t ray_table_entries = 0;
+    hipEvent_t ray_table_ev = nullptr;
+    uint64_t ray_table_gen = 0;
+    uint64_t ray_table_seen[MAXL] = {};
     int32_t dedupe_class_replicas = 4;
     size_t dedupe_class_bytes = (size_t)96 << 20;
     int32_t b_ncls = 0, b_cls_repl = 1;
diff --git a/small-project-uv-robot-ray-tracer_amd/csrc/uvrt_dedupe.h b/small-project-uv-robot-ray-tracer_amd/csrc/uvrt_dedupe.h
--- a/small-project-uv-robot-ray-tracer_amd/csrc/uvrt_dedupe.h
+++ b/small-project-uv-robot-ray-tracer_amd/csrc/uvrt_dedupe.h
@@ -601,4 +601,40 @@
     return from_table;
 }
 
-}
+constexpr uint32_t RAY_KEY_WITHOUT_RAY = 61u;
+constexpr uint32_t RAY_TABLE_KEY_END = 1u << 27;
+constexpr uint32_t RAY_TABLE_ENTRIES_MAX = 5u << 23;
+constexpr int32_t RAY_TABLE_DEFAULT_MB = 0;
+
+UVRT_HD uint32_t ray_table_index(uint32_t key)
+{
+    const uint32_t sh = key < (1u << 24) ? 0u : (uint32_t)(8 - __builtin_clz(key));
+    return (sh << 23) + (key >> sh);
+}
+UVRT_HD uint32_t ray_table_key(uint32_t index)
+{
+    const uint32_t sh = index < (1u << 24) ? 0u : (index >> 23) - 1u;
+    return (index - (sh << 23)) << sh;
+}
+UVRT_HD uint32_t ray_table_entries(uint32_t max_key)
+{
+    return max_key >= RAY_TABLE_KEY_END ? RAY_TABLE_ENTRIES_MAX : ray_table_index(max_key) + 1u;
+}
+inline uint32_t ray_table_fit(uint32_t max_key, uint64_t budget_bytes)
+{
+    const uint64_t room = budget_bytes / 16u;
+    const uint32_t want = ray_table_entries(max_key);
+    return (uint64_t)want <= room ? want : (uint32_t)room;
+}
+inline int64_t dedupe_max_key(const DedupeGroup& G)
+{
+    int64_t kmax = -1;
+    const int64_t last = G.first_gid + G.n - 1, lo1 = G.first_gid > 1 ? G.first_gid : 1;
+    for (int j = 0; j < G.count; ++j) {
+        if (G.first_gid == 0) kmax = std::max<int64_t>(kmax, G.key0[j]);
+        if (lo1 <= last) kmax = std::max<int64_t>(kmax, dedupe_key1(G, j, (int32_t)last));
+    }
+    return kmax;
+}
+
+}
diff --git a/small-project-uv-robot-ray-tracer_amd/csrc/uvrt_device.h b/small-project-uv-robot-ray-tracer_amd/csrc/uvrt_device.h
--- a/small-project-uv-robot-ray-tracer_amd/csrc/uvrt_device.h
+++ b/small-project-uv-robot-ray-tracer_amd/csrc/uvrt_device.h
@@ -93,14 +93,13 @@
     return (float)s * 2.3283064365387e-10f;
 }
 
-__device__ __forceinline__ float4 generate_ray_rng(float lx, float ly, float lz, float light_length, int64_t gid,
-                                                   uint32_t seed_prev, uint32_t seed_next, int32_t seed_mode,
-                                                   float& r0, double& x, double& y, uint32_t& seed)
-{
-    seed = wang_hash(seed_input(gid, lx, ly, lz, seed_prev, seed_next, seed_mode));
+template <bool ORIGIN>
+__device__ __forceinline__ float4 ray_behind_key(uint32_t h, float ly, float light_length, float& r0, double& x, double& y, uint32_t& seed)
+{
+    seed = wang_hash(h);
 
     r0 = random_float(seed);
-    const float origy = ly + r0 * light_length;
+    const float w = ORIGIN ? ly + r0 * light_length : r0;
     const float diry = random_float(seed) * 2.0f - 1.0f;
     const double dirxzlength = sqrt(1.0 - (double)diry * (double)diry);
 
@@ -111,7 +110,17 @@
         y = (double)(random_float(seed) * 2.0f - 1.0f);
     }
     const double s = dirxzlength / sqrt(x * x + y * y);
-    return make_float4((float)(x * s), diry, (float)(y * s), origy);
+    return make_float4((float)(x * s), diry, (float)(y * s), w);
+}
+__device__ __forceinline__ float4 ray_of_key(uint32_t h, float& r0, double& x, double& y, uint32_t& seed)
+{
+    return ray_behind_key<false>(h, 0.0f, 0.0f, r0, x, y, seed);
+}
+__device__ __forceinline__ float4 generate_ray_rng(float lx, float ly, float lz, float light_length, int64_t gid,
+                                                   uint32_t seed_prev, uint32_t seed_next, int32_t seed_mode,
+                                                   float& r0, double& x, double& y, uint32_t& seed)
+{
+    return ray_behind_key<true>(seed_input(gid, lx, ly, lz, seed_prev, seed_next, seed_mode), ly, light_length, r0, x, y, seed);
 }
 __device__ __forceinline__ float4 generate_ray(float lx, float ly, float lz, float light_length, int64_t gid,
                                                uint32_t seed_prev, uint32_t seed_next, int32_t seed_mode,
@@ -155,9 +164,12 @@
     int32_t gap_key[DEDUPE_PERIODIC_STRATA + 1];
     uint32_t gap_keys[DEDUPE_PERIODIC_STRATA + 1];
     int32_t gap_strip0[DEDUPE_PERIODIC_STRATA + 2];
+    const float4* ray_table;
+    uint32_t ray_table_keys;
 };
 static_assert(sizeof(GenDedupeParams) <= 3584, "kernel arguments: 4 KB with the hidden ones");
 void launch_generate_dedupe(const GenDedupeParams& p, hipStream_t s);
+void launch_ray_table_build(float4* table, uint32_t entries, hipStream_t s);
 void launch_dedupe_mark(const GenDedupeParams& p, hipStream_t s);
 struct ExtendParams;
 bool launch_extend6_dedupe(const ExtendParams& p, int code, int grid_per_cu, hipStream_t s);
diff --git a/small-project-uv-robot-ray-tracer_amd/csrc/uvrt_kernels.hip b/small-project-uv-robot-ray-tracer_amd/csrc/uvrt_kernels.hip
--- a/small-project-uv-robot-ray-tracer_amd/csrc/uvrt_kernels.hip
+++ b/small-project-uv-robot-ray-tracer_amd/csrc/uvrt_kernels.hip
@@ -230,7 +230,7 @@
             }
         }
     }
-    uint32_t mask[DD_ROUNDS], rank[DD_ROUNDS];
+    uint32_t mask[DD_ROUNDS];
 #pragma unroll
     for (int r = 0; r < DD_ROUNDS; ++r) mask[r] = 0u;
     for (uint32_t left = near; left != 0u; left &= left - 1u) {
@@ -255,36 +255,68 @@
             }
         }
     }
-    uint32_t pos = p.block_counts[(size_t)k * gridDim.x + blockIdx.x];
+    uint32_t pos = __builtin_amdgcn_readfirstlane(p.block_counts[(size_t)k * gridDim.x + blockIdx.x]);
 #pragma unroll
     for (int r = 0; r < DD_ROUNDS; ++r) {
         const int64_t i = (int64_t)blockIdx.x * DD_SLOTS + r * 256 + threadIdx.x;
         if (!((worded >> r) & 1u) && i < p.gn) mask[r] = p.tmp[(int64_t)k * p.gn + i];
         const unsigned long long owners = __builtin_amdgcn_ballot_w64(mask[r] != 0u);
-        rank[r] = __builtin_amdgcn_mbcnt_hi((uint32_t)(owners >> 32), __builtin_amdgcn_mbcnt_lo((uint32_t)owners, 0u));
         if ((threadIdx.x & 63u) == 0u) s_cnt[r][wv] = (uint32_t)__popcll(owners);
+    }
+    typedef float f32x4 __attribute__((ext_vector_type(4)));
+    f32x4 ent[DD_ROUNDS];
+    uint32_t tabled = 0u;
+    if (p.ray_table_keys != 0u) {
+        const f32x4* __restrict__ table = (const f32x4*)p.ray_table;
+#pragma unroll
+        for (int r = 0; r < DD_ROUNDS; ++r) {
+            const int32_t g = gid0 + r * 256;
+            const uint32_t key = (uint32_t)(g == 0 ? p.g.key0[k] : dedupe_key1_of(p.g, seed1, g));
+            if (mask[r] != 0u && key < p.ray_table_keys && key != RAY_KEY_WITHOUT_RAY) {
+                ent[r] = __builtin_nontemporal_load(&table[ray_table_index(key)]);
+                tabled |= 1u << r;
+            }
+        }
     }
     __syncthreads();
     if (threadIdx.x == 0) p.block_counts[(size_t)k * gridDim.x + blockIdx.x] = 0u;
 #pragma unroll
     for (int r = 0; r < DD_ROUNDS; ++r) {
-        for (uint32_t w = 0; w < 4u; ++w) {
-            if (w == wv && mask[r] != 0u) {
-                const int64_t i = (int64_t)blockIdx.x * DD_SLOTS + r * 256 + threadIdx.x;
-                float r0;
-                double x, y;
-                p.rays[pos + rank[r]] = generate_ray(p.g.lx, p.g.ly, p.g.lz, p.light_length, p.g0 + i, p.g.seed_prev[k],
-                                                     p.g.seed_next[k], p.g.seed_mode, r0, x, y);
-                const uint32_t word = ((worded >> r) & 1u) ? mask[r] : dedupe_deposit_word(classes, s_slot_mask, s_slot_word, mask[r]);
-                p.masks[pos + rank[r]] = word;
-                dep += (uint32_t)dedupe_word_deposits(classes, word);
-            }
-            pos += s_cnt[r][w];
-        }
+        const unsigned long long owners = __builtin_amdgcn_ballot_w64(mask[r] != 0u);
+        const uint32_t rank = __builtin_amdgcn_mbcnt_hi((uint32_t)(owners >> 32), __builtin_amdgcn_mbcnt_lo((uint32_t)owners, 0u));
+        const uint32_t c0 = __builtin_amdgcn_readfirstlane(s_cnt[r][0]), c1 = __builtin_amdgcn_readfirstlane(s_cnt[r][1]);
+        const uint32_t c2 = __builtin_amdgcn_readfirstlane(s_cnt[r][2]), c3 = __builtin_amdgcn_readfirstlane(s_cnt[r][3]);
+        const uint32_t at = pos + (wv > 0u ? c0 : 0u) + (wv > 1u ? c1 : 0u) + (wv > 2u ? c2 : 0u) + rank;
+        if (mask[r] != 0u) {
+            const int64_t i = (int64_t)blockIdx.x * DD_SLOTS + r * 256 + threadIdx.x;
+            float r0;
+            double x, y;
+            if ((tabled >> r) & 1u)
+                p.rays[at] = make_float4(ent[r].x, ent[r].y, ent[r].z, p.g.ly + ent[r].w * p.light_length);
+            else
+                p.rays[at] = generate_ray(p.g.lx, p.g.ly, p.g.lz, p.light_length, p.g0 + i, p.g.seed_prev[k], p.g.seed_next[k],
+                                          p.g.seed_mode, r0, x, y);
+            const uint32_t word = ((worded >> r) & 1u) ? mask[r] : dedupe_deposit_word(classes, s_slot_mask, s_slot_word, mask[r]);
+            p.masks[at] = word;
+            dep += (uint32_t)dedupe_word_deposits(classes, word);
+        }
+        pos += c0 + c1 + c2 + c3;
     }
     if (dep != 0u) atomicAdd(&s_dep, dep);
     __syncthreads();
     if (threadIdx.x == 0 && s_dep != 0u) atomicAdd(p.deposits, s_dep);
+}
+
+__global__ __launch_bounds__(256) void k_ray_table_build(float4* __restrict__ table, uint32_t entries)
+{
+    const uint32_t i = blockIdx.x * 256u + threadIdx.x;
+    if (i >= entries) return;
+    const uint32_t key = ray_table_key(i);
+    if (key == RAY_KEY_WITHOUT_RAY) { table[i] = make_float4(0.0f, 0.0f, 0.0f, 0.0f); return; }
+    float r0;
+    double x, y;
+    uint32_t seed;
+    table[i] = ray_of_key(key, r0, x, y, seed);
 }
 
 __global__ __launch_bounds__(1024) void k_scan_bins(uint32_t* hist, uint32_t* bin_start,
@@ -701,6 +733,12 @@
     hipLaunchKernelGGL(k_dedupe_write, grid, dim3(256), 0, s, p);
 }
 
+void launch_ray_table_build(float4* table, uint32_t entries, hipStream_t s)
+{
+    if (entries == 0u) return;
+    hipLaunchKernelGGL(k_ray_table_build, dim3((entries + 255u) / 256u), dim3(256), 0, s, table, entries);
+}
+
 void launch_fold_planes(int32_t* planes, int32_t* folded, int32_t nplanes, int32_t replicas, int32_t T, int prio, hipStream_t s)
 {
     if (nplanes <= 0 || T <= 0) return;
```

Result: no change. 17320 Mray/s (-0.3%).
